# smhassanerfani/nasa-niswan

Measured on NVIDIA B200. Metric: train samples/sec, higher is better.
Workload: dtype bf16

## Files before the change

nasa_niswan_b200/csrc/nint_api.cu:

```cuda
#include <cuda.h>
#include <cuda_runtime.h>
#include <stdarg.h>
#include <stdio.h>
#include <stdlib.h>
#include <string.h>

#include <new>
#include <vector>

#include "../../include/nint.h"
#include "nint_kernels.h"

namespace {

using namespace nint;
enum : int { BF16 = 0, TF32 = 1 };

thread_local char g_err[512] = "";
int fail(const char* fmt, ...) {
  va_list ap;
  va_start(ap, fmt);
  vsnprintf(g_err, sizeof(g_err), fmt, ap);
  va_end(ap);
  return 1;
}
#define CK(expr)                                                                                   \
  do {                                                                                             \
    cudaError_t e__ = (expr);                                                                      \
    if (e__ != cudaSuccess) return fail("%s failed: %s (%s:%d)", #expr, cudaGetErrorString(e__), __FILE__, __LINE__); \
  } while (0)

typedef CUresult (*EncodeTiledFn)(CUtensorMap*, CUtensorMapDataType, cuuint32_t, void*, const cuuint64_t*,
                                  const cuuint64_t*, const cuuint32_t*, const cuuint32_t*, CUtensorMapInterleave,
                                  CUtensorMapSwizzle, CUtensorMapL2promotion, CUtensorMapFloatOOBfill);
EncodeTiledFn get_encode() {
  static EncodeTiledFn fn = nullptr;
  if (!fn) {
    void* p = nullptr;
    cudaDriverEntryPointQueryResult q;
    if (cudaGetDriverEntryPoint("cuTensorMapEncodeTiled", &p, cudaEnableDefault, &q) == cudaSuccess &&
        q == cudaDriverEntryPointSuccess)
      fn = reinterpret_cast<EncodeTiledFn>(p);
  }
  return fn;
}

inline size_t align_up(size_t v, size_t a) { return (v + a - 1) / a * a; }

enum : int { K_FWD = 0, K_BWD = 1, K_WGRAD = 2, K_OTHER = 3, K_NCLS = 4 };
constexpr int kResidCtas = 160;
constexpr long long kResidMaxPixelSteps = 1LL << 20;
long long g_launches[K_NCLS] = {0, 0, 0, 0};

struct Profile {
  bool on = false;
  std::vector<cudaEvent_t> pool;
  std::vector<int> cls;
  std::vector<int> weight;
  size_t used = 0;
};

struct Layer {
  int cin, hc_real, hc, k, taps;
  int cin_rows;
  int cx_pad, hc_pad, chx, chh;
  int hcb, n_blocks, n_tile;
  int nslots_h, nslots_c;
  uint8_t* Hs = nullptr;
  float* Cs = nullptr;
  uint8_t* G = nullptr;
  float* dC = nullptr;
  uint8_t *wx = nullptr, *wh = nullptr, *wdx = nullptr, *wdh = nullptr;
  float *bias_q = nullptr, *dw_acc = nullptr, *db_acc = nullptr;
  float* db_resid = nullptr;
  size_t dw_acc_bytes = 0;
  int det_splits = 0;
  int ncols = 0;
  CUtensorMap tm_H, tm_G;
  struct WMap { int ts = 0, rows = 0, n_tile = 0; CUtensorMap map; };
  std::vector<WMap> wmaps[4];
  CUtensorMap tm_H_up;
  CUtensorMap tmw_H, tmw_G;
  CUtensorMap tmw_H_up;
  CUtensorMap tmp_G, tmp_H, tmp_H_up;
  struct WgBlock {
    int col0 = 0, cols = 0;
    int n_mma = 0;
    int nch_x = 0, nch_h = 0;
    int chan0_x = 0, chan0_h = 0;
    bool pair = false;
    int pw = 16, a_bufs = 0, b_stages = 0;
  };
  std::vector<WgBlock> wg_blocks;
  CUtensorMap tme_C, tme_H, tme_G, tme_dC;
  bool weights_set = false;
  bool bias_folded = false;
  struct CachedConv { bool valid = false; ConvGemmParams g; };
  CachedConv fwd_cache[2][2], bwd_cache[2];
};

}

struct nint_plan {
  nint_config cfg;
  int L, B, T, H, W, dtype, esize, ce;
  int tile_w, tile_h, tiles_x, tiles_y;
  int num_sms = 148;
  Layer layer[NINT_MAX_LAYERS];
  size_t ws_bytes = 0;
  uint8_t* ws = nullptr;
  uint8_t* X = nullptr;
  CUtensorMap tm_X, tmw_X, tmp_X;
  bool x_bank = false;
  const void* bank_ptr = nullptr;
  long long bank_frames = 0;
  const int* win_start = nullptr;
  CUtensorMap tmb_X, tmbw_X, tmbp_X;
  float *head_w = nullptr, *head_b = nullptr;
  float* raw = nullptr;
  float* dh_ext = nullptr;
  float* head_part = nullptr;
  unsigned* step_done = nullptr;
  int fuse_steps = -1;
  bool head_set = false;
  bool zero_init = true;
  bool fwd_done = false;
  bool gates_valid = false;
  bool bptt_done = false;
  bool deterministic = false, input_grad = false;
  int pdl = 0;
  int sub_batch = 0;
  int final_slot_h = 0, final_slot_c = 0;
  int cluster = 2;
  int debug_flags = 0;
  int ones_lane = -1;
  int plan_g = 0, plan_ns = 0;
  Profile prof;
};

namespace {

template <typename F>
int launch(nint_plan* p, int cls, cudaStream_t st, const char* what, F&& f) {
  cudaEvent_t e1 = nullptr;
  if (p && p->prof.on) {
    Profile& pr = p->prof;
    if (pr.pool.size() < 2 * (pr.used + 1)) {
      cudaEvent_t a, b;
      if (cudaEventCreate(&a) != cudaSuccess || cudaEventCreate(&b) != cudaSuccess) return fail("cudaEventCreate failed");
      pr.pool.push_back(a);
      pr.pool.push_back(b);
    }
    e1 = pr.pool[2 * pr.used + 1];
    if (pr.cls.size() <= pr.used) pr.cls.resize(pr.used + 1), pr.weight.resize(pr.used + 1);
    pr.cls[pr.used] = cls;
    pr.weight[pr.used] = 1;
    cudaEventRecord(pr.pool[2 * pr.used], st);
    ++pr.used;
  }
  cudaError_t e = f();
  if (e1) cudaEventRecord(e1, st);
  if (e != cudaSuccess) return fail("%s failed: %s", what, cudaGetErrorString(e));
  ++g_launches[cls];
  return 0;
}
#define LAUNCH(plan, cls, st, call) \
  do { if (launch(plan, cls, st, #call, [&]() { return (call); })) return 1; } while (0)

int pick_tile(int H, int W, int* tw_out, int* th_out) {
  (void)H; (void)W;
  *tw_out = 8;
  *th_out = 16;
  return 0;
}

int encode_act_map(CUtensorMap* m, int dtype, void* base, int C, int W, int H, int B, int slots, int ce, int tw,
                   int th, bool wgrad = false, int halo = 0) {
  tw += 2 * halo;
  th += 2 * halo;
  EncodeTiledFn enc = get_encode();
  if (!enc) return fail("cuTensorMapEncodeTiled not available (no CUDA driver?)");
  const cuuint64_t es = dtype == BF16 ? 2 : 4;
  cuuint64_t dims[5] = {(cuuint64_t)C, (cuuint64_t)W, (cuuint64_t)H, (cuuint64_t)B, (cuuint64_t)slots};
  cuuint64_t strides[4] = {C * es, (cuuint64_t)W * C * es, (cuuint64_t)H * W * C * es,
                           (cuuint64_t)B * H * W * C * es};
  cuuint32_t box[5] = {(cuuint32_t)(wgrad ? 32 : ce), (cuuint32_t)tw, (cuuint32_t)th, 1, 1};
  cuuint32_t estr[5] = {1, 1, 1, 1, 1};
  const CUtensorMapSwizzle sw = (wgrad && dtype == TF32) ? CU_TENSOR_MAP_SWIZZLE_128B_ATOM_32B : CU_TENSOR_MAP_SWIZZLE_64B;
  CUresult r = enc(m, dtype == BF16 ? CU_TENSOR_MAP_DATA_TYPE_BFLOAT16 : CU_TENSOR_MAP_DATA_TYPE_FLOAT32, 5, base,
                   dims, strides, box, estr, CU_TENSOR_MAP_INTERLEAVE_NONE, sw,
                   CU_TENSOR_MAP_L2_PROMOTION_L2_128B, CU_TENSOR_MAP_FLOAT_OOB_FILL_NONE);
  if (r != CUDA_SUCCESS) return fail("cuTensorMapEncodeTiled(activation C=%d W=%d H=%d B=%d slots=%d) -> %d", C, W, H, B, slots, (int)r);
  return 0;
}

int encode_act_box(CUtensorMap* m, int dtype, void* base, int C, int W, int H, int B, int slots, int box_c, int tw,
                   int th, int halo, CUtensorMapSwizzle sw) {
  EncodeTiledFn enc = get_encode();
  if (!enc) return fail("cuTensorMapEncodeTiled not available (no CUDA driver?)");
  const cuuint64_t es = dtype == BF16 ? 2 : 4;
  cuuint64_t dims[5] = {(cuuint64_t)C, (cuuint64_t)W, (cuuint64_t)H, (cuuint64_t)B, (cuuint64_t)slots};
  cuuint64_t strides[4] = {C * es, (cuuint64_t)W * C * es, (cuuint64_t)H * W * C * es,
                           (cuuint64_t)B * H * W * C * es};
  cuuint32_t box[5] = {(cuuint32_t)box_c, (cuuint32_t)(tw + 2 * halo), (cuuint32_t)(th + 2 * halo), 1, 1};
  cuuint32_t estr[5] = {1, 1, 1, 1, 1};
  CUresult r = enc(m, dtype == BF16 ? CU_TENSOR_MAP_DATA_TYPE_BFLOAT16 : CU_TENSOR_MAP_DATA_TYPE_FLOAT32, 5, base,
                   dims, strides, box, estr, CU_TENSOR_MAP_INTERLEAVE_NONE, sw, CU_TENSOR_MAP_L2_PROMOTION_L2_128B,
                   CU_TENSOR_MAP_FLOAT_OOB_FILL_NONE);
  if (r != CUDA_SUCCESS) return fail("cuTensorMapEncodeTiled(box C=%d box_c=%d halo=%d) -> %d", C, box_c, halo, (int)r);
  return 0;
}

int encode_io_map(CUtensorMap* m, bool fp32, void* base, int C, int W, int H, int B, int slots, int box_c) {
  EncodeTiledFn enc = get_encode();
  if (!enc) return fail("cuTensorMapEncodeTiled not available (no CUDA driver?)");
  const cuuint64_t es = fp32 ? 4 : 2;
  cuuint64_t dims[5] = {(cuuint64_t)C, (cuuint64_t)W, (cuuint64_t)H, (cuuint64_t)B, (cuuint64_t)slots};
  cuuint64_t strides[4] = {C * es, (cuuint64_t)W * C * es, (cuuint64_t)H * W * C * es,
                           (cuuint64_t)B * H * W * C * es};
  cuuint32_t box[5] = {(cuuint32_t)box_c, 8, 16, 1, 1};
  cuuint32_t estr[5] = {1, 1, 1, 1, 1};
  const int row_bytes = box_c * (int)es;
  CUtensorMapSwizzle sw;
  if (row_bytes == 32) sw = CU_TENSOR_MAP_SWIZZLE_32B;
  else if (row_bytes == 64) sw = CU_TENSOR_MAP_SWIZZLE_64B;
  else if (row_bytes == 128) sw = CU_TENSOR_MAP_SWIZZLE_128B;
  else return fail("encode_io_map: unsupported box row of %d bytes", row_bytes);
  CUresult r = enc(m, fp32 ? CU_TENSOR_MAP_DATA_TYPE_FLOAT32 : CU_TENSOR_MAP_DATA_TYPE_BFLOAT16, 5, base, dims, strides,
                   box, estr, CU_TENSOR_MAP_INTERLEAVE_NONE, sw, CU_TENSOR_MAP_L2_PROMOTION_L2_128B,
                   CU_TENSOR_MAP_FLOAT_OOB_FILL_NONE);
  if (r != CUDA_SUCCESS) return fail("cuTensorMapEncodeTiled(io C=%d W=%d H=%d B=%d slots=%d box=%d) -> %d", C, W, H, B, slots, box_c, (int)r);
  return 0;
}

int encode_w_map(CUtensorMap* m, int dtype, void* base, long long chunk_taps, int ce, int n_tile, int w_rows, int ts) {
  EncodeTiledFn enc = get_encode();
  if (!enc) return fail("cuTensorMapEncodeTiled not available (no CUDA driver?)");
  const cuuint64_t es = dtype == BF16 ? 2 : 4;
  cuuint64_t dims[3] = {(cuuint64_t)ce, (cuuint64_t)n_tile, (cuuint64_t)chunk_taps};
  cuuint64_t strides[2] = {ce * es, (cuuint64_t)n_tile * ce * es};
  cuuint32_t box[3] = {(cuuint32_t)ce, (cuuint32_t)w_rows, (cuuint32_t)ts};
  cuuint32_t estr[3] = {1, 1, 1};
  CUresult r = enc(m, dtype == BF16 ? CU_TENSOR_MAP_DATA_TYPE_BFLOAT16 : CU_TENSOR_MAP_DATA_TYPE_FLOAT32, 3, base,
                   dims, strides, box, estr, CU_TENSOR_MAP_INTERLEAVE_NONE, CU_TENSOR_MAP_SWIZZLE_64B,
                   CU_TENSOR_MAP_L2_PROMOTION_L2_256B, CU_TENSOR_MAP_FLOAT_OOB_FILL_NONE);
  if (r != CUDA_SUCCESS) return fail("cuTensorMapEncodeTiled(weights chunk_taps=%lld n_tile=%d rows=%d ts=%d) -> %d", chunk_taps, n_tile, w_rows, ts, (int)r);
  return 0;
}

uint32_t idesc_of(int dtype, int m, int n, int a_mn, int b_mn) {
  const uint32_t fmt = dtype == BF16 ? 1u : 2u;
  return (1u << 4) | (fmt << 7) | (fmt << 10) | ((uint32_t)(a_mn & 1) << 15) | ((uint32_t)(b_mn & 1) << 16) |
         ((uint32_t)(n >> 3) << 17) | ((uint32_t)(m >> 4) << 24);
}

size_t act_bytes(const nint_plan* p, int slots, int c) {
  return static_cast<size_t>(slots) * p->B * p->H * p->W * c * p->esize;
}

size_t carve(nint_plan* p, uint8_t* base) {
  size_t off = 0;
  auto take = [&](size_t bytes) -> uint8_t* {
    uint8_t* r = base ? base + off : nullptr;
    off += align_up(bytes, 1024);
    return r;
  };
  const bool tr = p->cfg.training != 0;
  const size_t npix = static_cast<size_t>(p->B) * p->H * p->W;
  p->X = take(act_bytes(p, p->T, p->layer[0].cx_pad));
  for (int l = 0; l < p->L; ++l) {
    Layer& y = p->layer[l];
    y.Hs = take(act_bytes(p, y.nslots_h, y.hc_pad));
    y.Cs = reinterpret_cast<float*>(take(static_cast<size_t>(y.nslots_c) * npix * y.hc * 4));
    y.G = tr ? take(act_bytes(p, p->T, 4 * y.hc)) : nullptr;
    y.dC = tr ? reinterpret_cast<float*>(take(npix * y.hc * 4)) : nullptr;
    const size_t wrow = static_cast<size_t>(p->ce) * p->esize;
    y.wx = take(static_cast<size_t>(y.n_blocks) * y.taps * y.chx * y.n_tile * wrow);
    y.wh = take(static_cast<size_t>(y.n_blocks) * y.taps * y.chh * y.n_tile * wrow);
    y.bias_q = reinterpret_cast<float*>(take(4 * y.hc * 4));
    if (tr) {
      const int nch = 4 * y.hc / p->ce;
      y.wdx = (l > 0 || p->input_grad) ? take(static_cast<size_t>(y.taps) * nch * y.cin_rows * wrow) : nullptr;
      y.wdh = take(static_cast<size_t>(y.taps) * nch * y.hc * wrow);
      y.dw_acc_bytes = static_cast<size_t>(y.taps) * 4 * y.hc * y.ncols * 4;
      const size_t slices = p->deterministic ? static_cast<size_t>(y.det_splits) : 1;
      y.dw_acc = reinterpret_cast<float*>(take(y.dw_acc_bytes * slices));
      y.db_acc = reinterpret_cast<float*>(take(4 * y.hc * 4 * slices));
      y.db_resid = p->dtype == TF32 ? reinterpret_cast<float*>(take(static_cast<size_t>(kResidCtas) * 4 * 4 * y.hc * 4)) : nullptr;
    }
  }
  const Layer& top = p->layer[p->L - 1];
  p->head_w = reinterpret_cast<float*>(take(top.hc * 4));
  p->head_b = reinterpret_cast<float*>(take(16));
  if (tr && p->deterministic)
    p->head_part = reinterpret_cast<float*>(take(static_cast<size_t>(head_bwd_blocks(p->B)) * (top.hc_real + 1) * 4));
  p->step_done = reinterpret_cast<unsigned*>(take(static_cast<size_t>(p->T) * p->B * 4));
  if (tr && p->input_grad) {
    const Layer& y0 = p->layer[0];
    const size_t cols = y0.cin_rows > y0.hc ? y0.cin_rows : y0.hc;
    p->raw = reinterpret_cast<float*>(take(npix * cols * 4));
    p->dh_ext = reinterpret_cast<float*>(take(npix * y0.hc * 4));
  }
  return off;
}

inline uint8_t* slot_ptr(const nint_plan* p, uint8_t* base, int slot, int c) {
  return base + act_bytes(p, 1, c) * slot;
}
inline float* cslot_ptr(const nint_plan* p, const Layer& y, int slot) {
  return y.Cs + static_cast<size_t>(slot) * p->B * p->H * p->W * y.hc;
}

void fill_common(const nint_plan* p, const Layer& y, ConvGemmParams& g) {
  memset(&g, 0, sizeof(g));
  g.debug_flags = p->debug_flags;
  g.pdl = p->pdl;
  g.plan_g = p->plan_g; g.plan_ns = p->plan_ns;
  g.B = p->B; g.b0 = 0; g.H = p->H; g.W = p->W;
  g.tile_w = p->tile_w; g.tile_h = p->tile_h; g.tiles_x = p->tiles_x; g.tiles_y = p->tiles_y;
  g.hc = y.hc; g.hc_pad = y.hc_pad; g.hcb = y.hcb;
  g.n_steps = 1;
  g.c_prev_none_step = -1;
}

int arm_fused(nint_plan* p, ConvGemmParams& g, int n_steps, int storer_warps, cudaStream_t st) {
  g.n_steps = n_steps;
  g.step_done = p->step_done;
  g.step_target = static_cast<unsigned>(p->tiles_x * p->tiles_y * g.n_blocks * storer_warps);
  if (reinterpret_cast<uint8_t*>(p->step_done) < p->ws ||
      reinterpret_cast<uint8_t*>(p->step_done + static_cast<size_t>(n_steps) * p->B) > p->ws + p->ws_bytes)
    return fail("internal: step counters outside the workspace (%p, ws %p + %zu)", (void*)p->step_done, (void*)p->ws, p->ws_bytes);
  CK(cudaMemsetAsync(p->step_done, 0, static_cast<size_t>(n_steps) * p->B * 4, st));
  return 0;
}

int fwd_cluster(const nint_plan* p, int l) {
  (void)l;
  return p->cluster;
}
int bwd_cluster(const nint_plan* p, int l) {
  return p->layer[l].hc % 32 == 0 ? p->cluster : 1;
}

int get_w_map(nint_plan* p, Layer& y, int which, int n_tile, int rows, int ts, CUtensorMap* out) {
  for (const Layer::WMap& w : y.wmaps[which])
    if (w.ts == ts && w.rows == rows && w.n_tile == n_tile) { *out = w.map; return 0; }
  void* base = which == 0 ? y.wx : which == 1 ? y.wh : which == 2 ? y.wdx : y.wdh;
  if (!base) return fail("internal: packed weight tensor %d of this layer was not allocated", which);
  long long chunk_taps;
  if (which == 0) chunk_taps = (long long)y.n_blocks * y.chx * y.taps;
  else if (which == 1) chunk_taps = (long long)y.n_blocks * y.chh * y.taps;
  else chunk_taps = (long long)(4 * y.hc / p->ce) * y.taps;
  Layer::WMap w;
  w.ts = ts; w.rows = rows; w.n_tile = n_tile;
  if (encode_w_map(&w.map, p->dtype, base, chunk_taps, p->ce, n_tile, rows, ts)) return 1;
  y.wmaps[which].push_back(w);
  *out = w.map;
  return 0;
}

inline void set_batch_range(const nint_plan* p, ConvGemmParams& g, int b0, int nb) {
  g.b0 = nb > 0 ? b0 : 0;
  g.B = nb > 0 ? nb : p->B;
}

int fwd_conv_params(nint_plan* p, int l, bool have_state, int epi, ConvGemmParams& g) {
  Layer& y = p->layer[l];
  const bool tr = p->cfg.training != 0;
  const bool bank = l == 0 && p->x_bank;
  Layer::CachedConv* cache = epi == EPI_FWD ? &y.fwd_cache[have_state ? 1 : 0][bank ? 1 : 0] : nullptr;
  if (cache && cache->valid) {
    g = cache->g;
  } else {
    fill_common(p, y, g);
    g.n_tile = y.n_tile;
    g.n_blocks = y.n_blocks;
    g.cluster = fwd_cluster(p, l);
    g.idesc = idesc_of(p->dtype, 128 * g.cluster, y.n_tile, 0, 0);
    int s = 0;
    g.seg[s].tmap_act = l == 0 ? (bank ? p->tmb_X : p->tm_X) : p->layer[l - 1].tm_H_up;
    g.seg[s].wsel = 0;
    g.seg[s].ksize = y.k;
    g.seg[s].nchunks = y.chx;
    ++s;
    if (have_state) {
      g.seg[s].tmap_act = y.tm_H;
      g.seg[s].wsel = 1;
      g.seg[s].ksize = y.k;
      g.seg[s].nchunks = y.chh;
      ++s;
    }
    g.nseg = s;
    g.tm_c = y.tme_C; g.tm_h = y.tme_H; g.tm_g = y.tme_G; g.tm_dc = y.tme_dC;
    g.slot_g = (tr && epi == EPI_FWD) ? 0 : -1;
    if (conv_halo_plan(epi, p->dtype, g)) return fail("layer %d: the conv kernel's shared-memory plan does not fit (hidden %d, k %d)", l, y.hc, y.k);
    for (int i = 0; i < g.nseg; ++i)
      if (get_w_map(p, y, g.seg[i].wsel, g.n_tile, g.n_tile / g.cluster, g.seg[i].ts, &g.seg[i].tmap_w)) return 1;
    if (cache) { cache->g = g; cache->valid = true; }
  }
  return 0;
}

int cell_step(nint_plan* p, int l, int t, int epi, float* raw_out, cudaStream_t st, int b0 = 0, int nb = 0, int n_steps = 1) {
  Layer& y = p->layer[l];
  const bool tr = p->cfg.training != 0;
  const bool have_state = !(t == 0 && p->zero_init);
  const bool bank = l == 0 && p->x_bank;
  ConvGemmParams g;
  if (fwd_conv_params(p, l, have_state, epi, g)) return 1;
  const int in_slot_h = tr ? t : (t & 1);
  const int out_slot_h = tr ? t + 1 : ((t + 1) & 1);
  g.seg[0].slot = l == 0 ? t : (tr ? t + 1 : ((t + 1) & 1));
  g.seg[0].win_start = bank ? p->win_start : nullptr;
  g.seg[0].bank_frames = bank ? static_cast<int>(p->bank_frames) : 0;
  if (have_state) g.seg[1].slot = in_slot_h;
  g.slot_c_in = have_state ? (tr ? t : 0) : -1;
  g.slot_c_out = tr ? t + 1 : 0;
  g.slot_h_out = out_slot_h;
  g.slot_g = (tr && epi == EPI_FWD) ? t : -1;
  g.bias_q = (y.bias_folded && epi == EPI_FWD) ? nullptr : y.bias_q;
  g.raw_out = raw_out;
  set_batch_range(p, g, b0, nb);
  g.n_steps = 1;
  if (n_steps > 1) {
    if (!have_state || epi != EPI_FWD || nb > 0) return fail("internal: time-fused forward launch without a recurrent state");
    g.d_seg[0] = g.d_seg[1] = g.d_h_out = g.d_g = 1;
    g.d_c_in = g.d_c_out = tr ? 1 : 0;
    g.ring_bits = tr ? 0 : ((l > 0 ? 1 : 0) | 2 | 16);
    if (arm_fused(p, g, n_steps, 2, st)) return 1;
  }
  LAUNCH(p, (epi == EPI_FWD ? K_FWD : K_OTHER), st, launch_conv_halo(epi, p->dtype, g, p->num_sms, st));
  if (p->prof.on && p->prof.used > 0) p->prof.weight[p->prof.used - 1] = n_steps;
  return 0;
}

int dgrad_raw(nint_plan* p, int l, int t, int wsel, int n_rows, float* raw_out, cudaStream_t st) {
  Layer& y = p->layer[l];
  ConvGemmParams g;
  fill_common(p, y, g);
  g.n_tile = n_rows;
  g.n_blocks = 1;
  g.cluster = (n_rows % 32 == 0) ? p->cluster : 1;
  g.idesc = idesc_of(p->dtype, 128 * g.cluster, n_rows, 0, 0);
  g.seg[0].tmap_act = y.tm_G; g.seg[0].wsel = wsel; g.seg[0].slot = t;
  g.seg[0].ksize = y.k; g.seg[0].nchunks = 4 * y.hc / p->ce;
  g.nseg = 1;
  g.tm_c = y.tme_C; g.tm_h = y.tme_H; g.tm_g = y.tme_G; g.tm_dc = y.tme_dC;
  g.slot_g = g.slot_c_in = g.slot_c_out = g.slot_h_out = g.slot_c_prev = -1;
  g.raw_out = raw_out;
  if (conv_halo_plan(EPI_RAW, p->dtype, g)) return fail("layer %d: the dgrad kernel's shared-memory plan does not fit (N %d, k %d)", l, n_rows, y.k);
  if (get_w_map(p, y, wsel, g.n_tile, g.n_tile / g.cluster, g.seg[0].ts, &g.seg[0].tmap_w)) return 1;
  LAUNCH(p, K_OTHER, st, launch_conv_halo(EPI_RAW, p->dtype, g, p->num_sms, st));
  return 0;
}

}

static int plan_wgrad_blocks(nint_plan* p, Layer& y) {
  y.wg_blocks.clear();
  const int px = y.cx_pad / 32, ph = y.hc_pad / 32;
  auto pair_block = [&](int col0, int x_cols, int cols) {
    Layer::WgBlock b;
    b.col0 = col0; b.cols = cols;
    b.nch_x = x_cols / 32; b.nch_h = (cols - x_cols) / 32;
    b.pair = true;
    b.pw = wgrad_pair_panel_width(x_cols, cols);
    b.a_bufs = 3;
    b.b_stages = wgrad_pair_b_stages(x_cols, cols, y.k);
    b.n_mma = cols;
    return b;
  };
  if (p->cluster == 2 && p->dtype == TF32 && (4 * y.hc) % 256 == 0 && &y == &p->layer[0] && p->ones_lane >= 0) {
    const int n_mma = (y.ncols / 32 + 1) / 2 * 64;
    const int st = n_mma <= 256 ? wgrad_pair_b_stages_tf32(n_mma, y.k) : 0;
    if (st >= 2) {
      Layer::WgBlock b;
      b.col0 = 0; b.cols = y.ncols; b.n_mma = n_mma;
      b.nch_x = y.cx_pad / 32; b.nch_h = y.hc_pad / 32;
      b.pair = true; b.pw = 32; b.a_bufs = 2; b.b_stages = st;
      y.wg_blocks.push_back(b);
      return 0;
    }
  }
  if (p->cluster == 2 && p->dtype == BF16 && (4 * y.hc) % 256 == 0) {
    if (wgrad_pair_supported(p->dtype, 4 * y.hc, y.cx_pad, y.ncols, y.k)) {
      y.wg_blocks.push_back(pair_block(0, y.cx_pad, y.ncols));
      return 0;
    }
    if (wgrad_pair_supported(p->dtype, 4 * y.hc, y.cx_pad, y.cx_pad, y.k) &&
        wgrad_pair_supported(p->dtype, 4 * y.hc, 0, y.hc_pad, y.k)) {
      y.wg_blocks.push_back(pair_block(0, y.cx_pad, y.cx_pad));
      y.wg_blocks.push_back(pair_block(y.cx_pad, 0, y.hc_pad));
      return 0;
    }
  }
  const int panels = px + ph, bpb = wgrad_b_panel_bytes(p->dtype, 1, y.k);
  int per = panels, a_bufs = 0, b_stages = 0;
  for (; per >= 1; --per) {
    wgrad_pick_buffers(p->dtype, per, bpb, &a_bufs, &b_stages);
    if (per * 32 <= 256 && (b_stages >= 2 || (per == 1 && b_stages >= 1))) break;
  }
  if (per < 1) return 1;
  for (int j0 = 0; j0 < panels; j0 += per) {
    const int j1 = j0 + per < panels ? j0 + per : panels;
    Layer::WgBlock b;
    b.col0 = j0 * 32; b.cols = b.n_mma = (j1 - j0) * 32;
    b.nch_x = (j1 < px ? j1 : px) - (j0 < px ? j0 : px);
    b.nch_h = (j1 - j0) - b.nch_x;
    b.chan0_x = (j0 < px ? j0 : px) * 32;
    b.chan0_h = (j0 > px ? j0 - px : 0) * 32;
    wgrad_pick_buffers(p->dtype, j1 - j0, bpb, &b.a_bufs, &b.b_stages);
    y.wg_blocks.push_back(b);
  }
  return 0;
}

static int wgrad_params(nint_plan* p, int l, size_t bi, int num_sms, WgradParams& w) {
  Layer& y = p->layer[l];
  const int T = p->T;
  const Layer::WgBlock& blk = y.wg_blocks[bi];
  const int bias_col = (l == 0) ? p->ones_lane : -1;
  const long long total_tiles = static_cast<long long>(T) * p->B * p->tiles_x * p->tiles_y;
  memset(&w, 0, sizeof(w));
  w.halo = 1;
  w.debug_flags = p->debug_flags;
  w.b_panel_bytes = wgrad_b_panel_bytes(p->dtype, w.halo, y.k);
  w.slot_b0[0] = l == 0 ? 0 : 1;
  w.slot_b0[1] = 0;
  w.nchunks_b[0] = blk.nch_x;
  w.nchunks_b[1] = blk.nch_h;
  w.chan0[0] = blk.chan0_x;
  w.chan0[1] = blk.chan0_h;
  w.T = T; w.B = p->B; w.H = p->H; w.W = p->W;
  w.tile_w = p->tile_w; w.tile_h = p->tile_h; w.tiles_x = p->tiles_x; w.tiles_y = p->tiles_y;
  w.ksize = y.k;
  w.hc4 = 4 * y.hc;
  w.pair = blk.pair ? 1 : 0;
  const bool bank = l == 0 && p->x_bank;
  w.win_start = bank ? p->win_start : nullptr;
  if (w.pair && p->dtype == BF16) {
    w.tmap_dg = y.tmp_G;
    w.tmap_b[0] = l == 0 ? (bank ? p->tmbp_X : p->tmp_X) : p->layer[l - 1].tmp_H_up;
    w.tmap_b[1] = y.tmp_H;
  } else {
    w.tmap_dg = y.tmw_G;
    w.tmap_b[0] = l == 0 ? (bank ? p->tmbw_X : p->tmw_X) : p->layer[l - 1].tmw_H_up;
    w.tmap_b[1] = y.tmw_H;
  }
  if (blk.nch_x == 0) { w.tmap_b[0] = w.tmap_b[1]; w.win_start = nullptr; }
  if (blk.nch_h == 0) w.tmap_b[1] = w.tmap_b[0];
  w.m_blocks = w.pair ? w.hc4 / 256 : (w.hc4 + 127) / 128;
  w.ncols = y.ncols;
  w.acc_cols = blk.n_mma;
  w.real_cols = blk.cols;
  w.col0 = blk.col0;
  const int bias_cols = (bias_col >= 0 || bi > 0) ? 0 : 32;
  const int tpg = 512 / blk.n_mma;
  if (tpg < 1) return fail("wgrad: %d columns exceed the accumulator", blk.n_mma);
  int ng = 0, tap = 0;
  w.group_tap0[0] = 0;
  const int rest = y.taps % tpg;
  const bool bias_last = rest > 0 && rest * blk.n_mma + bias_cols <= 512;
  const int g0 = bias_last ? tpg : ((512 - bias_cols) / blk.n_mma < tpg ? (512 - bias_cols) / blk.n_mma : tpg);
  if (g0 < 1) return fail("wgrad: %d columns leave no room for the bias columns", blk.n_mma);
  while (tap < y.taps) {
    const int n = ng == 0 ? g0 : tpg;
    tap = tap + n > y.taps ? y.taps : tap + n;
    if (ng + 1 > kMaxWgradGroups) return fail("wgrad: too many tap groups");
    w.group_tap0[++ng] = tap;
  }
  w.bias_group = bias_cols == 0 ? -1 : (bias_last ? ng - 1 : 0);
  w.n_groups = ng;
  {
    int units = (w.pair ? num_sms / 2 : num_sms) / w.m_blocks;
    if (units < ng) units = ng;
    auto mma_cost = [&](int n) { return w.pair ? (n / 2 > 40 ? n / 2 : 40) : (n * 2 / 3 > 88 ? n * 2 / 3 : 88); };
    int cost[kMaxWgradGroups], tot = 0;
    for (int g = 0; g < ng; ++g) {
      cost[g] = (w.group_tap0[g + 1] - w.group_tap0[g]) * mma_cost(blk.n_mma) + (g == w.bias_group ? mma_cost(32) : 0);
      tot += cost[g];
    }
    const bool even = (p->debug_flags & 64) != 0;
    int used = 0;
    for (int g = 0; g < ng; ++g) {
      int sp = even ? units / ng : static_cast<int>(static_cast<long long>(units) * cost[g] / tot);
      if (sp < 1) sp = 1;
      w.group_splits[g] = sp;
      used += sp;
    }
    while (!even && used < units) {
      int best = 0;
      for (int g = 1; g < ng; ++g)
        if (static_cast<long long>(cost[g]) * w.group_splits[best] > static_cast<long long>(cost[best]) * w.group_splits[g]) best = g;
      ++w.group_splits[best];
      ++used;
    }
    w.group_unit0[0] = 0;
    for (int g = 0; g < ng; ++g) {
      if (w.group_splits[g] > total_tiles) w.group_splits[g] = static_cast<int>(total_tiles);
      w.group_unit0[g + 1] = w.group_unit0[g] + w.m_blocks * w.group_splits[g];
    }
  }
  w.b_pw = blk.pw;
  w.a_bufs = blk.a_bufs;
  w.b_stages = blk.b_stages;
  if (w.b_stages < 1) return fail("wgrad: operand panels do not fit in shared memory");
  w.idesc = idesc_of(p->dtype, w.pair ? 256 : 128, blk.n_mma, 1, 1);
  w.idesc_bias = idesc_of(p->dtype, w.pair ? 256 : 128, 32, 1, 1);
  w.dw_acc = y.dw_acc;
  w.db_acc = y.db_acc;
  w.dw_part = p->deterministic ? y.dw_acc : nullptr;
  w.db_part = p->deterministic ? y.db_acc : nullptr;
  return 0;
}
static int wgrad_max_splits(const WgradParams& w) {
  int m = 1;
  for (int g = 0; g < w.n_groups; ++g) if (w.group_splits[g] > m) m = w.group_splits[g];
  return m;
}

extern "C" {

int nint_version(void) { return 100; }
const char* nint_last_error(void) { return g_err; }
int nint_gate_column(int q, int hidden) { return q_to_n(q, hidden); }
int nint_pick_tile(int height, int width, int* tile_w, int* tile_h) {
  if (height < 1 || width < 1 || !tile_w || !tile_h) return fail("nint_pick_tile: bad arguments");
  return pick_tile(height, width, tile_w, tile_h);
}

long long nint_launch_count(int kernel_class) {
  if (kernel_class < 0) return g_launches[0] + g_launches[1] + g_launches[2] + g_launches[3];
  return kernel_class < K_NCLS ? g_launches[kernel_class] : 0;
}

int nint_plan_profile(nint_plan* p, int enable) {
  if (!p) return fail("null plan");
  p->prof.on = enable != 0;
  p->prof.used = 0;
  return 0;
}

int nint_plan_profile_read(nint_plan* p, double* ms, long long* count) {
  if (!p || !ms || !count) return fail("nint_plan_profile_read: null argument");
  Profile& pr = p->prof;
  for (int c = 0; c < K_NCLS; ++c) ms[c] = 0.0, count[c] = 0;
  for (size_t i = 0; i < pr.used; ++i) {
    CK(cudaEventSynchronize(pr.pool[2 * i + 1]));
    float t = 0.f;
    CK(cudaEventElapsedTime(&t, pr.pool[2 * i], pr.pool[2 * i + 1]));
    ms[pr.cls[i]] += t;
    count[pr.cls[i]] += pr.weight[i];
  }
  pr.used = 0;
  return 0;
}

int nint_plan_create(const nint_config* cfg, nint_plan** out) {
  if (!cfg || !out) return fail("nint_plan_create: null argument");
  if (cfg->num_layers < 1 || cfg->num_layers > NINT_MAX_LAYERS)
    return fail("num_layers must be in [1,%d], got %d", NINT_MAX_LAYERS, cfg->num_layers);
  if (cfg->batch < 1 || cfg->seq_len < 1 || cfg->height < 1 || cfg->width < 1 || cfg->in_channels < 1)
    return fail("batch/seq_len/height/width/in_channels must be positive");
  if (cfg->dtype != BF16 && cfg->dtype != TF32) return fail("unknown dtype %d", cfg->dtype);
  nint_plan* p = new (std::nothrow) nint_plan();
  if (!p) return fail("out of host memory");
  p->cfg = *cfg;
  p->L = cfg->num_layers; p->B = cfg->batch; p->T = cfg->seq_len; p->H = cfg->height; p->W = cfg->width;
  p->dtype = cfg->dtype;
  p->esize = cfg->dtype == BF16 ? 2 : 4;
  p->ce = 64 / p->esize;
  p->deterministic = (cfg->flags & NINT_FLAG_DETERMINISTIC) != 0;
  p->input_grad = (cfg->flags & NINT_FLAG_INPUT_GRAD) != 0;
  {
    const char* c = getenv("NINT_CLUSTER");
    p->cluster = c ? atoi(c) : 2;
    if (p->cluster != 1 && p->cluster != 2) p->cluster = 1;
    const char* d = getenv("NINT_DEBUG_FLAGS");
    p->debug_flags = d ? atoi(d) : 0;
    if (!NINT_KNOBS && (p->debug_flags & ~512)) {
      const int flags = p->debug_flags;
      delete p;
      return fail("NINT_DEBUG_FLAGS=%d needs the experiment build of the library (python -m nasa_niswan_b200.build --knobs, "
                  "then NINT_LIB=<...>/libnint_knobs.so): the product build compiles the kernel knobs out", flags);
    }
    const char* pg = getenv("NINT_PLAN_G");
    p->plan_g = pg ? atoi(pg) : 0;
    const char* pn = getenv("NINT_PLAN_NS");
    p->plan_ns = pn ? atoi(pn) : 0;
    if (const char* e = getenv("NINT_DETERMINISTIC")) p->deterministic = p->deterministic || atoi(e) != 0;
    const char* pd = getenv("NINT_PDL");
    p->pdl = pd ? (atoi(pd) != 0) : 0;
    if (const char* e = getenv("NINT_FUSE_STEPS")) p->fuse_steps = atoi(e);
    const char* sb = getenv("NINT_SUB_BATCH");
    p->sub_batch = sb ? atoi(sb) : 0;
    if (p->sub_batch < 0 || p->sub_batch >= p->B) p->sub_batch = 0;
  }
  pick_tile(p->H, p->W, &p->tile_w, &p->tile_h);
  p->tiles_x = (p->W + p->tile_w - 1) / p->tile_w;
  p->tiles_y = (p->H + p->tile_h - 1) / p->tile_h;
  int cin = cfg->in_channels, below_hc = 0;
  for (int l = 0; l < p->L; ++l) {
    Layer& y = p->layer[l];
    y.cin = cin; y.hc_real = cfg->hidden[l]; y.k = cfg->ksize[l]; y.taps = y.k * y.k;
    if (y.hc_real < 1 || y.hc_real > 256) {
      delete p;
      return fail("hidden_channels[%d] = %d unsupported (1 .. 256)", l, cfg->hidden[l]);
    }
    y.hc = y.hc_real <= 64 ? (y.hc_real + 15) / 16 * 16 : (y.hc_real + 63) / 64 * 64;
    if (y.k < 1 || y.k % 2 == 0 || y.k > 15) {
      delete p;
      return fail("kernel_size[%d] = %d unsupported (odd, <= 15)", l, y.k);
    }
    if (l > 0 && cin > 256) { delete p; return fail("layer %d input channels %d > 256", l, cin); }
    y.cx_pad = l == 0 ? (y.cin + 31) / 32 * 32 : (below_hc + 31) / 32 * 32;
    y.chx = y.cx_pad / p->ce;
    y.hc_pad = (y.hc + 31) / 32 * 32;  y.chh = y.hc_pad / p->ce;
    y.cin_rows = l == 0 ? y.cx_pad : below_hc;
    if (l == 0 && y.cx_pad > y.cin && !(p->debug_flags & 128)) p->ones_lane = y.cin;
    y.hcb = y.hc < 64 ? y.hc : 64;
    if (cfg->dtype == BF16) {
      bool fits = false;
      for (int cand = y.hcb; cand >= 32 && !fits; cand >>= 1) {
        const long long w_cta = static_cast<long long>(y.cx_pad / 32 + y.hc_pad / 32) * y.taps * (4 * cand / p->cluster) * 64;
        if (y.hc % cand == 0 && w_cta <= 112 * 1024) { y.hcb = cand; fits = true; }
      }
      if (!fits && y.hc >= 32 && y.hc % 32 == 0) y.hcb = 32;
    }
    if (const char* e = getenv("NINT_HCB")) {
      const int v = atoi(e);
      if (v >= 16 && v <= 64 && (v & (v - 1)) == 0 && y.hc % v == 0) y.hcb = v;
    }
    y.n_blocks = y.hc / y.hcb; y.n_tile = 4 * y.hcb;
    y.nslots_h = cfg->training ? p->T + 1 : 2;
    y.nslots_c = cfg->training ? p->T + 1 : 1;
    y.ncols = y.cx_pad + y.hc_pad;
    if (cfg->training && plan_wgrad_blocks(p, y)) {
      const int hc = y.hc, k = y.k;
      delete p;
      return fail("layer %d: training with hidden %d, kernel %d: not even one 32-channel wgrad operand panel fits in "
                  "shared memory", l, hc, k);
    }
    if (cfg->training && p->deterministic) {
      y.det_splits = 1;
      for (size_t bi = 0; bi < y.wg_blocks.size(); ++bi) {
        WgradParams w;
        if (wgrad_params(p, l, bi, 148, w)) { delete p; return 1; }
        if (wgrad_max_splits(w) > y.det_splits) y.det_splits = wgrad_max_splits(w);
      }
    }
    cin = y.hc_real;
    below_hc = y.hc;
  }
  if (p->input_grad && cfg->training && p->layer[0].cin_rows > 256) {
    delete p;
    return fail("input gradient: %d input channels exceed one MMA N (256)", cfg->in_channels);
  }
  p->ws_bytes = carve(p, nullptr);
  *out = p;
  return 0;
}

void nint_plan_destroy(nint_plan* plan) {
  if (!plan) return;
  for (cudaEvent_t e : plan->prof.pool) cudaEventDestroy(e);
  delete plan;
}

size_t nint_plan_workspace_bytes(const nint_plan* plan) { return plan ? plan->ws_bytes : 0; }

int nint_plan_input_layout(const nint_plan* plan, int* c_pad, int* ones_lane, int* elem_bytes) {
  if (!plan) return fail("null plan");
  if (c_pad) *c_pad = plan->layer[0].cx_pad;
  if (ones_lane) *ones_lane = plan->ones_lane;
  if (elem_bytes) *elem_bytes = plan->esize;
  return 0;
}

static int encode_input_maps(nint_plan* p, void* base, long long images, int slots, CUtensorMap* conv, CUtensorMap* wg,
                             CUtensorMap* wg_pair) {
  const int tw = p->tile_w, th = p->tile_h, ce = p->ce, pad0 = p->layer[0].k / 2;
  Layer& y = p->layer[0];
  if (images > 0x7fffffffLL) return fail("too many frames (%lld)", images);
  const int n = static_cast<int>(images);
  if (encode_act_map(conv, p->dtype, base, y.cx_pad, p->W, p->H, n, slots, ce, tw, th, false, pad0)) return 1;
  if (encode_act_map(wg, p->dtype, base, y.cx_pad, p->W, p->H, n, slots, ce, tw, th, true, pad0)) return 1;
  if (p->cfg.training && p->dtype == BF16)
    for (const Layer::WgBlock& b : y.wg_blocks) {
      if (!b.pair || b.nch_x == 0) continue;
      const CUtensorMapSwizzle sw = b.pw == 64 ? CU_TENSOR_MAP_SWIZZLE_128B : (b.pw == 32 ? CU_TENSOR_MAP_SWIZZLE_64B : CU_TENSOR_MAP_SWIZZLE_32B);
      if (encode_act_box(wg_pair, p->dtype, base, y.cx_pad, p->W, p->H, n, slots, b.pw, tw, th, pad0, sw)) return 1;
    }
  return 0;
}

int nint_plan_bind(nint_plan* p, void* workspace, size_t bytes, void* stream) {
  if (!p || !workspace) return fail("nint_plan_bind: null argument");
  if (bytes < p->ws_bytes) return fail("workspace too small: %zu < %zu", bytes, p->ws_bytes);
  if (reinterpret_cast<uintptr_t>(workspace) % 256) return fail("workspace must be 256-byte aligned");
  cudaStream_t st = static_cast<cudaStream_t>(stream);
  int dev = 0, sms = 0, cc_major = 0;
  CK(cudaGetDevice(&dev));
  CK(cudaDeviceGetAttribute(&sms, cudaDevAttrMultiProcessorCount, dev));
  CK(cudaDeviceGetAttribute(&cc_major, cudaDevAttrComputeCapabilityMajor, dev));
  if (cc_major != 10) return fail("libnint needs an sm_100 device (Blackwell B200); found compute capability %d.x", cc_major);
  p->num_sms = sms;
  p->ws = static_cast<uint8_t*>(workspace);
  carve(p, p->ws);
  CK(cudaMemsetAsync(p->ws, 0, p->ws_bytes, st));
  const int tw = p->tile_w, th = p->tile_h, ce = p->ce;
  auto pad_of = [&](int l) { return p->layer[l].k / 2; };
  if (encode_input_maps(p, p->X, p->B, p->T, &p->tm_X, &p->tmw_X, &p->tmp_X)) return 1;
  p->x_bank = false; p->bank_ptr = nullptr; p->bank_frames = 0; p->win_start = nullptr;
  for (int l = 0; l < p->L; ++l) {
    Layer& y = p->layer[l];
    for (auto& a : y.fwd_cache) for (auto& c : a) c.valid = false;
    for (auto& c : y.bwd_cache) c.valid = false;
    if (encode_act_map(&y.tm_H, p->dtype, y.Hs, y.hc_pad, p->W, p->H, p->B, y.nslots_h, ce, tw, th, false, pad_of(l))) return 1;
    if (l + 1 < p->L &&
        encode_act_map(&y.tm_H_up, p->dtype, y.Hs, y.hc_pad, p->W, p->H, p->B, y.nslots_h, ce, tw, th, false, pad_of(l + 1))) return 1;
    if (encode_io_map(&y.tme_C, true, y.Cs, y.hc, p->W, p->H, p->B, y.nslots_c, 16)) return 1;
    if (encode_io_map(&y.tme_H, p->dtype == TF32, y.Hs, y.hc_pad, p->W, p->H, p->B, y.nslots_h, 16)) return 1;
    if (p->cfg.training) {
      if (encode_io_map(&y.tme_G, p->dtype == TF32, y.G, 4 * y.hc, p->W, p->H, p->B, p->T, 128 / p->esize)) return 1;
      if (encode_io_map(&y.tme_dC, true, y.dC, y.hc, p->W, p->H, p->B, 1, 16)) return 1;
    } else {
      y.tme_G = y.tme_C;
      y.tme_dC = y.tme_C;
    }
    for (auto& v : y.wmaps) v.clear();
    if (p->cfg.training) {
      if (encode_act_map(&y.tm_G, p->dtype, y.G, 4 * y.hc, p->W, p->H, p->B, p->T, ce, tw, th, false, pad_of(l))) return 1;
      if (encode_act_map(&y.tmw_G, p->dtype, y.G, 4 * y.hc, p->W, p->H, p->B, p->T, ce, tw, th, true)) return 1;
      if (encode_act_map(&y.tmw_H, p->dtype, y.Hs, y.hc_pad, p->W, p->H, p->B, y.nslots_h, ce, tw, th, true, pad_of(l))) return 1;
      if (l + 1 < p->L &&
          encode_act_map(&y.tmw_H_up, p->dtype, y.Hs, y.hc_pad, p->W, p->H, p->B, y.nslots_h, ce, tw, th, true, pad_of(l + 1))) return 1;
    }
  }
  if (p->cfg.training) {
    for (int l = 0; l < p->L; ++l) {
      Layer& y = p->layer[l];
      auto sw_of = [](int pw) {
        return pw == 64 ? CU_TENSOR_MAP_SWIZZLE_128B : (pw == 32 ? CU_TENSOR_MAP_SWIZZLE_64B : CU_TENSOR_MAP_SWIZZLE_32B);
      };
      bool any_pair = false;
      for (const Layer::WgBlock& b : y.wg_blocks) {
        if (!b.pair || p->dtype != BF16) continue;
        any_pair = true;
        if (b.nch_h > 0 &&
            encode_act_box(&y.tmp_H, p->dtype, y.Hs, y.hc_pad, p->W, p->H, p->B, y.nslots_h, b.pw, tw, th, pad_of(l), sw_of(b.pw))) return 1;
        if (b.nch_x > 0 && l > 0) {
          Layer& dn = p->layer[l - 1];
          if (encode_act_box(&dn.tmp_H_up, p->dtype, dn.Hs, dn.hc_pad, p->W, p->H, p->B, dn.nslots_h, b.pw, tw, th, pad_of(l), sw_of(b.pw))) return 1;
        }
      }
      if (any_pair &&
          encode_act_box(&y.tmp_G, p->dtype, y.G, 4 * y.hc, p->W, p->H, p->B, p->T, 64, tw, th, 0, CU_TENSOR_MAP_SWIZZLE_128B)) return 1;
    }
  }
  p->zero_init = true;
  p->fwd_done = false;
  p->gates_valid = false;
  p->bptt_done = false;
  return 0;
}

int nint_plan_set_weights(nint_plan* p, int l, const float* weight, const float* bias, void* stream) {
  if (!p || !p->ws) return fail("plan not bound");
  if (l < 0 || l >= p->L) return fail("layer %d out of range", l);
  if (!weight) return fail("null weight");
  Layer& y = p->layer[l];
  cudaStream_t st = static_cast<cudaStream_t>(stream);
  y.bias_folded = l == 0 && p->ones_lane >= 0 && bias != nullptr && !(p->debug_flags & 512);
  LAUNCH(p, K_OTHER, st, launch_pack_weights_fwd(p->dtype, weight, bias, y.wx, y.wh, y.bias_q, y.cin, y.hc_real, y.hc, y.hcb, y.k, y.cx_pad, y.hc_pad,
                                                 y.bias_folded ? p->ones_lane : -1, st));
  if (p->cfg.training) LAUNCH(p, K_OTHER, st, launch_pack_weights_bwd(p->dtype, weight, y.wdx, y.wdh, y.cin, y.cin_rows, y.hc_real, y.hc, y.k, st));
  y.weights_set = true;
  return 0;
}

int nint_plan_set_head(nint_plan* p, const float* weight, const float* bias, void* stream) {
  if (!p || !p->ws) return fail("plan not bound");
  if (!weight || !bias) return fail("null head parameter");
  cudaStream_t st = static_cast<cudaStream_t>(stream);
  CK(cudaMemcpyAsync(p->head_w, weight, p->layer[p->L - 1].hc_real * 4, cudaMemcpyDeviceToDevice, st));
  CK(cudaMemcpyAsync(p->head_b, bias, 4, cudaMemcpyDeviceToDevice, st));
  p->head_set = true;
  return 0;
}

int nint_plan_reset_state(nint_plan* p, void* stream) {
  if (!p || !p->ws) return fail("plan not bound");
  cudaStream_t st = static_cast<cudaStream_t>(stream);
  if (!p->zero_init) {
    for (int l = 0; l < p->L; ++l) {
      Layer& y = p->layer[l];
      CK(cudaMemsetAsync(y.Hs, 0, act_bytes(p, 1, y.hc_pad), st));
      CK(cudaMemsetAsync(y.Cs, 0, static_cast<size_t>(p->B) * p->H * p->W * y.hc * 4, st));
    }
  }
  p->zero_init = true;
  return 0;
}

int nint_plan_set_state(nint_plan* p, int l, const float* h, const float* c, void* stream) {
  if (!p || !p->ws) return fail("plan not bound");
  if (l < 0 || l >= p->L || !h || !c) return fail("nint_plan_set_state: bad arguments");
  Layer& y = p->layer[l];
  cudaStream_t st = static_cast<cudaStream_t>(stream);
  if (p->zero_init) {
    for (int j = 0; j < p->L; ++j) {
      Layer& z = p->layer[j];
      CK(cudaMemsetAsync(z.Hs, 0, act_bytes(p, 1, z.hc_pad), st));
      CK(cudaMemsetAsync(z.Cs, 0, static_cast<size_t>(p->B) * p->H * p->W * z.hc * 4, st));
    }
  }
  LAUNCH(p, K_OTHER, st, launch_pack_state(p->dtype, h, y.Hs, p->B, y.hc_real, p->H, p->W, y.hc_pad, st));
  LAUNCH(p, K_OTHER, st, launch_nchw_to_nhwc_f32(c, y.Cs, p->B, y.hc_real, p->H, p->W, y.hc, st));
  p->zero_init = false;
  return 0;
}

int nint_plan_get_state(nint_plan* p, int l, float* h, float* c, void* stream) {
  if (!p || !p->ws) return fail("plan not bound");
  if (l < 0 || l >= p->L) return fail("layer %d out of range", l);
  if (!p->fwd_done) return fail("nint_plan_get_state before nint_forward");
  Layer& y = p->layer[l];
  cudaStream_t st = static_cast<cudaStream_t>(stream);
  if (h) LAUNCH(p, K_OTHER, st, launch_unpack_state(p->dtype, slot_ptr(p, y.Hs, p->final_slot_h, y.hc_pad), h, p->B, y.hc_real, p->H, p->W, y.hc_pad, st));
  if (c) LAUNCH(p, K_OTHER, st, launch_nhwc_to_nchw_f32(cslot_ptr(p, y, p->final_slot_c), c, p->B, y.hc_real, p->H, p->W, y.hc, st));
  return 0;
}

static int check_ready(nint_plan* p) {
  if (!p || !p->ws) return fail("plan not bound");
  for (int l = 0; l < p->L; ++l)
    if (!p->layer[l].weights_set) return fail("weights of layer %d not set", l);
  if (!p->head_set) return fail("head parameters not set");
  return 0;
}

static int fwd_should_fuse(nint_plan* p, int l, bool* fuse) {
  *fuse = false;
  if (p->fuse_steps == 0) return 0;
  if (p->fuse_steps > 0) {
    *fuse = (p->fuse_steps & 1) != 0;
    return 0;
  }
  ConvGemmParams g;
  if (fwd_conv_params(p, l, true, EPI_FWD, g)) return 1;
  const int per_group = g.cluster * g.group;
  const double groups = (static_cast<double>(p->B) * p->tiles_x * p->tiles_y + per_group - 1) / per_group;
  const int clusters = p->num_sms / (g.cluster * g.n_blocks);
  *fuse = clusters > 0 && groups / clusters <= 16.0;
  return 0;
}

static int forward_steps(nint_plan* p, float* pred, float* seq, cudaStream_t st) {
  const bool tr = p->cfg.training != 0;
  const long long HW = static_cast<long long>(p->H) * p->W;
  const Layer& top = p->layer[p->L - 1];
  const size_t top_img = static_cast<size_t>(HW) * top.hc_pad * p->esize;
  const int SB = p->sub_batch > 0 ? p->sub_batch : p->B;
  bool fuse_l[NINT_MAX_LAYERS];
  bool any_fused = false;
  for (int l = 0; l < p->L; ++l) {
    fuse_l[l] = false;
    if (SB >= p->B && p->T > 1 && (tr || (p->L == 1 && !seq)) && fwd_should_fuse(p, l, &fuse_l[l])) return 1;
    any_fused = any_fused || fuse_l[l];
  }
  if (any_fused) {
    for (int l = 0; l < p->L; ++l) {
      int t = 0;
      if (p->zero_init || !fuse_l[l]) {
        if (cell_step(p, l, 0, EPI_FWD, nullptr, st)) return 1;
        t = 1;
      }
      if (!fuse_l[l] || p->T - t == 1) {
        for (; t < p->T; ++t)
          if (cell_step(p, l, t, EPI_FWD, nullptr, st)) return 1;
      } else if (cell_step(p, l, t, EPI_FWD, nullptr, st, 0, 0, p->T - t)) return 1;
    }
    if (seq)
      for (int t = 0; t < p->T; ++t)
        LAUNCH(p, K_OTHER, st, launch_head_fwd(p->dtype, slot_ptr(p, top.Hs, t + 1, top.hc_pad), p->head_w, p->head_b,
                           seq + t * HW, HW, p->B, top.hc_real, top.hc_pad, p->T * HW, st));
  } else
  for (int b0 = 0; b0 < p->B; b0 += SB) {
    const int nb = b0 + SB <= p->B ? SB : p->B - b0;
    for (int t = 0; t < p->T; ++t) {
      for (int l = 0; l < p->L; ++l)
        if (cell_step(p, l, t, EPI_FWD, nullptr, st, b0, SB < p->B ? nb : 0)) return 1;
      if (seq) {
        const int slot = tr ? t + 1 : ((t + 1) & 1);
        LAUNCH(p, K_OTHER, st, launch_head_fwd(p->dtype, slot_ptr(p, top.Hs, slot, top.hc_pad) + b0 * top_img, p->head_w, p->head_b,
                           seq + b0 * p->T * HW + t * HW, HW, nb, top.hc_real, top.hc_pad, p->T * HW, st));
      }
    }
  }
  p->final_slot_h = tr ? p->T : (p->T & 1);
  p->final_slot_c = tr ? p->T : 0;
  LAUNCH(p, K_OTHER, st, launch_head_fwd(p->dtype, slot_ptr(p, top.Hs, p->final_slot_h, top.hc_pad), p->head_w, p->head_b, pred, HW, p->B,
                     top.hc_real, top.hc_pad, HW, st));
  p->fwd_done = true;
  p->gates_valid = tr;
  p->bptt_done = false;
  return 0;
}

int nint_forward_ex(nint_plan* p, const void* x, int x_dtype, float* pred, float* seq, void* stream) {
  if (check_ready(p)) return 1;
  if (!x || !pred) return fail("nint_forward: null x / pred");
  if (seq && !p->cfg.return_sequence) return fail("seq output requires return_sequence in the plan");
  if (x_dtype != NINT_X_FP32 && x_dtype != NINT_X_BF16) return fail("unknown x dtype %d", x_dtype);
  if (x_dtype == NINT_X_BF16 && p->dtype != BF16) return fail("bf16 inputs need a bf16 plan (a tf32 plan would lose input precision)");
  cudaStream_t st = static_cast<cudaStream_t>(stream);
  p->x_bank = false;
  LAUNCH(p, K_OTHER, st, launch_pack_input(p->dtype, x, x_dtype == NINT_X_BF16, p->X, p->B, p->T, p->cfg.in_channels, p->H, p->W, p->layer[0].cx_pad, p->ones_lane, st));
  return forward_steps(p, pred, seq, st);
}

int nint_forward(nint_plan* p, const float* x, float* pred, float* seq, void* stream) {
  return nint_forward_ex(p, x, NINT_X_FP32, pred, seq, stream);
}

int nint_forward_bank(nint_plan* p, const void* bank, long long n_frames, const int* win_start, float* pred, float* seq,
                      void* stream) {
  if (check_ready(p)) return 1;
  if (!bank || !win_start || !pred) return fail("nint_forward_bank: null bank / win_start / pred");
  if (n_frames < p->T) return fail("nint_forward_bank: %lld frames cannot hold a window of %d steps", n_frames, p->T);
  if (reinterpret_cast<uintptr_t>(bank) % 128) return fail("the frame bank must be 128-byte aligned");
  if (seq && !p->cfg.return_sequence) return fail("seq output requires return_sequence in the plan");
  cudaStream_t st = static_cast<cudaStream_t>(stream);
  if (bank != p->bank_ptr || n_frames != p->bank_frames) {
    if (encode_input_maps(p, const_cast<void*>(bank), n_frames, 1, &p->tmb_X, &p->tmbw_X, &p->tmbp_X)) return 1;
    p->bank_ptr = bank;
    p->bank_frames = n_frames;
    for (auto& a : p->layer[0].fwd_cache) a[1].valid = false;
  }
  p->x_bank = true;
  p->win_start = win_start;
  return forward_steps(p, pred, seq, st);
}

int nint_pack_frames(int dtype, const void* frames, int x_dtype, long long n_frames, int channels, int height, int width,
                     int c_pad, int ones_lane, void* bank, void* stream) {
  if (!frames || !bank) return fail("nint_pack_frames: null argument");
  if (dtype != BF16 && dtype != TF32) return fail("unknown dtype %d", dtype);
  if (x_dtype != NINT_X_FP32 && x_dtype != NINT_X_BF16) return fail("unknown x dtype %d", x_dtype);
  if (n_frames < 1 || channels < 1 || height < 1 || width < 1) return fail("nint_pack_frames: bad shape");
  if (c_pad < channels || c_pad % 16) return fail("nint_pack_frames: c_pad %d must be a multiple of 16 and >= %d", c_pad, channels);
  if (ones_lane >= 0 && (ones_lane < channels || ones_lane >= c_pad)) return fail("nint_pack_frames: ones lane %d outside the padding lanes", ones_lane);
  cudaStream_t st = static_cast<cudaStream_t>(stream);
  LAUNCH(nullptr, K_OTHER, st, launch_pack_frames(dtype, frames, x_dtype == NINT_X_BF16, bank, n_frames, channels, height, width, c_pad, ones_lane, st));
  return 0;
}

static int check_fuse_args(const float* levels3d, const float* emis2d, const float* mean, const float* std,
                           const float* statics, int n_static, long long frames, int levels, int height, int width,
                           int padded_height, int padded_width, int mode, const void* out) {
  if ((!levels3d && levels > 0) || !emis2d || !mean || !std || !out) return fail("nint_fuse_inputs: null argument");
  if (n_static < 0 || (n_static > 0 && !statics)) return fail("nint_fuse_inputs: %d static fields but no data", n_static);
  if (frames < 1 || levels < 0 || height < 1 || width < 1) return fail("nint_fuse_inputs: bad shape");
  if (mode != 0 && mode != 1) return fail("nint_fuse_inputs: mode must be 0 (reflect) or 1 (reference RNN dataset)");
  const int left = (padded_width - width) / 2, right = padded_width - width - left;
  const int top = (padded_height - height) / 2, bot = padded_height - height - top;
  if (padded_width < width || padded_height < height) return fail("nint_fuse_inputs: padded size smaller than the grid");
  if (left > width || right > width)
    return fail("The requested padding size is larger than width size of the input image.");
  if (top + 1 > height || bot + 1 > height)
    return fail("The requested padding size is larger than height size of the input image.");
  return 0;
}

int nint_fuse_inputs(const float* levels3d, const float* emis2d, const float* mean, const float* std,
                     const float* statics, int n_static, long long frames, int levels, int height, int width,
                     int padded_height, int padded_width, int mode, float* out, void* stream) {
  if (check_fuse_args(levels3d, emis2d, mean, std, statics, n_static, frames, levels, height, width, padded_height, padded_width, mode, out)) return 1;
  cudaStream_t st = static_cast<cudaStream_t>(stream);
  LAUNCH(nullptr, K_OTHER, st, launch_fuse_inputs(levels3d, emis2d, mean, std, statics, n_static, out, frames, levels, height, width, padded_height, padded_width, mode, st));
  return 0;
}

int nint_fuse_inputs_bank(const float* levels3d, const float* emis2d, const float* mean, const float* std,
                          const float* statics, int n_static, long long frames, int levels, int height, int width,
                          int padded_height, int padded_width, int mode, int dtype, int c_pad, int ones_lane,
                          void* bank, void* stream) {
  if (check_fuse_args(levels3d, emis2d, mean, std, statics, n_static, frames, levels, height, width, padded_height, padded_width, mode, bank)) return 1;
  if (dtype != BF16 && dtype != TF32) return fail("unknown dtype %d", dtype);
  const int C = levels + 1 + n_static;
  if (c_pad < C || c_pad % 16 || c_pad > 64) return fail("nint_fuse_inputs_bank: c_pad %d must be a multiple of 16 in [%d, 64]", c_pad, C);
  if (ones_lane >= 0 && (ones_lane < C || ones_lane >= c_pad)) return fail("nint_fuse_inputs_bank: ones lane %d outside the padding lanes", ones_lane);
  cudaStream_t st = static_cast<cudaStream_t>(stream);
  LAUNCH(nullptr, K_OTHER, st, launch_fuse_inputs_bank(dtype, levels3d, emis2d, mean, std, statics, n_static, bank, frames, levels, height, width, padded_height, padded_width, mode, c_pad, ones_lane, st));
  return 0;
}

static int check_loss_args(const float* pred, const float* y, const float* loss, const float* stats, int batch, int height,
                           int width, int crop_y0, int crop_y1, int crop_x0, int crop_x1) {
  if (!pred || !y || !loss || !stats) return fail("nint_loss_mse_l1: null argument");
  if (batch < 1 || height < 1 || width < 1) return fail("nint_loss_mse_l1: bad shape");
  if (crop_y0 < 0 || crop_y1 > height || crop_y0 >= crop_y1 || crop_x0 < 0 || crop_x1 > width || crop_x0 >= crop_x1)
    return fail("nint_loss_mse_l1: crop [%d:%d, %d:%d] outside %dx%d", crop_y0, crop_y1, crop_x0, crop_x1, height, width);
  return 0;
}

int nint_loss_mse_l1(const float* pred, const float* y, int batch, int height, int width, int crop_y0, int crop_y1,
                     int crop_x0, int crop_x1, float* dpred, float* loss, float* stats, void* stream) {
  if (check_loss_args(pred, y, loss, stats, batch, height, width, crop_y0, crop_y1, crop_x0, crop_x1)) return 1;
  cudaStream_t st = static_cast<cudaStream_t>(stream);
  LAUNCH(nullptr, K_OTHER, st, launch_loss_mse_l1(pred, y, dpred, stats, loss, batch, height, width, crop_y0, crop_y1, crop_x0, crop_x1, nullptr, 0, 0, st));
  return 0;
}

int nint_loss_mse_l1_bank(const float* pred, const float* ybank, long long n_frames, const int* win_start, int y_offset, int batch,
                          int height, int width, int crop_y0, int crop_y1, int crop_x0, int crop_x1, float* dpred,
                          float* loss, float* stats, void* stream) {
  if (check_loss_args(pred, ybank, loss, stats, batch, height, width, crop_y0, crop_y1, crop_x0, crop_x1)) return 1;
  if (!win_start || n_frames < 1) return fail("nint_loss_mse_l1_bank: null win_start / empty target bank");
  cudaStream_t st = static_cast<cudaStream_t>(stream);
  LAUNCH(nullptr, K_OTHER, st, launch_loss_mse_l1(pred, ybank, dpred, stats, loss, batch, height, width, crop_y0, crop_y1, crop_x0, crop_x1, win_start, y_offset, n_frames, st));
  return 0;
}

int nint_adam_step(float* params, const float* grads, float* exp_avg, float* exp_avg_sq, long long n, float lr,
                   float beta1, float beta2, float eps, int step, float grad_scale, void* stream) {
  if (!params || !grads || !exp_avg || !exp_avg_sq) return fail("nint_adam_step: null argument");
  if (n < 0 || step < 1) return fail("nint_adam_step: n >= 0 and step >= 1 required");
  cudaStream_t st = static_cast<cudaStream_t>(stream);
  LAUNCH(nullptr, K_OTHER, st, launch_adam(params, grads, exp_avg, exp_avg_sq, n, lr, beta1, beta2, eps, step, grad_scale, st));
  return 0;
}

int nint_adam_step_dev(float* params, const float* grads, float* exp_avg, float* exp_avg_sq, long long n, float* state,
                       float beta1, float beta2, float eps, float grad_scale, void* stream) {
  if (!params || !grads || !exp_avg || !exp_avg_sq || !state) return fail("nint_adam_step_dev: null argument");
  if (n < 0) return fail("nint_adam_step_dev: n >= 0 required");
  cudaStream_t st = static_cast<cudaStream_t>(stream);
  LAUNCH(nullptr, K_OTHER, st, launch_adam_dev(params, grads, exp_avg, exp_avg_sq, n, state, beta1, beta2, eps, grad_scale, st));
  ++g_launches[K_OTHER];
  return 0;
}

int nint_dp_allreduce_adam(const void* const* peer_buffers, long long slot_offset_bytes, long long flags_offset_bytes,
                           int rank, int world, unsigned seq, float* params, float* exp_avg, float* exp_avg_sq,
                           long long n, float* state, float beta1, float beta2, float eps, float grad_scale, void* stream) {
  if (!peer_buffers || !params || !exp_avg || !exp_avg_sq || !state) return fail("nint_dp_allreduce_adam: null argument");
  if (world < 1 || world > 16 || rank < 0 || rank >= world) return fail("nint_dp_allreduce_adam: rank %d of %d (at most 16 ranks)", rank, world);
  if (n < 0 || seq == 0) return fail("nint_dp_allreduce_adam: n >= 0 and seq >= 1 required");
  if (slot_offset_bytes % 16 || flags_offset_bytes % 16) return fail("nint_dp_allreduce_adam: offsets must be 16-byte aligned");
  for (int r = 0; r < world; ++r)
    if (!peer_buffers[r]) return fail("nint_dp_allreduce_adam: no mapping of rank %d's buffer", r);
  cudaStream_t st = static_cast<cudaStream_t>(stream);
  LAUNCH(nullptr, K_OTHER, st, launch_dp_allreduce_adam(peer_buffers, slot_offset_bytes, flags_offset_bytes, rank, world, seq, params,
                                                        exp_avg, exp_avg_sq, n, state, beta1, beta2, eps, grad_scale, st));
  return 0;
}

int nint_debug_read_trace(long long* host, int n, int clear) {
  if (!host || n < 0) return fail("nint_debug_read_trace: bad arguments");
  CK(cudaDeviceSynchronize());
  CK(read_trace(host, n));
  if (clear) CK(clear_trace());
  return 0;
}

int nint_debug_fail_record(unsigned long long* out5) {
  if (!out5) return fail("nint_debug_fail_record: null argument");
  cudaError_t e = fail_record(out5);
  if (e != cudaSuccess) return fail("nint_debug_fail_record: %s", cudaGetErrorString(e));
  return 0;
}

int nint_debug_raw_gates(nint_plan* p, const float* x, float* out, void* stream) {
  if (check_ready(p)) return 1;
  if (!x || !out) return fail("nint_debug_raw_gates: null argument");
  cudaStream_t st = static_cast<cudaStream_t>(stream);
  p->x_bank = false;
  LAUNCH(p, K_OTHER, st, launch_pack_input(p->dtype, x, 0, p->X, p->B, p->T, p->cfg.in_channels, p->H, p->W, p->layer[0].cx_pad, p->ones_lane, st));
  return cell_step(p, 0, 0, EPI_RAW, out, st);
}

static bool resid_on(const nint_plan* p) {
  return p->num_sms <= kResidCtas && static_cast<long long>(p->B) * p->T * p->H * p->W <= kResidMaxPixelSteps;
}

static int bwd_conv_params(nint_plan* p, int l, bool has_next, ConvGemmParams& g) {
  const int L = p->L;
  Layer& y = p->layer[l];
  Layer::CachedConv& cache = y.bwd_cache[has_next ? 1 : 0];
  if (cache.valid) {
    g = cache.g;
  } else {
    fill_common(p, y, g);
    g.n_tile = y.hc;
    g.n_blocks = 1;
    g.cluster = bwd_cluster(p, l);
    g.idesc = idesc_of(p->dtype, 128 * g.cluster, y.hc, 0, 0);
    int s = 0;
    if (has_next) {
      g.seg[s].tmap_act = y.tm_G; g.seg[s].wsel = 3;
      g.seg[s].ksize = y.k; g.seg[s].nchunks = 4 * y.hc / p->ce;
      ++s;
    }
    if (l < L - 1) {
      Layer& up = p->layer[l + 1];
      g.seg[s].tmap_act = up.tm_G; g.seg[s].wsel = 2;
      g.seg[s].ksize = up.k; g.seg[s].nchunks = 4 * up.hc / p->ce;
      ++s;
    }
    g.nseg = s;
    g.tm_c = y.tme_C; g.tm_h = y.tme_H; g.tm_g = y.tme_G; g.tm_dc = y.tme_dC;
    g.slot_c_in = g.slot_c_out = g.slot_h_out = -1;
    if (conv_halo_plan(EPI_BWD, p->dtype, g)) return fail("layer %d: the dgrad kernel's shared-memory plan does not fit (hidden %d, k %d)", l, y.hc, y.k);
    for (int i = 0; i < g.nseg; ++i) {
      Layer& owner = g.seg[i].wsel == 2 ? p->layer[l + 1] : y;
      if (get_w_map(p, owner, g.seg[i].wsel, g.n_tile, g.n_tile / g.cluster, g.seg[i].ts, &g.seg[i].tmap_w)) return 1;
    }
    cache.g = g;
    cache.valid = true;
  }
  return 0;
}

static int bwd_should_fuse(nint_plan* p, int l, bool* fuse) {
  *fuse = false;
  const int SB = p->sub_batch > 0 ? p->sub_batch : p->B;
  if (SB < p->B || p->T <= 2 || p->fuse_steps == 0) return 0;
  if (p->fuse_steps > 0) {
    *fuse = (p->fuse_steps & 2) != 0;
    return 0;
  }
  ConvGemmParams g;
  if (bwd_conv_params(p, l, true, g)) return 1;
  const int per_group = g.cluster * g.group;
  const double groups = (static_cast<double>(p->B) * p->tiles_x * p->tiles_y + per_group - 1) / per_group;
  const int clusters = p->num_sms / g.cluster;
  *fuse = clusters > 0 && groups / clusters <= 10.0;
  return 0;
}

static int bwd_step(nint_plan* p, int l, int t, const float* dpred, const float* dseq, const float* dh_ext, bool dc_given,
                    cudaStream_t st, int b0, int nb, int n_steps = 1) {
  const long long HW = static_cast<long long>(p->H) * p->W;
  const int L = p->L, T = p->T;
  Layer& y = p->layer[l];
  const bool has_next = t < T - 1;
  ConvGemmParams g;
  if (bwd_conv_params(p, l, has_next, g)) return 1;
  int s = 0;
  if (has_next) g.seg[s++].slot = t + 1;
  if (l < L - 1) g.seg[s++].slot = t;
  g.slot_g = t;
  g.slot_c_prev = (t == 0 && p->zero_init) ? -1 : t;
  g.has_dc_in = (t == T - 1) ? (dc_given ? 1 : 0) : 1;
  g.head_dpred = nullptr; g.head_w = nullptr; g.head_dpred_bstride = 0;
  if (l == L - 1) {
    if (dseq) {
      g.head_dpred = dseq + t * HW;
      g.head_dpred_bstride = T * HW;
      g.head_w = p->head_w;
    } else if (t == T - 1 && dpred) {
      g.head_dpred = dpred;
      g.head_dpred_bstride = HW;
      g.head_w = p->head_w;
    }
  }
  g.dh_ext = (l == L - 1 && t == T - 1) ? dh_ext : nullptr;
  g.db_resid = resid_on(p) ? y.db_resid : nullptr;
  set_batch_range(p, g, b0, nb);
  g.n_steps = 1;
  g.c_prev_none_step = -1;
  if (n_steps > 1) {
    if (!has_next || nb > 0 || t - n_steps + 1 < 0) return fail("internal: bad time-fused backward launch");
    g.d_seg[0] = g.d_seg[1] = g.d_g = g.d_c_prev = -1;
    g.ring_bits = 0;
    g.slot_c_prev = t;
    g.c_prev_none_step = (p->zero_init && t - n_steps + 1 == 0) ? n_steps - 1 : -1;
    g.head_dpred_sstride = -HW;
    if (arm_fused(p, g, n_steps, 2, st)) return 1;
  }
  LAUNCH(p, K_BWD, st, launch_conv_halo(EPI_BWD, p->dtype, g, p->num_sms, st));
  if (p->prof.on && p->prof.used > 0) p->prof.weight[p->prof.used - 1] = n_steps;
  return 0;
}

static int bptt_loop(nint_plan* p, const float* dpred, const float* dseq, const float* dh_ext, bool dc_given, cudaStream_t st) {
  const int SB = p->sub_batch > 0 ? p->sub_batch : p->B;
  for (int l = 0; l < p->L; ++l)
    if (p->layer[l].db_resid) CK(cudaMemsetAsync(p->layer[l].db_resid, 0, static_cast<size_t>(kResidCtas) * 4 * 4 * p->layer[l].hc * 4, st));
  bool any_fused = false;
  bool fuse_l[NINT_MAX_LAYERS];
  for (int l = 0; l < p->L; ++l) {
    if (bwd_should_fuse(p, l, &fuse_l[l])) return 1;
    any_fused = any_fused || fuse_l[l];
  }
  if (any_fused) {
    for (int l = p->L - 1; l >= 0; --l) {
      if (bwd_step(p, l, p->T - 1, dpred, dseq, dh_ext, dc_given, st, 0, 0)) return 1;
      if (fuse_l[l]) {
        if (bwd_step(p, l, p->T - 2, dpred, dseq, dh_ext, dc_given, st, 0, 0, p->T - 1)) return 1;
      } else {
        for (int t = p->T - 2; t >= 0; --t)
          if (bwd_step(p, l, t, dpred, dseq, dh_ext, dc_given, st, 0, 0)) return 1;
      }
    }
  } else
  for (int b0 = 0; b0 < p->B; b0 += SB) {
    const int nb = b0 + SB <= p->B ? SB : p->B - b0;
    for (int t = p->T - 1; t >= 0; --t)
      for (int l = p->L - 1; l >= 0; --l)
        if (bwd_step(p, l, t, dpred, dseq, dh_ext, dc_given, st, b0, SB < p->B ? nb : 0)) return 1;
  }
  p->gates_valid = false;
  p->bptt_done = true;
  return 0;
}

int nint_backward_bptt(nint_plan* p, const float* dpred, const float* dseq, float* grad_head_weight,
                       float* grad_head_bias, void* stream) {
  if (check_ready(p)) return 1;
  if (!p->cfg.training) return fail("nint_backward needs a training plan");
  if (!p->fwd_done) return fail("nint_backward before nint_forward");
  if (!p->gates_valid)
    return fail("nint_backward: the activations saved by the last forward were already consumed by a backward (BPTT "
                "turns the saved gates into their gradients in place); run the forward again");
  if (!dpred && !dseq) return fail("nint_backward: no upstream gradient");
  if (dseq && !p->cfg.return_sequence) return fail("dseq requires return_sequence in the plan");
  if (dseq && dpred) return fail("pass either dpred or dseq (fold dpred into dseq[:, T-1])");
  p->bptt_done = false;
  cudaStream_t st = static_cast<cudaStream_t>(stream);
  const long long HW = static_cast<long long>(p->H) * p->W;
  const int L = p->L, T = p->T;
  const Layer& top = p->layer[L - 1];
  if (grad_head_weight && grad_head_bias) {
    CK(cudaMemsetAsync(grad_head_weight, 0, top.hc_real * 4, st));
    CK(cudaMemsetAsync(grad_head_bias, 0, 4, st));
    if (dpred)
      LAUNCH(p, K_OTHER, st, launch_head_bwd(p->dtype, slot_ptr(p, top.Hs, T, top.hc_pad), dpred, HW, grad_head_weight, grad_head_bias, HW,
                         p->B, top.hc_real, top.hc_pad, p->head_part, st));
    if (dseq)
      for (int t = 0; t < T; ++t)
        LAUNCH(p, K_OTHER, st, launch_head_bwd(p->dtype, slot_ptr(p, top.Hs, t + 1, top.hc_pad), dseq + t * HW, T * HW, grad_head_weight,
                           grad_head_bias, HW, p->B, top.hc_real, top.hc_pad, p->head_part, st));
  }
  return bptt_loop(p, dpred, dseq, nullptr, false, st);
}

int nint_backward_wgrad(nint_plan* p, int l, float* grad_weight_l, float* grad_bias_l, void* stream) {
  if (check_ready(p)) return 1;
  if (!p->cfg.training) return fail("nint_backward_wgrad needs a training plan");
  if (!p->bptt_done) return fail("nint_backward_wgrad before nint_backward_bptt");
  if (l < 0 || l >= p->L) return fail("layer %d out of range", l);
  cudaStream_t st = static_cast<cudaStream_t>(stream);
  Layer& y = p->layer[l];
  const size_t slices = p->deterministic ? static_cast<size_t>(y.det_splits) : 1;
  CK(cudaMemsetAsync(y.dw_acc, 0, y.dw_acc_bytes * slices, st));
  CK(cudaMemsetAsync(y.db_acc, 0, 4 * y.hc * 4 * slices, st));
  const int bias_col = (l == 0) ? p->ones_lane : -1;
  for (size_t bi = 0; bi < y.wg_blocks.size(); ++bi) {
    WgradParams w;
    if (wgrad_params(p, l, bi, p->num_sms, w)) return 1;
    if (p->deterministic && wgrad_max_splits(w) > y.det_splits)
      return fail("deterministic wgrad: this device splits the reduction %d ways, the plan reserved %d slices", wgrad_max_splits(w), y.det_splits);
    LAUNCH(p, K_WGRAD, st, launch_wgrad(p->dtype, w, st));
  }
  if (grad_weight_l)
    LAUNCH(p, K_OTHER, st, launch_unpack_wgrad(y.dw_acc, y.db_acc, grad_weight_l, grad_bias_l, y.cin, y.hc_real, y.hc, y.k, y.ncols, y.cx_pad,
                                               bias_col, 0, p->deterministic ? y.det_splits : 0,
                                               resid_on(p) ? y.db_resid : nullptr, kResidCtas * 4, st));
  return 0;
}

int nint_backward(nint_plan* p, const float* dpred, const float* dseq, float* const* grad_weight,
                  float* const* grad_bias, float* grad_head_weight, float* grad_head_bias, void* stream) {
  if (!grad_weight || !grad_bias) return fail("nint_backward: null gradient tables");
  if (nint_backward_bptt(p, dpred, dseq, grad_head_weight, grad_head_bias, stream)) return 1;
  for (int l = 0; l < p->L; ++l)
    if (nint_backward_wgrad(p, l, grad_weight[l], grad_bias[l], stream)) return 1;
  return 0;
}

int nint_backward_input(nint_plan* p, float* dx, void* stream) {
  if (check_ready(p)) return 1;
  if (!p->cfg.training || !p->input_grad) return fail("nint_backward_input needs a training plan created with NINT_FLAG_INPUT_GRAD");
  if (!p->bptt_done) return fail("nint_backward_input before nint_backward_bptt");
  if (!dx) return fail("nint_backward_input: null dx");
  cudaStream_t st = static_cast<cudaStream_t>(stream);
  const Layer& y = p->layer[0];
  const long long HW = static_cast<long long>(p->H) * p->W;
  const int C = p->cfg.in_channels;
  for (int t = 0; t < p->T; ++t) {
    if (dgrad_raw(p, 0, t, 2, y.cin_rows, p->raw, st)) return 1;
    LAUNCH(p, K_OTHER, st, launch_unpack_raw(p->raw, dx + t * C * HW, p->B, C, p->H, p->W, y.cin_rows, static_cast<long long>(p->T) * C * HW, st));
  }
  return 0;
}

int nint_cell_forward(nint_plan* p, const float* x, const float* h, const float* c, float* h_out, float* c_out,
                      void* stream) {
  if (check_ready(p)) return 1;
  if (p->L != 1 || p->T != 1) return fail("nint_cell_forward needs a plan with one layer and seq_len 1");
  if (!x || !h || !c) return fail("nint_cell_forward: null argument");
  cudaStream_t st = static_cast<cudaStream_t>(stream);
  if (nint_plan_set_state(p, 0, h, c, stream)) return 1;
  p->x_bank = false;
  LAUNCH(p, K_OTHER, st, launch_pack_input(p->dtype, x, 0, p->X, p->B, 1, p->cfg.in_channels, p->H, p->W, p->layer[0].cx_pad, p->ones_lane, st));
  if (cell_step(p, 0, 0, EPI_FWD, nullptr, st)) return 1;
  const bool tr = p->cfg.training != 0;
  p->final_slot_h = tr ? 1 : 1;
  p->final_slot_c = tr ? 1 : 0;
  p->fwd_done = true;
  p->gates_valid = tr;
  p->bptt_done = false;
  return nint_plan_get_state(p, 0, h_out, c_out, stream);
}

int nint_cell_backward(nint_plan* p, const float* dh_out, const float* dc_out, float* dx, float* dh, float* dc,
                       float* grad_weight, float* grad_bias, void* stream) {
  if (check_ready(p)) return 1;
  if (p->L != 1 || p->T != 1 || !p->cfg.training || !p->input_grad)
    return fail("nint_cell_backward needs a one-layer, seq_len 1 training plan created with NINT_FLAG_INPUT_GRAD");
  if (!p->fwd_done || !p->gates_valid) return fail("nint_cell_backward: no forward to differentiate (or already consumed)");
  cudaStream_t st = static_cast<cudaStream_t>(stream);
  Layer& y = p->layer[0];
  const size_t npix = static_cast<size_t>(p->B) * p->H * p->W;
  if (dh_out) LAUNCH(p, K_OTHER, st, launch_nchw_to_nhwc_f32(dh_out, p->dh_ext, p->B, y.hc_real, p->H, p->W, y.hc, st));
  if (dc_out) {
    CK(cudaMemsetAsync(y.dC, 0, npix * y.hc * 4, st));
    LAUNCH(p, K_OTHER, st, launch_nchw_to_nhwc_f32(dc_out, y.dC, p->B, y.hc_real, p->H, p->W, y.hc, st));
  }
  if (bptt_loop(p, nullptr, nullptr, dh_out ? p->dh_ext : nullptr, dc_out != nullptr, st)) return 1;
  if (dc) LAUNCH(p, K_OTHER, st, launch_nhwc_to_nchw_f32(y.dC, dc, p->B, y.hc_real, p->H, p->W, y.hc, st));
  if (dh) {
    if (dgrad_raw(p, 0, 0, 3, y.hc, p->raw, st)) return 1;
    LAUNCH(p, K_OTHER, st, launch_unpack_raw(p->raw, dh, p->B, y.hc_real, p->H, p->W, y.hc, static_cast<long long>(y.hc_real) * p->H * p->W, st));
  }
  if (dx) {
    const int C = p->cfg.in_channels;
    if (dgrad_raw(p, 0, 0, 2, y.cin_rows, p->raw, st)) return 1;
    LAUNCH(p, K_OTHER, st, launch_unpack_raw(p->raw, dx, p->B, C, p->H, p->W, y.cin_rows, static_cast<long long>(C) * p->H * p->W, st));
  }
  if (grad_weight || grad_bias) {
    if (!grad_weight) return fail("nint_cell_backward: grad_bias without grad_weight");
    if (nint_backward_wgrad(p, 0, grad_weight, grad_bias, stream)) return 1;
  }
  return 0;
}

}
```

nasa_niswan_b200/csrc/nint_conv_halo.cu:

```cuda
#include "nint_epilogue.cuh"

namespace nint {

constexpr int kHaloCtrlBytes = 1024;
constexpr int kHaloMaxA = 12;
constexpr int kHaloMaxW = 28;
constexpr int kMaxAcc = 4;

__host__ __device__ inline int halo_rows(int ksize) { return (8 + (ksize & ~1)) * (16 + (ksize & ~1)); }
static inline int halo_a_buf_bytes(const ConvGemmParams& p) {
  int m = 0;
  for (int s = 0; s < p.nseg; ++s) {
    const int b = halo_rows(p.seg[s].ksize) * kChunkBytes;
    if (b > m) m = b;
  }
  return (m + 511) & ~511;
}

static int halo_operand_bytes(int a_buf_bytes, int na, int n_tile, int nw, int ts, int cluster) {
  return (na * a_buf_bytes + nw * ts * (n_tile / cluster) * kChunkBytes + 1023) & ~1023;
}
int conv_halo_smem_bytes(const ConvGemmParams& p) {
  return 1024 + halo_operand_bytes(p.a_buf_bytes, p.na_bufs, p.n_tile, p.num_stages, p.taps_per_stage, p.cluster) +
         p.e_stages * p.e_stage_bytes + p.c_ring * kEpiBoxBytes16 + kHaloCtrlBytes + (4 * p.hc + p.hc) * 4;
}

__device__ __forceinline__ int halo_operand_bytes_dev(int a_buf_bytes, int na, int stage_bytes, int nw) {
  return (na * a_buf_bytes + nw * stage_bytes + 1023) & ~1023;
}

template <typename E, int EPI, bool PAIR, bool FUSED>
__global__ void __launch_bounds__(kConvThreads, 1) conv_halo_kernel(const __grid_constant__ ConvGemmParams p) {
  constexpr int DT = ElemTraits<E>::kDtype;
  constexpr int CE = ElemTraits<E>::kPerChunk;
  extern __shared__ uint8_t smem_raw[];
  uint8_t* smem = reinterpret_cast<uint8_t*>((reinterpret_cast<uintptr_t>(smem_raw) + 1023) & ~uintptr_t(1023));
  const int warp = __shfl_sync(0xffffffffu, static_cast<int>(threadIdx.x >> 5), 0);
  const int lane = threadIdx.x & 31;
  constexpr int S = PAIR ? 2 : 1;
  constexpr bool pair = PAIR;
  const int NA = p.na_bufs, NW = p.num_stages, TS = p.taps_per_stage;
  const int w_rows = p.n_tile / S;
  const int w_bytes = w_rows * kChunkBytes;
  const int stage_bytes = TS * w_bytes;
  uint8_t* sA = smem;
  uint8_t* sW = sA + NA * p.a_buf_bytes;
  uint8_t* sE = smem + halo_operand_bytes_dev(p.a_buf_bytes, NA, stage_bytes, NW);
  uint8_t* ctrl = sE + p.e_stages * p.e_stage_bytes + p.c_ring * kEpiBoxBytes16;
  uint64_t* a_full = reinterpret_cast<uint64_t*>(ctrl);
  uint64_t* a_empty = a_full + kHaloMaxA;
  uint64_t* w_full = a_empty + kHaloMaxA;
  uint64_t* w_empty = w_full + kHaloMaxW;
  uint64_t* tfull_bar = w_empty + kHaloMaxW;
  uint64_t* tempty_bar = tfull_bar + kMaxAcc;
  uint64_t* e_full = tempty_bar + kMaxAcc;
  uint64_t* e_empty = e_full + kEpiMaxStages;
  uint64_t* st_ready = e_empty + kEpiMaxStages;
  uint64_t* hg_ready = st_ready + kEpiMaxStages;
  uint64_t* hg_empty = hg_ready + kEpiMaxStages;
  uint32_t* tmem_slot = reinterpret_cast<uint32_t*>(ctrl + kHaloCtrlBytes - 16);
  float* s_bias = reinterpret_cast<float*>(ctrl + kHaloCtrlBytes);
  float* s_headw = s_bias + 4 * p.hc;

  uint32_t crank = 0;
  if constexpr (pair) crank = __shfl_sync(0xffffffffu, cluster_ctarank(), 0);
  const bool lead_cta = crank == 0;
  const int G = p.group;
  const TileWalk walk = make_walk(p, S, static_cast<int>(crank));
  const bool resident = p.w_resident != 0;
  int chunks_per_tile = 0;
  bool all_k3 = true;
  for (int s = 0; s < p.nseg; ++s) {
    chunks_per_tile += p.seg[s].nchunks;
    all_k3 = all_k3 && p.seg[s].ksize == 3;
  }
  const bool dual = EPI == EPI_FWD && resident && G == 1 && all_k3 && TS == 9 && NA >= 4 && !(NINT_DBG(p) & 32);
  volatile uint32_t* mma_started = reinterpret_cast<volatile uint32_t*>(ctrl + kHaloCtrlBytes - 32);

  if (warp == 0 && lane == 0) {
    for (int s = 0; s < p.nseg; ++s) {
      prefetch_tensormap(&p.seg[s].tmap_act);
      prefetch_tensormap(&p.seg[s].tmap_w);
    }
  }
  if (warp == 3 && lane == 0 && EPI != EPI_RAW) {
    prefetch_tensormap(&p.tm_c);
    prefetch_tensormap(&p.tm_g);
    prefetch_tensormap(EPI == EPI_FWD ? &p.tm_h : &p.tm_dc);
  }
  if (warp == 1 && lane == 0) {
    for (int s = 0; s < NA; ++s) {
      mbar_init(&a_full[s], 1);
      mbar_init(&a_empty[s], 1);
    }
    for (int s = 0; s < NW; ++s) {
      mbar_init(&w_full[s], 1);
      mbar_init(&w_empty[s], 1);
    }
    *mma_started = 0;
    for (int s = 0; s < kMaxAcc; ++s) {
      mbar_init(&tfull_bar[s], (dual && chunks_per_tile >= 2) ? 2 : 1);
      mbar_init(&tempty_bar[s], 8 * S);
    }
    for (int s = 0; s < kEpiMaxStages; ++s) {
      mbar_init(&e_full[s], 1);
      mbar_init(&e_empty[s], 1);
      mbar_init(&st_ready[s], 8);
      mbar_init(&hg_ready[s], 8);
      mbar_init(&hg_empty[s], 1);
    }
    fence_barrier_init();
  }
  if (warp == 2) {
    if constexpr (pair) {
      tmem_alloc_pair(tmem_slot, kTmemCols);
    } else {
      tmem_alloc(tmem_slot, kTmemCols);
      tmem_relinquish();
    }
  }
  if (p.pdl) {
    asm volatile("griddepcontrol.launch_dependents;" ::: "memory");
    asm volatile("griddepcontrol.wait;" ::: "memory");
  }
  if (EPI == EPI_FWD) {
    for (int i = threadIdx.x; i < 4 * p.hc; i += kConvThreads) s_bias[i] = p.bias_q ? p.bias_q[i] : 0.f;
  }
  if (EPI == EPI_BWD) {
    for (int i = threadIdx.x; i < p.hc; i += kConvThreads) s_headw[i] = p.head_w ? p.head_w[i] : 0.f;
  }
  tc_fence_before();
  __syncthreads();
  if constexpr (pair) cluster_sync_all();
  tc_fence_after();
  const uint32_t tmem_base = __shfl_sync(0xffffffffu, *tmem_slot, 0);

  auto produce = [&](bool do_a, int a_par, int a_npar, bool do_w) {
    const bool by_tile = do_a && a_npar == 2 && G == 2;
    const bool leader = elect_one();
    Tracer tr(p, do_w ? 5 : 0, leader && (do_w || a_par == 0));
    int ia = 0, iw = 0, cc = 0, seen = -1;
    uint32_t pa = 0, pw = 0;
    bool first = true;
    StepCursor<FUSED> cur;
    for (int base = walk.first_tile; base < walk.tiles_padded; base += walk.tile_stride) {
      const GroupPos gp = cur.at(walk, base);
      const int g_begin = by_tile ? a_par : 0, g_end = by_tile ? a_par + 1 : G;
      ItemCoord c_first;
      c_first.b = c_first.x0 = c_first.y0 = 0;
      if (do_a) c_first = decode_tile(p, gp.tile0 + g_begin);
      if (FUSED && do_a && gp.step > 0) {
        ItemCoord cw = c_first;
        for (int g = g_begin; g < g_end; ++g, next_tile(p, cw))
          if (gp.tile0 + g < walk.num_tiles) wait_prev_step_warp<FUSED>(p, gp.step, cw.b, seen);
      }
      for (int s = 0; s < p.nseg; ++s) {
        const ConvSegment& sg = p.seg[s];
        const int seg_slot = step_slot<FUSED>(p, sg.slot, p.d_seg[s], s, gp.step);
        const int pad = sg.ksize >> 1;
        const int taps = sg.ksize * sg.ksize;
        const uint32_t a_bytes = static_cast<uint32_t>(halo_rows(sg.ksize) * kChunkBytes);
        int wtap = (walk.nb * sg.nchunks) * taps;
        for (int ch = 0; ch < sg.nchunks; ++ch, ++cc, wtap += taps) {
          if (do_a && (a_npar == 1 || by_tile || (cc & 1) == a_par)) {
            tr.stamp();
            mbar_wait(&a_empty[ia], pa ^ 1);
            tr.stamp();
            if (leader) {
              if (lead_cta && (!by_tile || a_par == 0)) mbar_arrive_expect_tx(&a_full[ia], a_bytes * G * S);
              uint32_t bar = 0;
              if constexpr (pair) bar = mapa_rank(smem_u32(&a_full[ia]), 0);
              ItemCoord cg = c_first;
              for (int g = g_begin; g < g_end; ++g, next_tile(p, cg)) {
                uint8_t* dst = sA + ia * p.a_buf_bytes + g * p.a_halo_bytes;
                int img = cg.b, slot = seg_slot;
                if (sg.win_start) {
                  img = (gp.tile0 + g < walk.num_tiles) ? __ldg(sg.win_start + cg.b) + seg_slot : sg.bank_frames;
                  slot = 0;
                }
                if constexpr (pair)
                  tma_load_5d_pair(dst, &sg.tmap_act, bar, ch * CE, cg.x0 - pad, cg.y0 - pad, img, slot);
                else
                  tma_load_5d(dst, &sg.tmap_act, &a_full[ia], ch * CE, cg.x0 - pad, cg.y0 - pad, img, slot);
              }
            }
            tr.stamp();
          }
          if (++ia == NA) {
            ia = 0;
            pa ^= 1;
          }
          if (!do_w || (resident && !first)) continue;
          for (int tap0 = 0; tap0 < taps; tap0 += sg.ts) {
            if (!resident) mbar_wait(&w_empty[iw], pw ^ 1);
            if (leader) {
              if (lead_cta) mbar_arrive_expect_tx(&w_full[iw], static_cast<uint32_t>(sg.ts * w_bytes * S));
              uint8_t* dst = sW + iw * stage_bytes;
              if constexpr (pair)
                tma_load_3d_pair(dst, &sg.tmap_w, mapa_rank(smem_u32(&w_full[iw]), 0), 0, static_cast<int>(crank) * w_rows, wtap + tap0);
              else
                tma_load_3d(dst, &sg.tmap_w, &w_full[iw], 0, 0, wtap + tap0);
            }
            if (++iw == NW) {
              iw = 0;
              pw ^= 1;
            }
          }
        }
      }
      first = false;
    }
  };
  auto issue_dual = [&](int which) {
    const bool leader = elect_one();
    Tracer tr(p, 1, leader && which == 0);
    const bool issue_any = !(NINT_DBG(p) & 2);
    const int n_acc = p.n_acc, acc_cols = p.acc_cols, a_buf_bytes = p.a_buf_bytes;
    const uint32_t idesc = p.idesc;
    const uint32_t w16l = static_cast<uint32_t>(w_bytes >> 4);
    const uint32_t sA_addr = smem_u32(sA), sW_addr = smem_u32(sW);
    const int ntiles = (walk.tiles_padded - walk.first_tile + walk.tile_stride - 1) / walk.tile_stride;
    const int cpt = chunks_per_tile;
    const int total = walk.first_tile < walk.tiles_padded ? ntiles * cpt : 0;
    const uint64_t adesc0 = make_smem_desc_sw64(0, 16, 10 * kChunkBytes);
    const uint64_t bdesc0 = make_smem_desc_sw64(0, 16, 512);
    const uint32_t ahi = static_cast<uint32_t>(adesc0 >> 32), bhi = static_cast<uint32_t>(bdesc0 >> 32);
    int k = which / cpt, j = which % cpt, ia = which % NA, abuf = k % n_acc;
    uint32_t pa = static_cast<uint32_t>(which / NA) & 1u, aphase = static_cast<uint32_t>(k / n_acc) & 1u;
    for (int c = which; c < total; c += 2) {
      tr.stamp();
      if (j == 0) mbar_wait(&tempty_bar[abuf], aphase ^ 1);
      mbar_wait(&a_full[ia], pa);
      if (k == 0) mbar_wait(&w_full[j], 0);
      spin_until_at_least(mma_started, static_cast<uint32_t>(c));
      tc_fence_after();
      tr.stamp();
      const uint32_t d_tmem = tmem_base + static_cast<uint32_t>(abuf * acc_cols);
      if (leader && issue_any) {
        const uint32_t alo = static_cast<uint32_t>(adesc0) + ((sA_addr + ia * a_buf_bytes) >> 4);
        const uint32_t blo = static_cast<uint32_t>(bdesc0) + ((sW_addr + j * stage_bytes) >> 4);
#pragma unroll 1
        for (int dy = 0; dy < 3; ++dy) {
          const uint32_t ar = alo + static_cast<uint32_t>(dy * 10 * (kChunkBytes >> 4));
          const uint32_t br = blo + static_cast<uint32_t>(dy * 3) * w16l;
#pragma unroll
          for (int dxc = 0; dxc < 3; ++dxc) {
            const uint32_t acc = (j | dy | dxc) == 0 ? 0u : 1u;
            umma_lohi<DT, pair>(d_tmem, ar + 4 * dxc, ahi, br + dxc * w16l, bhi, idesc, acc);
            umma_lohi<DT, pair>(d_tmem, ar + 4 * dxc + 2, ahi, br + dxc * w16l + 2, bhi, idesc, 1u);
          }
        }
      }
      if (leader) {
        __threadfence_block();
        *mma_started = static_cast<uint32_t>(c + 1);
      }
      __syncwarp();
      umma_commit_elect<pair>(&a_empty[ia]);
      if (j + 2 >= cpt) umma_commit_elect<pair>(&tfull_bar[abuf]);
      tr.stamp();
      j += 2;
      while (j >= cpt) {
        j -= cpt;
        ++k;
        if (++abuf == n_acc) {
          abuf = 0;
          aphase ^= 1;
        }
      }
      ia += 2;
      if (ia >= NA) {
        ia -= NA;
        pa ^= 1;
      }
    }
  };

  const bool a_split = (EPI != EPI_RAW);

  if (warp == 0) {
    if (p.nseg > 0) produce(true, 0, a_split ? 2 : 1, false);
  } else if (warp == 7) {
    if (p.nseg > 0 && a_split) produce(true, 1, 2, false);
  } else if (warp == 6) {
    if (p.nseg > 0) produce(false, 0, 1, true);
  } else if (warp == 1) {
    if (p.nseg > 0 && lead_cta && dual) {
      issue_dual(0);
    } else if (p.nseg > 0 && lead_cta) {
      const bool leader = elect_one();
      Tracer tr(p, 1, leader);
      const bool issue_any = !(NINT_DBG(p) & 2);
      const int n_acc = p.n_acc, acc_cols = p.acc_cols, nseg = p.nseg, a_buf_bytes = p.a_buf_bytes;
      const uint32_t idesc = p.idesc;
      const uint32_t n_tile = static_cast<uint32_t>(p.n_tile);
      const uint64_t a_halo16 = static_cast<uint64_t>(p.a_halo_bytes >> 4);
      const uint64_t w16 = static_cast<uint64_t>(w_bytes >> 4);
      const uint32_t sA_addr = smem_u32(sA), sW_addr = smem_u32(sW);
      int cbase = walk.first_tile, cs = 0, cch = 0;
      bool valid = cbase < walk.tiles_padded;
      int ia = 0, iw = 0;
      uint32_t pa = 0, pw = 0;
      int abuf = 0;
      uint32_t aphase = 0;
      bool first = true;
      const bool lookahead = NA >= 3;
      bool single_stage = true;
      for (int s = 0; s < nseg; ++s) single_stage = single_stage && (p.seg[s].ts == p.seg[s].ksize * p.seg[s].ksize);
      const bool w_ahead = lookahead && !resident && NW >= 3 && single_stage;
      bool cur_ready = false;
      int step_hi = walk.tiles_step;
      if (valid && lookahead) {
        mbar_wait(&tempty_bar[abuf], aphase ^ 1);
        mbar_wait(&a_full[ia], pa);
        if (w_ahead) mbar_wait(&w_full[0], 0);
        tc_fence_after();
        cur_ready = true;
      }
      while (valid) {
        int nbase = cbase, ns = cs, nch = cch + 1;
        if (nch == p.seg[cs].nchunks) {
          nch = 0;
          if (++ns == nseg) {
            ns = 0;
            nbase += walk.tile_stride;
          }
        }
        const bool nvalid = nbase < walk.tiles_padded;
        const bool last_of_tile = nbase != cbase;
        const int nia = (ia + 1 == NA) ? 0 : ia + 1;
        const uint32_t npa = (ia + 1 == NA) ? pa ^ 1 : pa;
        int nabuf = abuf;
        uint32_t naphase = aphase;
        if (last_of_tile && ++nabuf == n_acc) {
          nabuf = 0;
          naphase ^= 1;
        }
        const bool fast = lookahead && issue_any && p.seg[cs].ksize == 3 && p.seg[cs].ts == 9 && G == 2 && (resident || w_ahead);
        bool cross = false;
        if constexpr (FUSED) {
          if (last_of_tile) {
            while (cbase >= step_hi) step_hi += walk.tiles_step;
            cross = nvalid && (nbase >= step_hi || (NINT_DBG(p) & 4096));
          }
        }
        const bool look = lookahead && !cross;
        tr.stamp();
        if (!cur_ready) {
          if ((cs | cch) == 0) mbar_wait(&tempty_bar[abuf], aphase ^ 1);
          mbar_wait(&a_full[ia], pa);
          if (w_ahead) mbar_wait(&w_full[iw], pw);
          tc_fence_after();
        }
        if (look && !fast && nvalid) {
          if (last_of_tile) mbar_wait(&tempty_bar[nabuf], naphase ^ 1);
          mbar_wait(&a_full[nia], npa);
          if (w_ahead) {
            const int niw = (iw + 1 == NW) ? 0 : iw + 1;
            mbar_wait(&w_full[niw], (iw + 1 == NW) ? pw ^ 1 : pw);
          }
          tc_fence_after();
        }
        cur_ready = look && nvalid;
        tr.stamp();
        const int ks = p.seg[cs].ksize;
        const int hw = 8 + (ks & ~1);
        const uint32_t sbo = static_cast<uint32_t>(hw * kChunkBytes);
        const int taps = ks * ks;
        const uint64_t row_skip = static_cast<uint64_t>((hw - ks) * (kChunkBytes >> 4));
        const uint32_t d_tmem = tmem_base + static_cast<uint32_t>(abuf * acc_cols);
        uint32_t accumulate = (cs | cch) != 0 ? 1u : 0u;
        if (resident && (cs | cch) == 0) iw = 0;
        uint64_t adesc = make_smem_desc_sw64(sA_addr + ia * a_buf_bytes, 16, sbo);
        int dx = 0;
        if (fast) {
          if (resident && first) {
            mbar_wait(&w_full[iw], pw);
            tc_fence_after();
          }
          const uint64_t bdesc = make_smem_desc_sw64(sW_addr + iw * stage_bytes, 16, 512);
          const uint32_t alo = static_cast<uint32_t>(adesc), blo = static_cast<uint32_t>(bdesc);
          const uint32_t ahi = static_cast<uint32_t>(adesc >> 32), bhi = static_cast<uint32_t>(bdesc >> 32);
          const uint32_t w16l = static_cast<uint32_t>(w16);
          const uint32_t halo16l = static_cast<uint32_t>(a_halo16);
          const uint32_t d1 = d_tmem + n_tile;
          auto issue_row = [&](int dy) {
            if (leader) {
              const uint32_t ar = alo + static_cast<uint32_t>(dy * 10 * (kChunkBytes >> 4));
              const uint32_t br = blo + static_cast<uint32_t>(dy * 3) * w16l;
              if (G == 1) {
#pragma unroll
// ... 364 lines not shown
```

nasa_niswan_b200/csrc/nint_epilogue.cuh:

```cuda
#pragma once
#include "nint_common.cuh"
#include "nint_kernels.h"
#include "nint_pair.cuh"

namespace nint {

constexpr int kConvIoWarps = 8;
constexpr int kConvThreads = 512;
constexpr int kEpiMaxStages = 4;
constexpr int kEpiBoxBytes16 = kTilePixels * 16 * 4;

static __device__ unsigned long long* g_fail_host = nullptr;

constexpr int kTraceRoles = 8, kTraceLen = 1024;
__device__ long long g_trace[kTraceRoles * kTraceLen];
struct Tracer {
  long long* dst;
  int n;
  __device__ __forceinline__ Tracer(const ConvGemmParams& p, int role, bool on) {
    dst = (on && (NINT_DBG(p) & 8) && blockIdx.x == 0) ? g_trace + role * kTraceLen : nullptr;
    n = 0;
  }
  __device__ __forceinline__ void stamp() {
    if (dst && n < kTraceLen) dst[n++] = clock64();
  }
};

struct ItemCoord {
  int b, x0, y0;
};
__device__ __forceinline__ ItemCoord decode_tile(const ConvGemmParams& p, int tile) {
  ItemCoord c;
  const int tx = tile % p.tiles_x;
  int r = tile / p.tiles_x;
  const int ty = r % p.tiles_y;
  c.b = p.b0 + r / p.tiles_y;
  c.x0 = tx * p.tile_w;
  c.y0 = ty * p.tile_h;
  return c;
}

__device__ __forceinline__ void next_tile(const ConvGemmParams& p, ItemCoord& c) {
  c.x0 += p.tile_w;
  if (c.x0 >= p.tiles_x * p.tile_w) {
    c.x0 = 0;
    c.y0 += p.tile_h;
    if (c.y0 >= p.tiles_y * p.tile_h) {
      c.y0 = 0;
      ++c.b;
    }
  }
}

struct TileWalk {
  int nb, first_tile, tile_stride, tiles_padded, num_tiles;
  int tiles_step;
};
__device__ __forceinline__ TileWalk make_walk(const ConvGemmParams& p, int S, int crank) {
  TileWalk w;
  const int G = p.group;
  w.num_tiles = p.B * p.tiles_x * p.tiles_y;
  const int groups = (w.num_tiles + S * G - 1) / (S * G);
  const int cpn = static_cast<int>(gridDim.x) / (S * p.n_blocks);
  const int cid = static_cast<int>(blockIdx.x) / S;
  w.nb = cid % p.n_blocks;
  w.first_tile = ((cid / p.n_blocks) * S + crank) * G;
  w.tile_stride = cpn * S * G;
  w.tiles_step = groups * S * G;
  w.tiles_padded = w.tiles_step * p.n_steps;
  return w;
}

struct GroupPos {
  int step, tile0;
};
template <bool FUSED>
struct StepCursor {
  int step, lo;
  __device__ __forceinline__ StepCursor() : step(0), lo(0) {}
  __device__ __forceinline__ GroupPos at(const TileWalk& w, int base) {
    GroupPos g;
    if constexpr (FUSED) {
      while (base >= lo + w.tiles_step) {
        ++step;
        lo += w.tiles_step;
      }
      g.step = step;
      g.tile0 = base - lo;
    } else {
      g.step = 0;
      g.tile0 = base;
    }
    return g;
  }
  __device__ __forceinline__ bool last_in_step(const TileWalk& w, int base) const {
    if constexpr (!FUSED) return false;
    const int nb = base + w.tile_stride;
    return nb >= w.tiles_padded || nb >= lo + w.tiles_step;
  }
};
template <bool FUSED>
__device__ __forceinline__ int step_slot(const ConvGemmParams& p, int slot, int d, int ring_bit, int step) {
  if constexpr (!FUSED) return slot;
  if (slot < 0) return slot;
  const int v = slot + d * step;
  return (p.ring_bits >> ring_bit) & 1 ? (v & 1) : v;
}
__device__ __forceinline__ void wait_prev_step(const ConvGemmParams& p, int step, int b) {
  if (step == 0) return;
  const unsigned* ctr = p.step_done + static_cast<long long>(step - 1) * p.B + (b - p.b0);
  unsigned v;
  long long t0 = 0;
  unsigned spins = 0;
  const bool diag = (NINT_DBG(p) & 2048) != 0;
  for (;;) {
    asm volatile("ld.acquire.gpu.global.u32 %0, [%1];" : "=r"(v) : "l"(ctr) : "memory");
    if (v >= p.step_target) break;
    if (spins == 0) t0 = clock64();
    if ((++spins & 0x3ff) == 0 &&
        (clock64() - t0 > (diag ? 200000000LL : 4000000000LL) ||
         (diag && *reinterpret_cast<volatile long long*>(g_trace + (kTraceRoles - 1) * kTraceLen) != 0))) {
      if (!diag) {
        unsigned long long* h = g_fail_host;
        if (h && (threadIdx.x & 31) == 0) {
          h[1] = blockIdx.x;
          h[2] = threadIdx.x;
          h[3] = (static_cast<unsigned long long>(step) << 32) | static_cast<unsigned>(b);
          h[4] = v;
          h[0] = 3;
          __threadfence_system();
        }
        __syncwarp();
        __trap();
      }
      if ((threadIdx.x & 31) != 0) break;
      long long* row = g_trace + (kTraceRoles - 1) * kTraceLen;
      const unsigned long long i = atomicAdd(reinterpret_cast<unsigned long long*>(row), 1ULL);
      if (i < 200) {
        row[1 + 5 * i] = blockIdx.x;
        row[2 + 5 * i] = threadIdx.x >> 5;
        row[3 + 5 * i] = step;
        row[4 + 5 * i] = b;
        row[5 + 5 * i] = v;
      }
      break;
    }
  }
}
template <bool FUSED>
__device__ __forceinline__ void wait_prev_step_warp(const ConvGemmParams& p, int step, int b, int& seen) {
  if constexpr (!FUSED) return;
  if (step == 0) return;
  const int key = step * p.B + (b - p.b0);
  if (key == seen) return;
  seen = key;
  wait_prev_step(p, step, b);
}
template <bool FUSED>
struct TileSignal {
  int step, b;
  __device__ __forceinline__ TileSignal() : step(0), b(-1) {}
  __device__ __forceinline__ void count(const ConvGemmParams& p) {
    unsigned* ctr = p.step_done + static_cast<long long>(step) * p.B + (b - p.b0);
    asm volatile("red.relaxed.gpu.global.add.u32 [%0], 1;" ::"l"(ctr) : "memory");
    b = -1;
  }
  __device__ __forceinline__ void tile_done(const ConvGemmParams& p, int step_, int b_, int newest) {
    if constexpr (!FUSED) return;
    if (b >= 0) {
      if (newest <= 0) asm volatile("cp.async.bulk.wait_group 0;" ::: "memory");
      else if (newest == 1) asm volatile("cp.async.bulk.wait_group 1;" ::: "memory");
      else if (newest == 2) asm volatile("cp.async.bulk.wait_group 2;" ::: "memory");
      else if (newest == 3) asm volatile("cp.async.bulk.wait_group 3;" ::: "memory");
      else asm volatile("cp.async.bulk.wait_group 4;" ::: "memory");
      count(p);
    }
    step = step_;
    b = b_;
  }
  __device__ __forceinline__ void flush(const ConvGemmParams& p) {
    if constexpr (!FUSED) return;
    if (b < 0) return;
    asm volatile("cp.async.bulk.wait_group 0;" ::: "memory");
    count(p);
  }
};

template <int ROWB>
__device__ __forceinline__ uint32_t swz(uint32_t base, int row, int chunk) {
  const uint32_t off = static_cast<uint32_t>(row * ROWB + chunk * 16);
  constexpr uint32_t mask = ROWB / 16 - 1;
  return base + (off ^ (((off >> 7) & mask) << 4));
}
__device__ __forceinline__ void sts128(uint32_t saddr, const float* v) {
  asm volatile("st.shared.v4.f32 [%0], {%1,%2,%3,%4};" ::"r"(saddr), "f"(v[0]), "f"(v[1]), "f"(v[2]), "f"(v[3]) : "memory");
}
__device__ __forceinline__ void lds128u(uint32_t saddr, uint32_t* v) {
  asm volatile("ld.shared.v4.b32 {%0,%1,%2,%3}, [%4];" : "=r"(v[0]), "=r"(v[1]), "=r"(v[2]), "=r"(v[3]) : "r"(saddr));
}
__device__ __forceinline__ void sts128u(uint32_t saddr, const uint32_t* v) {
  asm volatile("st.shared.v4.b32 [%0], {%1,%2,%3,%4};" ::"r"(saddr), "r"(v[0]), "r"(v[1]), "r"(v[2]), "r"(v[3]) : "memory");
}
__device__ __forceinline__ void tmem_ld8(uint32_t taddr, float* v) {
  uint32_t* r = reinterpret_cast<uint32_t*>(v);
  asm volatile("tcgen05.ld.sync.aligned.32x32b.x8.b32 {%0,%1,%2,%3,%4,%5,%6,%7}, [%8];"
               : "=r"(r[0]), "=r"(r[1]), "=r"(r[2]), "=r"(r[3]), "=r"(r[4]), "=r"(r[5]), "=r"(r[6]), "=r"(r[7])
               : "r"(taddr)
               : "memory");
}
__device__ __forceinline__ void tma_store_5d(const CUtensorMap* map, const void* smem_src, int c0, int c1, int c2,
                                             int c3, int c4) {
  asm volatile("cp.async.bulk.tensor.5d.global.shared::cta.tile.bulk_group [%0, {%2, %3, %4, %5, %6}], [%1];" ::"l"(
                   reinterpret_cast<uint64_t>(map)),
               "r"(smem_u32(smem_src)), "r"(c0), "r"(c1), "r"(c2), "r"(c3), "r"(c4)
               : "memory");
}
__device__ __forceinline__ void tma_store_commit() { asm volatile("cp.async.bulk.commit_group;" ::: "memory"); }
__device__ __forceinline__ void tma_store_wait_read() { asm volatile("cp.async.bulk.wait_group.read 0;" ::: "memory"); }
__device__ __forceinline__ void tma_store_wait_all() { asm volatile("cp.async.bulk.wait_group 0;" ::: "memory"); }

template <typename E, int ROWB>
__device__ __forceinline__ void lds8(uint32_t base, int row, int ec, float* v) {
  if constexpr (sizeof(E) == 2) {
    uint32_t u[4];
    lds128u(swz<ROWB>(base, row, ec), u);
#pragma unroll
    for (int j = 0; j < 4; ++j) unpack_bf16x2(u[j], v[2 * j], v[2 * j + 1]);
  } else {
    lds128(swz<ROWB>(base, row, 2 * ec), v);
    lds128(swz<ROWB>(base, row, 2 * ec + 1), v + 4);
  }
}
template <typename E, int ROWB>
__device__ __forceinline__ void sts8(uint32_t base, int row, int ec, const float* v) {
  if constexpr (sizeof(E) == 2) {
    uint32_t u[4];
#pragma unroll
    for (int j = 0; j < 4; ++j) u[j] = pack_bf16x2(v[2 * j], v[2 * j + 1]);
    sts128u(swz<ROWB>(base, row, ec), u);
  } else {
    sts128(swz<ROWB>(base, row, 2 * ec), v);
    sts128(swz<ROWB>(base, row, 2 * ec + 1), v + 4);
  }
}

template <typename E>
struct EpiGeom {
  static constexpr int kGateBoxes = (64 * sizeof(E)) / 128;
  static constexpr int kGateBoxCols = 128 / sizeof(E);
  static constexpr int kGateBoxBytes = kTilePixels * 128;
  static constexpr int kGateBytes = kGateBoxes * kGateBoxBytes;
  static constexpr int kHRowB = 16 * sizeof(E);
  static constexpr int kHBytes = kTilePixels * kHRowB;
};

template <typename E>
__device__ __forceinline__ void lds_gate(uint32_t st, int row, int g, int half, float* v) {
  if constexpr (sizeof(E) == 2) lds8<E, 128>(st, row, g * 2 + half, v);
  else lds8<E, 128>(st + (g >> 1) * EpiGeom<E>::kGateBoxBytes, row, (g & 1) * 2 + half, v);
}
template <typename E>
__device__ __forceinline__ void sts_gate(uint32_t st, int row, int g, int half, const float* v) {
  if constexpr (sizeof(E) == 2) sts8<E, 128>(st, row, g * 2 + half, v);
  else sts8<E, 128>(st + (g >> 1) * EpiGeom<E>::kGateBoxBytes, row, (g & 1) * 2 + half, v);
}

__device__ __forceinline__ int group_q0(int ch) { return (ch >> 4) * 64; }

template <int EPI>
__device__ __forceinline__ int epi_groups(const ConvGemmParams& p) {
  return (EPI == EPI_FWD ? p.hcb : p.hc) >> 4;
}

struct FwdEpiBars {
  uint64_t *c_full, *c_empty, *c_ready, *hg_ready, *hg_empty;
};
__device__ __forceinline__ uint8_t* fwd_c_slot(const ConvGemmParams& p, uint8_t* sE, int s) { return sE + s * kEpiBoxBytes16; }
__device__ __forceinline__ uint8_t* fwd_hg_stage(const ConvGemmParams& p, uint8_t* sE, int s) {
  return sE + p.c_ring * kEpiBoxBytes16 + s * p.e_stage_bytes;
}

template <typename E, bool FUSED>
__device__ __forceinline__ void fwd_c_loader(const ConvGemmParams& p, uint8_t* sE, const FwdEpiBars& b, const TileWalk& w) {
  const bool leader = elect_one();
  Tracer tr(p, 2, leader);
  const int G = p.group, ngroups = p.hcb >> 4;
  int s = 0, seen = -1;
  uint32_t ph = 0;
  StepCursor<FUSED> cur;
  for (int base = w.first_tile; base < w.tiles_padded; base += w.tile_stride) {
    const GroupPos gp = cur.at(w, base);
    const int slot_c_in = step_slot<FUSED>(p, p.slot_c_in, p.d_c_in, 2, gp.step);
    for (int gi = 0; gi < G; ++gi) {
      const int tile = gp.tile0 + gi;
      if (tile >= w.num_tiles) break;
      const ItemCoord c = decode_tile(p, tile);
      wait_prev_step_warp<FUSED>(p, gp.step, c.b, seen);
      for (int grp = 0; grp < ngroups; ++grp) {
        tr.stamp();
        mbar_wait(&b.c_empty[s], ph ^ 1);
        tr.stamp();
        if (leader) {
          if (p.slot_c_in >= 0) {
            mbar_arrive_expect_tx(&b.c_full[s], kEpiBoxBytes16);
            tma_load_5d(fwd_c_slot(p, sE, s), &p.tm_c, &b.c_full[s], w.nb * p.hcb + grp * 16, c.x0, c.y0, c.b, slot_c_in);
          } else {
            mbar_arrive(&b.c_full[s]);
          }
        }
        tr.stamp();
        if (++s == p.c_ring) {
          s = 0;
          ph ^= 1;
        }
      }
    }
  }
}

template <typename E, bool FUSED>
__device__ __forceinline__ void fwd_storer(const ConvGemmParams& p, uint8_t* sE, const FwdEpiBars& b, const TileWalk& w, int kind) {
  using GE = EpiGeom<E>;
  const bool leader = elect_one();
  Tracer tr(p, 3, leader && kind == 1);
  const int G = p.group, ngroups = p.hcb >> 4;
  const int ring = kind == 0 ? p.c_ring : p.e_stages;
  uint64_t* ready = kind == 0 ? b.c_ready : b.hg_ready;
  uint64_t* empty = kind == 0 ? b.c_empty : b.hg_empty;
  int s = 0;
  uint32_t ph = 0;
  TileSignal<FUSED> sig;
  StepCursor<FUSED> cur;
  for (int base = w.first_tile; base < w.tiles_padded; base += w.tile_stride) {
    const GroupPos gp = cur.at(w, base);
    const int slot_c_out = step_slot<FUSED>(p, p.slot_c_out, p.d_c_out, 3, gp.step);
    const int slot_h_out = step_slot<FUSED>(p, p.slot_h_out, p.d_h_out, 4, gp.step);
    const int slot_g = step_slot<FUSED>(p, p.slot_g, p.d_g, 31, gp.step);
    for (int gi = 0; gi < G; ++gi) {
      const int tile = gp.tile0 + gi;
      if (tile >= w.num_tiles) break;
      const ItemCoord c = decode_tile(p, tile);
      for (int grp = 0; grp < ngroups; ++grp) {
        tr.stamp();
        mbar_wait(&ready[s], ph);
        tr.stamp();
        if (leader) {
          if (!(NINT_DBG(p) & 1)) {
            const int ch = w.nb * p.hcb + grp * 16;
            if (kind == 0) {
              tma_store_5d(&p.tm_c, fwd_c_slot(p, sE, s), ch, c.x0, c.y0, c.b, slot_c_out);
            } else {
              const uint8_t* st = fwd_hg_stage(p, sE, s);
              tma_store_5d(&p.tm_h, st + p.e_off_h, ch, c.x0, c.y0, c.b, slot_h_out);
              if (p.slot_g >= 0) {
                const int q0 = group_q0(ch);
#pragma unroll
                for (int bx = 0; bx < GE::kGateBoxes; ++bx)
                  tma_store_5d(&p.tm_g, st + bx * GE::kGateBoxBytes, q0 + bx * GE::kGateBoxCols, c.x0, c.y0, c.b, slot_g);
              }
            }
            tma_store_commit();
            tma_store_wait_read();
          }
          mbar_arrive(&empty[s]);
        }
        tr.stamp();
        if (++s == ring) {
          s = 0;
          ph ^= 1;
        }
      }
      if (leader) sig.tile_done(p, gp.step, c.b, (NINT_DBG(p) & 1) ? 0 : ngroups);
    }
    if (leader && cur.last_in_step(w, base)) sig.flush(p);
  }
  if (leader) tma_store_wait_all();
}

template <typename E, bool FUSED>
__device__ __forceinline__ void fwd_math(const ConvGemmParams& p, int warp, int lane, uint32_t tmem_base, uint8_t* sE,
                                         const FwdEpiBars& b, uint64_t* tfull_bar, uint64_t* tempty_bar,
                                         const float* s_bias, const TileWalk& w, uint32_t tempty_remote) {
  using GE = EpiGeom<E>;
  constexpr int DT = ElemTraits<E>::kDtype;
  constexpr bool FAST = (DT == NINT_BF16);
  const int G = p.group, ngroups = p.hcb >> 4;
  const int quad = warp & 3;
  const int half = (warp - kConvIoWarps) >> 2;
  const int row = quad * 32 + lane;
  const bool skip = (NINT_DBG(p) & 1) != 0;
  Tracer tr(p, 4, warp == kConvIoWarps && lane == 0);
  int cs = 0, hs = 0;
  uint32_t cph = 0, hph = 0;
  int abuf = 0;
  uint32_t aphase = 0;
  StepCursor<FUSED> cur;
  for (int base = w.first_tile; base < w.tiles_padded; base += w.tile_stride) {
    bool waited = false;
    const GroupPos gp = cur.at(w, base);
    for (int gi = 0; gi < G; ++gi) {
      const int tile = gp.tile0 + gi;
      if (tile >= w.num_tiles) break;
      const uint32_t taddr = tmem_base + (static_cast<uint32_t>(quad * 32) << 16) +
                             static_cast<uint32_t>(abuf * p.acc_cols + gi * p.n_tile);
      for (int grp = 0; grp < ngroups; ++grp) {
        const uint32_t cslot = smem_u32(fwd_c_slot(p, sE, cs));
        const uint32_t st = smem_u32(fwd_hg_stage(p, sE, hs));
        tr.stamp();
        mbar_wait(&b.c_full[cs], cph);
        mbar_wait(&b.hg_empty[hs], hph ^ 1);
        tr.stamp();
        if (!waited) {
          mbar_wait(&tfull_bar[abuf], aphase);
          tc_fence_after();
          waited = true;
        }
        tr.stamp();
        float a[4][8], cn[8], hn[8];
#pragma unroll
        for (int g = 0; g < 4; ++g) tmem_ld8(taddr + grp * 64 + g * 16 + half * 8, a[g]);
        if (p.slot_c_in >= 0 && !skip) {
          lds8<float, 64>(cslot, row, half, cn);
        } else {
#pragma unroll
          for (int j = 0; j < 8; ++j) cn[j] = 0.f;
        }
        const uint32_t bq = smem_u32(s_bias + w.nb * p.n_tile + grp * 64 + half * 8);
        tmem_ld_wait();
        if (!skip) {
          if (p.bias_q) {
#pragma unroll
            for (int g = 0; g < 4; ++g) {
              float bias[8];
              lds128(bq + g * 64, bias);
              lds128(bq + g * 64 + 16, bias + 4);
#pragma unroll
              for (int j = 0; j < 8; ++j) a[g][j] += bias[j];
            }
          }
#pragma unroll
          for (int j = 0; j < 8; ++j) {
            const float gi_ = act_sigmoid_halved<FAST>(a[0][j]);
            const float gf = act_sigmoid_halved<FAST>(a[1][j]);
            const float gg = act_tanh<FAST>(a[2][j]);
            const float go = act_sigmoid_halved<FAST>(a[3][j]);
            const float cv = fmaf(cn[j], gf, gi_ * gg);
            cn[j] = cv;
            float hv = go * act_tanh<FAST>(cv);
            if constexpr (DT == NINT_TF32) hv = round_tf32(hv);
            hn[j] = hv;
            a[0][j] = gi_; a[1][j] = gf; a[2][j] = gg; a[3][j] = go;
          }
          sts8<float, 64>(cslot, row, half, cn);
          sts8<E, GE::kHRowB>(st + p.e_off_h, row, half, hn);
          if (p.slot_g >= 0) {
#pragma unroll
            for (int g = 0; g < 4; ++g) sts_gate<E>(st, row, g, half, a[g]);
          }
        }
        fence_proxy_async_smem();
        __syncwarp();
        if (lane == 0) {
          mbar_arrive(&b.c_ready[cs]);
          mbar_arrive(&b.hg_ready[hs]);
        }
        tr.stamp();
        if (++cs == p.c_ring) {
          cs = 0;
          cph ^= 1;
        }
        if (++hs == p.e_stages) {
          hs = 0;
          hph ^= 1;
        }
      }
    }
    if (!waited) {
      mbar_wait(&tfull_bar[abuf], aphase);
      tc_fence_after();
    }
    tc_fence_before();
    __syncwarp();
    if (lane == 0) {
      if (tempty_remote) mbar_arrive_cluster(tempty_remote + abuf * 8); else mbar_arrive(&tempty_bar[abuf]);
    }
    if (++abuf == p.n_acc) {
      abuf = 0;
      aphase ^= 1;
    }
  }
}

template <typename E, int EPI, bool FUSED>
__device__ __forceinline__ void epi_loader(const ConvGemmParams& p, uint8_t* sE, uint64_t* e_full, uint64_t* e_empty,
                                           const TileWalk& w, int which, int nwhich) {
  using GE = EpiGeom<E>;
  const bool leader = elect_one();
  Tracer tr(p, 2, leader && which == 0);
  const int G = p.group;
  const int ngroups = epi_groups<EPI>(p);
  int s = 0, n = 0, seen = -1;
  uint32_t ph = 0;
  StepCursor<FUSED> cur;
  for (int base = w.first_tile; base < w.tiles_padded; base += w.tile_stride) {
    const GroupPos gp = cur.at(w, base);
    const int slot_g = step_slot<FUSED>(p, p.slot_g, p.d_g, 31, gp.step);
    const int slot_c_prev = (FUSED && gp.step == p.c_prev_none_step) ? -1 : step_slot<FUSED>(p, p.slot_c_prev, p.d_c_prev, 31, gp.step);
    for (int gi = 0; gi < G; ++gi) {
      const int tile = gp.tile0 + gi;
      if (tile >= w.num_tiles) break;
      const ItemCoord c = decode_tile(p, tile);
      wait_prev_step_warp<FUSED>(p, gp.step, c.b, seen);
      for (int grp = 0; grp < ngroups; ++grp, ++n) {
        const bool mine = (nwhich == 1) || ((n % nwhich) == which);
        if (mine) tr.stamp();
        if (mine) mbar_wait(&e_empty[s], ph ^ 1);
        if (mine) tr.stamp();
        if (mine && leader) {
          uint8_t* st = sE + s * p.e_stage_bytes;
          uint64_t* bar = &e_full[s];
          const uint32_t bytes = GE::kGateBytes + kEpiBoxBytes16 * ((slot_c_prev >= 0) + (p.has_dc_in != 0));
          mbar_arrive_expect_tx(bar, bytes);
          const int q0 = group_q0(grp * 16);
#pragma unroll
          for (int bx = 0; bx < GE::kGateBoxes; ++bx)
            tma_load_5d(st + bx * GE::kGateBoxBytes, &p.tm_g, bar, q0 + bx * GE::kGateBoxCols, c.x0, c.y0, c.b, slot_g);
          if (slot_c_prev >= 0)
            tma_load_5d(st + p.e_off_c2, &p.tm_c, bar, grp * 16, c.x0, c.y0, c.b, slot_c_prev);
          if (p.has_dc_in) tma_load_5d(st + p.e_off_dc, &p.tm_dc, bar, grp * 16, c.x0, c.y0, c.b, 0);
        }
        if (mine) tr.stamp();
        if (++s == p.e_stages) {
          s = 0;
          ph ^= 1;
        }
      }
    }
  }
}

template <typename E, int EPI, bool FUSED>
__device__ __forceinline__ void epi_storer(const ConvGemmParams& p, uint8_t* sE, uint64_t* st_ready, uint64_t* e_empty,
                                           const TileWalk& w, int which, int nwhich) {
  using GE = EpiGeom<E>;
  const bool leader = elect_one();
  Tracer tr(p, 3, leader && which == 0);
  const int G = p.group;
  const int ngroups = epi_groups<EPI>(p);
  int s = 0, n = 0;
  uint32_t ph = 0;
  TileSignal<FUSED> sig;
  StepCursor<FUSED> cur;
  for (int base = w.first_tile; base < w.tiles_padded; base += w.tile_stride) {
    const GroupPos gp = cur.at(w, base);
    const int slot_g = step_slot<FUSED>(p, p.slot_g, p.d_g, 31, gp.step);
    for (int gi = 0; gi < G; ++gi) {
      const int tile = gp.tile0 + gi;
      if (tile >= w.num_tiles) break;
      const ItemCoord c = decode_tile(p, tile);
      int committed = 0;
      for (int grp = 0; grp < ngroups; ++grp, ++n) {
        const bool mine = (nwhich == 1) || ((n % nwhich) == which);
        if (mine && !(NINT_DBG(p) & 1)) ++committed;
        if (mine) tr.stamp();
        if (mine) mbar_wait(&st_ready[s], ph);
        if (mine) tr.stamp();
        if (mine && leader) {
          const uint8_t* st = sE + s * p.e_stage_bytes;
          if (!(NINT_DBG(p) & 1)) {
            const int q0 = group_q0(grp * 16);
#pragma unroll
            for (int bx = 0; bx < GE::kGateBoxes; ++bx)
              tma_store_5d(&p.tm_g, st + bx * GE::kGateBoxBytes, q0 + bx * GE::kGateBoxCols, c.x0, c.y0, c.b, slot_g);
            tma_store_5d(&p.tm_dc, st + p.e_off_dc, grp * 16, c.x0, c.y0, c.b, 0);
            tma_store_commit();
            tma_store_wait_read();
          }
          mbar_arrive(&e_empty[s]);
        }
        if (mine) tr.stamp();
        if (++s == p.e_stages) {
          s = 0;
          ph ^= 1;
        }
      }
      if (leader) sig.tile_done(p, gp.step, c.b, committed);
    }
    if (leader && cur.last_in_step(w, base)) sig.flush(p);
  }
  if (leader) tma_store_wait_all();
}

template <typename E, int EPI, bool FUSED>
__device__ __forceinline__ void epi_math(const ConvGemmParams& p, int warp, int lane, uint32_t tmem_base, uint8_t* sE,
                                         uint64_t* e_full, uint64_t* st_ready, uint64_t* tfull_bar, uint64_t* tempty_bar,
                                         const float* s_bias, const float* s_headw, const TileWalk& w,
                                         uint32_t tempty_remote) {
  using GE = EpiGeom<E>;
  constexpr int DT = ElemTraits<E>::kDtype;
  constexpr bool FAST = (DT == NINT_BF16);
  const int G = p.group;
  const int ngroups = epi_groups<EPI>(p);
  const int quad = warp & 3;
  const int half = (warp - kConvIoWarps) >> 2;
  const int row = quad * 32 + lane;
  const bool skip = (NINT_DBG(p) & 1) != 0;
  Tracer tr(p, 4, warp == kConvIoWarps && lane == 0);
  int s = 0;
  uint32_t ph = 0;
  int abuf = 0;
  uint32_t aphase = 0;
  StepCursor<FUSED> cur;
  for (int base = w.first_tile; base < w.tiles_padded; base += w.tile_stride) {
    bool waited = (p.nseg == 0);
    const GroupPos gp = cur.at(w, base);
    const bool have_c_prev = p.slot_c_prev >= 0 && !(FUSED && gp.step == p.c_prev_none_step);
    for (int gi = 0; gi < G; ++gi) {
      const int tile = gp.tile0 + gi;
      if (tile >= w.num_tiles) break;
      const ItemCoord c = decode_tile(p, tile);
      const uint32_t taddr = tmem_base + (static_cast<uint32_t>(quad * 32) << 16) +
                             static_cast<uint32_t>(abuf * p.acc_cols + gi * p.n_tile);
      float dpred = 0.f;
      if constexpr (EPI == EPI_BWD) {
        if (p.head_dpred) {
          const int y = c.y0 + (row >> 3), x = c.x0 + (row & 7);
          if (y < p.H && x < p.W)
            dpred = p.head_dpred[(FUSED ? gp.step * p.head_dpred_sstride : 0) + c.b * p.head_dpred_bstride + static_cast<long long>(y) * p.W + x];
        }
      }
      for (int grp = 0; grp < ngroups; ++grp) {
        const uint32_t st = smem_u32(sE + s * p.e_stage_bytes);
        tr.stamp();
        mbar_wait(&e_full[s], ph);
        tr.stamp();
        if (!waited) {
          mbar_wait(&tfull_bar[abuf], aphase);
          tc_fence_after();
          waited = true;
        }
        tr.stamp();
        {
        float gi_[8], gf[8], gg[8], go[8], cp[8], dc[8], dh[8];
        const int c0 = grp * 16 + half * 8;
        if (p.nseg > 0) {
          tmem_ld8(taddr + c0, dh);
        } else {
#pragma unroll
          for (int j = 0; j < 8; ++j) dh[j] = 0.f;
        }
        if (!skip) {
          lds_gate<E>(st, row, 0, half, gi_);
          lds_gate<E>(st, row, 1, half, gf);
          lds_gate<E>(st, row, 2, half, gg);
          lds_gate<E>(st, row, 3, half, go);
          if (have_c_prev) {
            lds8<float, 64>(st + p.e_off_c2, row, half, cp);
          } else {
#pragma unroll
            for (int j = 0; j < 8; ++j) cp[j] = 0.f;
          }
          if (p.has_dc_in) {
            lds8<float, 64>(st + p.e_off_dc, row, half, dc);
          } else {
#pragma unroll
            for (int j = 0; j < 8; ++j) dc[j] = 0.f;
          }
        }
        float hw[8];
        if (p.head_dpred) {
          lds128(smem_u32(s_headw + c0), hw);
          lds128(smem_u32(s_headw + c0 + 4), hw + 4);
        } else {
#pragma unroll
          for (int j = 0; j < 8; ++j) hw[j] = 0.f;
        }
        if (p.nseg > 0) tmem_ld_wait();
        if (p.dh_ext) {
          const int y = c.y0 + (row >> 3), x = c.x0 + (row & 7);
          if (y < p.H && x < p.W) {
            float e[8];
            load_elems<float, 8>(p.dh_ext + ((static_cast<long long>(c.b) * p.H + y) * p.W + x) * p.hc + c0, e);
#pragma unroll
            for (int j = 0; j < 8; ++j) dh[j] += e[j];
          }
        }
        if (!skip) {
#pragma unroll
          for (int j = 0; j < 8; ++j) {
            const float dhv = fmaf(dpred, hw[j], dh[j]);
            const float tc = act_tanh<FAST>(fmaf(cp[j], gf[j], gi_[j] * gg[j]));
            const float d_o = dhv * tc;
            const float dcv = fmaf(dhv * go[j], 1.f - tc * tc, dc[j]);
            const float d_i = dcv * gg[j];
            const float d_g = dcv * gi_[j];
            const float d_f = dcv * cp[j];
            dc[j] = dcv * gf[j];
            const float i_ = gi_[j], f_ = gf[j], g_ = gg[j], o_ = go[j];
            gi_[j] = d_i * fmaf(-i_, i_, i_);
            gf[j] = d_f * fmaf(-f_, f_, f_);
            gg[j] = d_g * fmaf(-g_, g_, 1.f);
            go[j] = d_o * fmaf(-o_, o_, o_);
          }
          if constexpr (DT == NINT_TF32) {
            float res[32];
#pragma unroll
            for (int j = 0; j < 8; ++j) {
              float r;
              r = round_tf32(gi_[j]); res[j] = gi_[j] - r; gi_[j] = r;
              r = round_tf32(gf[j]); res[8 + j] = gf[j] - r; gf[j] = r;
              r = round_tf32(gg[j]); res[16 + j] = gg[j] - r; gg[j] = r;
              r = round_tf32(go[j]); res[24 + j] = go[j] - r; go[j] = r;
            }
            if (p.db_resid) {
#pragma unroll
              for (int st_ = 16; st_ >= 1; st_ >>= 1) {
                const bool upper = (lane & st_) != 0;
#pragma unroll
                for (int i = 0; i < st_; ++i) {
                  const float send = upper ? res[i] : res[i + st_];
                  const float keep = upper ? res[i + st_] : res[i];
                  res[i] = keep + __shfl_xor_sync(0xffffffffu, send, st_);
                }
              }
              float* slot = p.db_resid + (static_cast<long long>(blockIdx.x) * 4 + quad) * (4 * p.hc);
              slot[grp * 64 + (lane >> 3) * 16 + half * 8 + (lane & 7)] += res[0];
            }
          }
          sts8<float, 64>(st + p.e_off_dc, row, half, dc);
          sts_gate<E>(st, row, 0, half, gi_);
          sts_gate<E>(st, row, 1, half, gf);
          sts_gate<E>(st, row, 2, half, gg);
          sts_gate<E>(st, row, 3, half, go);
        }
      
        }
        fence_proxy_async_smem();
        __syncwarp();
        if (lane == 0) mbar_arrive(&st_ready[s]);
        tr.stamp();
        if (++s == p.e_stages) {
          s = 0;
          ph ^= 1;
        }
      }
    }
    if (p.nseg > 0) {
      if (!waited) {
        mbar_wait(&tfull_bar[abuf], aphase);
        tc_fence_after();
      }
      tc_fence_before();
      __syncwarp();
      if (lane == 0) {
        if (tempty_remote) mbar_arrive_cluster(tempty_remote + abuf * 8); else mbar_arrive(&tempty_bar[abuf]);
      }
      if (++abuf == p.n_acc) {
        abuf = 0;
        aphase ^= 1;
      }
    }
  }
}

__device__ __forceinline__ void epi_raw(const ConvGemmParams& p, int warp, int lane, uint32_t tmem_base,
                                        uint64_t* tfull_bar, uint64_t* tempty_bar, const TileWalk& w,
                                        uint32_t tempty_remote) {
  const int G = p.group;
  const int quad = warp & 3;
  const int half = (warp - kConvIoWarps) >> 2;
  const int row = quad * 32 + lane;
  int abuf = 0;
  uint32_t aphase = 0;
  for (int base = w.first_tile; base < w.tiles_padded; base += w.tile_stride) {
    mbar_wait(&tfull_bar[abuf], aphase);
    tc_fence_after();
    for (int gi = 0; gi < G; ++gi) {
      const int tile = base + gi;
      if (tile >= w.num_tiles) break;
      const ItemCoord c = decode_tile(p, tile);
      const int y = c.y0 + (row >> 3), x = c.x0 + (row & 7);
      const bool valid = y < p.H && x < p.W;
      const long long pix = (static_cast<long long>(c.b) * p.H + y) * p.W + x;
      const uint32_t taddr = tmem_base + (static_cast<uint32_t>(quad * 32) << 16) +
                             static_cast<uint32_t>(abuf * p.acc_cols + gi * p.n_tile);
      float* ro = p.raw_out + pix * (p.n_blocks * p.n_tile) + w.nb * p.n_tile;
      for (int c0 = half * 16; c0 < p.n_tile; c0 += 32) {
        float v[16];
        tmem_ld16(taddr + c0, v);
        tmem_ld_wait();
        if (valid) store_elems<float, 16>(ro + c0, v);
      }
    }
    tc_fence_before();
    __syncwarp();
    if (lane == 0) {
      if (tempty_remote) mbar_arrive_cluster(tempty_remote + abuf * 8); else mbar_arrive(&tempty_bar[abuf]);
    }
    if (++abuf == p.n_acc) {
      abuf = 0;
      aphase ^= 1;
    }
  }
}

}
```

nasa_niswan_b200/csrc/nint_kernels.h:

```cpp
#pragma once
#include <cuda.h>
#include <cuda_runtime.h>
#include <stdint.h>

#ifndef NINT_KNOBS
#define NINT_KNOBS 0
#endif
#define NINT_DBG(p) (NINT_KNOBS ? (p).debug_flags : 0)

namespace nint {

enum : int { EPI_FWD = 0, EPI_BWD = 1, EPI_RAW = 2 };

struct alignas(64) ConvSegment {
  CUtensorMap tmap_act;
  CUtensorMap tmap_w;
  int slot;
  int ksize;
  int nchunks;
  int wsel;
  int ts;
  const int* win_start;
  int bank_frames;
};

struct alignas(64) ConvGemmParams {
  ConvSegment seg[2];
  int nseg;
  int B, H, W;
  int b0;
  int tile_w, tile_h;
  int tiles_x, tiles_y;
  int n_tile;
  int n_blocks;
  int num_stages;
  int na_bufs, a_buf_bytes, cluster, taps_per_stage;
  int group, a_halo_bytes;
  int acc_cols, n_acc;
  int plan_g, plan_ns;
  int w_resident;
  int debug_flags;
  int pdl;
  CUtensorMap tm_c, tm_h, tm_g, tm_dc;
  int slot_c_in, slot_c_out, slot_h_out, slot_g;
  int slot_c_prev, has_dc_in;
  int e_stages, e_stage_bytes, e_off_c, e_off_c2, e_off_dc, e_off_h;
  int c_ring;
  uint32_t idesc;
  int hc, hc_pad;
  int hcb;
  const float* bias_q;
  const float* head_dpred;
  long long head_dpred_bstride;
  const float* head_w;
  float* db_resid;
  const float* dh_ext;
  float* raw_out;
  int n_steps;
  int d_seg[2], d_c_in, d_c_out, d_h_out, d_g, d_c_prev;
  int ring_bits;
  int c_prev_none_step;
  long long head_dpred_sstride;
  unsigned* step_done;
  unsigned step_target;
};

int conv_halo_plan(int epi, int dtype, ConvGemmParams& p);
int conv_halo_smem_bytes(const ConvGemmParams& p);
cudaError_t launch_conv_halo(int epi, int dtype, const ConvGemmParams& p, int num_sms, cudaStream_t stream);
cudaError_t read_trace(long long* host, int n);
cudaError_t fail_record(unsigned long long* out5);
cudaError_t clear_trace();

constexpr int kMaxWgradGroups = 32;
struct alignas(64) WgradParams {
  CUtensorMap tmap_dg;
  CUtensorMap tmap_b[2];
  int slot_b0[2];
  int nchunks_b[2];
  int T, B, H, W;
  int tile_w, tile_h, tiles_x, tiles_y;
  int ksize;
  int m_blocks;
  int n_groups;
  int group_tap0[kMaxWgradGroups + 1];
  int bias_group;
  int group_splits[kMaxWgradGroups];
  int group_unit0[kMaxWgradGroups + 1];
  int ncols;
  int acc_cols;
  int col0;
  int real_cols;
  int chan0[2];
  int a_bufs, b_stages;
  int halo;
  int b_panel_bytes;
  int debug_flags;
  int pair;
  int b_pw;
  uint32_t idesc, idesc_bias;
  int hc4;
  const int* win_start;
  float* dw_part;
  float* db_part;
  float* dw_acc;
  float* db_acc;
};
int wgrad_b_panel_bytes(int dtype, int halo, int ksize);
int wgrad_smem_bytes(int dtype, int bpanels, int a_bufs, int b_stages, int b_panel_bytes);
void wgrad_pick_buffers(int dtype, int bpanels, int b_panel_bytes, int* a_bufs, int* b_stages);
int wgrad_pair_supported(int dtype, int hc4, int cx_pad, int ncols, int ksize);
int wgrad_pair_panel_width(int cx_pad, int ncols);
int wgrad_pair_b_stages(int cx_pad, int ncols, int ksize);
int wgrad_pair_b_stages_tf32(int n_mma, int ksize);
cudaError_t launch_wgrad(int dtype, const WgradParams& p, cudaStream_t stream);

cudaError_t launch_pack_input(int dtype, const void* x, int x_bf16, void* X, int B, int T, int C, int H, int W, int c_pad,
                              int ones_lane, cudaStream_t s);
cudaError_t launch_pack_frames(int dtype, const void* src, int src_bf16, void* bank, long long N, int C, int H, int W,
                               int c_pad, int ones_lane, cudaStream_t s);
cudaError_t launch_pack_state(int dtype, const float* src_nchw, void* dst_nhwc, int B, int C, int H, int W,
                              int c_pad, cudaStream_t s);
cudaError_t launch_unpack_state(int dtype, const void* src_nhwc, float* dst_nchw, int B, int C, int H, int W,
                                int c_pad, cudaStream_t s);
cudaError_t launch_nchw_to_nhwc_f32(const float* src, float* dst, int B, int C, int H, int W, int c_pad, cudaStream_t s);
cudaError_t launch_nhwc_to_nchw_f32(const float* src, float* dst, int B, int C, int H, int W, int c_pad, cudaStream_t s);
cudaError_t launch_pack_weights_fwd(int dtype, const float* w, const float* bias, void* wpack_x, void* wpack_h,
                                    float* bias_q, int cin, int hc_real, int hc, int hcb, int k, int cx_pad, int hc_pad,
                                    int bias_lane, cudaStream_t s);
cudaError_t launch_pack_weights_bwd(int dtype, const float* w, void* wpack_dx, void* wpack_dh, int cin, int cin_rows,
                                    int hc_real, int hc, int k, cudaStream_t s);
cudaError_t launch_head_fwd(int dtype, const void* h, const float* w, const float* b, float* out, long long npix_per_img,
                            int B, int hc, int hc_pad, long long out_bstride, cudaStream_t s);
int head_bwd_blocks(int B);
cudaError_t launch_head_bwd(int dtype, const void* h, const float* dpred, long long dpred_bstride, float* dw, float* db,
                            long long npix_per_img, int B, int hc, int hc_pad, float* part, cudaStream_t s);
cudaError_t launch_unpack_wgrad(const float* dw_acc, const float* db_acc, float* gw, float* gb, int cin, int hc_real,
                                int hc, int k, int ncols, int cx_pad, int bias_col, int accumulate, int nparts,
                                const float* db_resid, int resid_slots, cudaStream_t s);
cudaError_t launch_unpack_raw(const float* raw, float* dst, int B, int C, int H, int W, int ncols, long long dst_bstride,
                              cudaStream_t s);

cudaError_t launch_fuse_inputs(const float* lev, const float* emis, const float* mean, const float* stdv,
                               const float* statics, int S, float* out, long long N, int L, int H, int W, int Hp, int Wp,
                               int mode, cudaStream_t s);
cudaError_t launch_fuse_inputs_bank(int dtype, const float* lev, const float* emis, const float* mean, const float* stdv,
                                    const float* statics, int S, void* out, long long N, int L, int H, int W, int Hp, int Wp,
                                    int mode, int c_pad, int ones_lane, cudaStream_t s);
cudaError_t launch_loss_mse_l1(const float* pred, const float* y, float* dpred, float* stats, float* loss, int B, int H,
                               int W, int y0, int y1, int x0, int x1, const int* y_index, int y_offset, long long y_frames,
                               cudaStream_t s);
cudaError_t launch_adam(float* p, const float* g, float* m, float* v, long long n, float lr, float beta1, float beta2,
                        float eps, int step, float grad_scale, cudaStream_t s);
cudaError_t launch_adam_dev(float* p, const float* g, float* m, float* v, long long n, float* state, float beta1,
                            float beta2, float eps, float grad_scale, cudaStream_t s);

cudaError_t launch_dp_allreduce_adam(const void* const* peer_bases, long long slot_offset_bytes, long long flags_offset_bytes,
                                     int rank, int world, unsigned seq, float* params, float* m, float* v, long long n,
                                     float* state, float beta1, float beta2, float eps, float grad_scale, cudaStream_t s);

__host__ __device__ inline int q_to_n(int q, int hc) { return ((q >> 4) & 3) * hc + (q >> 6) * 16 + (q & 15); }

}
```

nasa_niswan_b200/csrc/nint_pointwise.cu:

```cuda
#include <type_traits>

#include "nint_common.cuh"
#include "nint_kernels.h"

namespace nint {

__device__ __forceinline__ float round_for(float v, __nv_bfloat16*) { return v; }
__device__ __forceinline__ float round_for(float v, float*) {
  uint32_t r;
  asm("cvt.rna.tf32.f32 %0, %1;" : "=r"(r) : "f"(v));
  return __uint_as_float(r);
}
template <typename E>
__device__ __forceinline__ E to_elem(float v);
template <>
__device__ __forceinline__ __nv_bfloat16 to_elem<__nv_bfloat16>(float v) { return __float2bfloat16_rn(v); }
template <>
__device__ __forceinline__ float to_elem<float>(float v) { return round_for(v, (float*)nullptr); }
__device__ __forceinline__ float from_elem(__nv_bfloat16 v) { return __bfloat162float(v); }
__device__ __forceinline__ float from_elem(float v) { return v; }

__device__ __forceinline__ float ldg_f(const float* p) { return __ldg(p); }
__device__ __forceinline__ float ldg_f(const __nv_bfloat16* p) {
  return __uint_as_float(static_cast<uint32_t>(__ldg(reinterpret_cast<const unsigned short*>(p))) << 16);
}
template <typename S> struct RawOf;
template <> struct RawOf<float> { using type = float; };
template <> struct RawOf<__nv_bfloat16> { using type = unsigned short; };
__device__ __forceinline__ float ldg_raw(const float* p) { return __ldg(p); }
__device__ __forceinline__ unsigned short ldg_raw(const __nv_bfloat16* p) { return __ldg(reinterpret_cast<const unsigned short*>(p)); }
__device__ __forceinline__ float raw_to_f(float v) { return v; }
__device__ __forceinline__ float raw_to_f(unsigned short v) { return __uint_as_float(static_cast<uint32_t>(v) << 16); }

template <typename S, typename E, int CP>
__global__ void pack_cl_kernel(const S* __restrict__ src, E* __restrict__ dst, int C, long long HW,
                               int n_outer, int n_inner, long long src_outer_stride, long long src_inner_stride,
                               long long dst_outer_stride, long long dst_inner_stride, int ones_lane) {
  const long long total = static_cast<long long>(n_outer) * n_inner * HW;
  for (long long idx = blockIdx.x * static_cast<long long>(blockDim.x) + threadIdx.x; idx < total;
       idx += static_cast<long long>(gridDim.x) * blockDim.x) {
    const long long pix = idx % HW;
    const long long img = idx / HW;
    const int i = static_cast<int>(img % n_inner);
    const int o = static_cast<int>(img / n_inner);
    const S* s = src + o * src_outer_stride + i * src_inner_stride + pix;
    E* d = dst + o * dst_outer_stride + i * dst_inner_stride + pix * CP;
    typename RawOf<S>::type raw[CP];
#pragma unroll
    for (int c = 0; c < CP; ++c) {
      if constexpr (sizeof(S) == 2) raw[c] = ldg_raw(s + (c < C ? c : C - 1) * HW);
      else raw[c] = (c < C) ? ldg_raw(s + c * HW) : typename RawOf<S>::type(0);
    }
    float v[CP];
#pragma unroll
    for (int c = 0; c < CP; ++c) v[c] = (c < C) ? round_for(raw_to_f(raw[c]), (E*)nullptr) : (c == ones_lane ? 1.f : 0.f);
    store_elems<E, CP>(d, v);
  }
}

template <typename S, typename E>
static cudaError_t pack_cl(const S* src, E* dst, int C, int c_pad, long long HW, int n_outer, int n_inner,
                           long long so, long long si, long long dso, long long dsi, int ones_lane, cudaStream_t s) {
  const long long total = static_cast<long long>(n_outer) * n_inner * HW;
  const int threads = 256;
  long long blocks = (total + threads - 1) / threads;
  if (blocks > 148 * 16) blocks = 148 * 16;
  if (blocks <= 0) return cudaSuccess;
  switch (c_pad) {
    case 16: pack_cl_kernel<S, E, 16><<<blocks, threads, 0, s>>>(src, dst, C, HW, n_outer, n_inner, so, si, dso, dsi, ones_lane); break;
    case 32: pack_cl_kernel<S, E, 32><<<blocks, threads, 0, s>>>(src, dst, C, HW, n_outer, n_inner, so, si, dso, dsi, ones_lane); break;
    case 48: pack_cl_kernel<S, E, 48><<<blocks, threads, 0, s>>>(src, dst, C, HW, n_outer, n_inner, so, si, dso, dsi, ones_lane); break;
    case 64: pack_cl_kernel<S, E, 64><<<blocks, threads, 0, s>>>(src, dst, C, HW, n_outer, n_inner, so, si, dso, dsi, ones_lane); break;
    default: return cudaErrorInvalidValue;
  }
  return cudaGetLastError();
}

template <typename S, typename E>
__global__ void pack_cl_wide_kernel(const S* __restrict__ src, E* __restrict__ dst, int C, int c_pad,
                                    long long HW, int n_outer, int n_inner, long long so, long long si,
                                    long long dso, long long dsi, int ones_lane) {
  const int groups = c_pad / 16;
  const long long total = static_cast<long long>(n_outer) * n_inner * groups * HW;
  for (long long idx = blockIdx.x * static_cast<long long>(blockDim.x) + threadIdx.x; idx < total;
       idx += static_cast<long long>(gridDim.x) * blockDim.x) {
    const long long pix = idx % HW;
    long long r = idx / HW;
    const int g = static_cast<int>(r % groups);
    r /= groups;
    const int i = static_cast<int>(r % n_inner);
    const int o = static_cast<int>(r / n_inner);
    const S* s = src + o * so + i * si + pix;
    E* d = dst + o * dso + i * dsi + pix * c_pad + g * 16;
    float v[16];
#pragma unroll
    for (int c = 0; c < 16; ++c) {
      const int ch = g * 16 + c;
      v[c] = (ch < C) ? round_for(ldg_f(s + ch * HW), (E*)nullptr) : (ch == ones_lane ? 1.f : 0.f);
    }
    store_elems<E, 16>(d, v);
  }
}

template <typename S, typename E>
static cudaError_t pack_any(const S* src, E* dst, int C, int c_pad, long long HW, int n_outer, int n_inner,
                            long long so, long long si, long long dso, long long dsi, cudaStream_t s, int ones_lane = -1) {
  if (c_pad % 16) return cudaErrorInvalidValue;
  if (c_pad <= 64) return pack_cl<S, E>(src, dst, C, c_pad, HW, n_outer, n_inner, so, si, dso, dsi, ones_lane, s);
  const long long total = static_cast<long long>(n_outer) * n_inner * (c_pad / 16) * HW;
  long long blocks = (total + 255) / 256;
  if (blocks > 148 * 16) blocks = 148 * 16;
  if (blocks <= 0) return cudaSuccess;
  pack_cl_wide_kernel<S, E><<<blocks, 256, 0, s>>>(src, dst, C, c_pad, HW, n_outer, n_inner, so, si, dso, dsi, ones_lane);
  return cudaGetLastError();
}

template <typename S>
static cudaError_t pack_dispatch(int dtype, const S* src, void* dst, int C, int c_pad, long long HW, int n_outer, int n_inner,
                                 long long so, long long si, long long dso, long long dsi, int ones_lane, cudaStream_t s) {
  if (dtype == NINT_BF16)
    return pack_any<S, __nv_bfloat16>(src, reinterpret_cast<__nv_bfloat16*>(dst), C, c_pad, HW, n_outer, n_inner, so, si, dso, dsi, s, ones_lane);
  return pack_any<S, float>(src, reinterpret_cast<float*>(dst), C, c_pad, HW, n_outer, n_inner, so, si, dso, dsi, s, ones_lane);
}

cudaError_t launch_pack_input(int dtype, const void* x, int x_bf16, void* X, int B, int T, int C, int H, int W, int c_pad,
                              int ones_lane, cudaStream_t s) {
  const long long HW = static_cast<long long>(H) * W;
  const long long so = static_cast<long long>(T) * C * HW, si = C * HW;
  const long long dso = HW * c_pad, dsi = static_cast<long long>(B) * HW * c_pad;
  if (x_bf16) return pack_dispatch(dtype, reinterpret_cast<const __nv_bfloat16*>(x), X, C, c_pad, HW, B, T, so, si, dso, dsi, ones_lane, s);
  return pack_dispatch(dtype, reinterpret_cast<const float*>(x), X, C, c_pad, HW, B, T, so, si, dso, dsi, ones_lane, s);
}

cudaError_t launch_pack_frames(int dtype, const void* src, int src_bf16, void* bank, long long N, int C, int H, int W,
                               int c_pad, int ones_lane, cudaStream_t s) {
  const long long HW = static_cast<long long>(H) * W;
  if (N > 0x7fffffffLL) return cudaErrorInvalidValue;
  if (src_bf16) return pack_dispatch(dtype, reinterpret_cast<const __nv_bfloat16*>(src), bank, C, c_pad, HW, static_cast<int>(N), 1, C * HW, 0, HW * c_pad, 0, ones_lane, s);
  return pack_dispatch(dtype, reinterpret_cast<const float*>(src), bank, C, c_pad, HW, static_cast<int>(N), 1, C * HW, 0, HW * c_pad, 0, ones_lane, s);
}

cudaError_t launch_pack_state(int dtype, const float* src, void* dst, int B, int C, int H, int W, int c_pad,
                              cudaStream_t s) {
  const long long HW = static_cast<long long>(H) * W;
  return pack_dispatch(dtype, src, dst, C, c_pad, HW, B, 1, C * HW, 0, HW * c_pad, 0, -1, s);
}

template <typename E>
__global__ void unpack_cl_kernel(const E* __restrict__ src, float* __restrict__ dst, int C, int c_pad, long long HW,
                                 long long dst_bstride) {
  __shared__ float tile[32][33];
  const int b = blockIdx.z;
  const long long p0 = static_cast<long long>(blockIdx.x) * 32;
  const int c0 = blockIdx.y * 32;
  const E* s = src + static_cast<long long>(b) * HW * c_pad;
  float* d = dst + static_cast<long long>(b) * dst_bstride;
  for (int r = threadIdx.y; r < 32; r += blockDim.y) {
    const long long p = p0 + r;
    const int c = c0 + threadIdx.x;
    tile[r][threadIdx.x] = (p < HW && c < C) ? from_elem(s[p * c_pad + c]) : 0.f;
  }
  __syncthreads();
  for (int r = threadIdx.y; r < 32; r += blockDim.y) {
    const int c = c0 + r;
    const long long p = p0 + threadIdx.x;
    if (c < C && p < HW) d[c * HW + p] = tile[threadIdx.x][r];
  }
}

cudaError_t launch_unpack_state(int dtype, const void* src, float* dst, int B, int C, int H, int W, int c_pad,
                                cudaStream_t s) {
  const long long HW = static_cast<long long>(H) * W;
  dim3 grid(static_cast<unsigned>((HW + 31) / 32), (C + 31) / 32, B), block(32, 8);
  if (dtype == NINT_BF16)
    unpack_cl_kernel<__nv_bfloat16><<<grid, block, 0, s>>>(reinterpret_cast<const __nv_bfloat16*>(src), dst, C, c_pad, HW, C * HW);
  else
    unpack_cl_kernel<float><<<grid, block, 0, s>>>(reinterpret_cast<const float*>(src), dst, C, c_pad, HW, C * HW);
  return cudaGetLastError();
}
cudaError_t launch_unpack_raw(const float* raw, float* dst, int B, int C, int H, int W, int ncols, long long dst_bstride,
                              cudaStream_t s) {
  const long long HW = static_cast<long long>(H) * W;
  dim3 grid(static_cast<unsigned>((HW + 31) / 32), (C + 31) / 32, B), block(32, 8);
  unpack_cl_kernel<float><<<grid, block, 0, s>>>(raw, dst, C, ncols, HW, dst_bstride);
  return cudaGetLastError();
}

__global__ void nchw_to_nhwc_f32_kernel(const float* __restrict__ src, float* __restrict__ dst, int C, int c_pad, long long HW) {
  __shared__ float tile[32][33];
  const int b = blockIdx.z;
  const long long p0 = static_cast<long long>(blockIdx.x) * 32;
  const int c0 = blockIdx.y * 32;
  const float* s = src + static_cast<long long>(b) * C * HW;
  float* d = dst + static_cast<long long>(b) * c_pad * HW;
  for (int r = threadIdx.y; r < 32; r += blockDim.y) {
    const int c = c0 + r;
    const long long p = p0 + threadIdx.x;
    tile[r][threadIdx.x] = (c < C && p < HW) ? s[c * HW + p] : 0.f;
  }
  __syncthreads();
  for (int r = threadIdx.y; r < 32; r += blockDim.y) {
    const long long p = p0 + r;
    const int c = c0 + threadIdx.x;
    if (p < HW && c < C) d[p * c_pad + c] = tile[threadIdx.x][r];
  }
}
cudaError_t launch_nchw_to_nhwc_f32(const float* src, float* dst, int B, int C, int H, int W, int c_pad, cudaStream_t s) {
  const long long HW = static_cast<long long>(H) * W;
  dim3 grid(static_cast<unsigned>((HW + 31) / 32), (C + 31) / 32, B), block(32, 8);
  nchw_to_nhwc_f32_kernel<<<grid, block, 0, s>>>(src, dst, C, c_pad, HW);
  return cudaGetLastError();
}
cudaError_t launch_nhwc_to_nchw_f32(const float* src, float* dst, int B, int C, int H, int W, int c_pad, cudaStream_t s) {
  return launch_unpack_state(NINT_TF32, src, dst, B, C, H, W, c_pad, s);
}

__device__ __forceinline__ int q_gate(int q) { return (q >> 4) & 3; }
__device__ __forceinline__ int q_chan(int q) { return (q >> 6) * 16 + (q & 15); }

template <typename E>
__global__ void pack_w_fwd_kernel(const float* __restrict__ w, const float* __restrict__ bias, E* __restrict__ wx,
                                  E* __restrict__ wh, float* __restrict__ bias_q, int cin, int hc_real, int hc, int hcb,
                                  int k, int cx_pad, int hc_pad, int bias_lane) {
  constexpr int CE = ElemTraits<E>::kPerChunk;
  const int n_blocks = hc / hcb, n_tile = 4 * hcb, taps = k * k;
  const int ctot = cin + hc_real;
  const int chx = cx_pad / CE, chh = hc_pad / CE;
  const long long nx = static_cast<long long>(n_blocks) * taps * chx * n_tile * CE;
  const long long nh = static_cast<long long>(n_blocks) * taps * chh * n_tile * CE;
  for (long long idx = blockIdx.x * static_cast<long long>(blockDim.x) + threadIdx.x; idx < nx + nh;
       idx += static_cast<long long>(gridDim.x) * blockDim.x) {
    const bool is_h = idx >= nx;
    long long r = is_h ? idx - nx : idx;
    const int nch = is_h ? chh : chx;
    const int e = static_cast<int>(r % CE); r /= CE;
    const int col = static_cast<int>(r % n_tile); r /= n_tile;
    const int tap = static_cast<int>(r % taps); r /= taps;
    const int ch = static_cast<int>(r % nch);
    const int nb = static_cast<int>(r / nch);
    const int q = nb * n_tile + col;
    const int oc = q_chan(q);
    const int cl = ch * CE + e;
    const int climit = is_h ? hc_real : cin;
    float v = 0.f;
    if (cl < climit && oc < hc_real)
      v = w[(static_cast<long long>(q_gate(q) * hc_real + oc) * ctot + (is_h ? cin + cl : cl)) * taps + tap];
    if (!is_h && cl == bias_lane && tap == taps / 2 && oc < hc_real && bias) v = bias[q_gate(q) * hc_real + oc];
    if (q_gate(q) != 2) v *= 0.5f;
    (is_h ? wh : wx)[is_h ? idx - nx : idx] = to_elem<E>(v);
  }
  for (int q = blockIdx.x * blockDim.x + threadIdx.x; q < 4 * hc; q += gridDim.x * blockDim.x)
    bias_q[q] = (bias && q_chan(q) < hc_real) ? bias[q_gate(q) * hc_real + q_chan(q)] * (q_gate(q) != 2 ? 0.5f : 1.f) : 0.f;
}

template <typename E>
__global__ void pack_w_bwd_kernel(const float* __restrict__ w, E* __restrict__ wdx, E* __restrict__ wdh, int cin,
                                  int cin_rows, int hc_real, int hc, int k) {
  constexpr int CE = ElemTraits<E>::kPerChunk;
  const int taps = k * k, ctot = cin + hc_real, nch = 4 * hc / CE;
  const long long nx = wdx ? static_cast<long long>(taps) * nch * cin_rows * CE : 0;
  const long long nh = static_cast<long long>(taps) * nch * hc * CE;
  for (long long idx = blockIdx.x * static_cast<long long>(blockDim.x) + threadIdx.x; idx < nx + nh;
       idx += static_cast<long long>(gridDim.x) * blockDim.x) {
    const bool is_h = idx >= nx;
    long long r = is_h ? idx - nx : idx;
    const int ncol = is_h ? hc : cin_rows;
    const int e = static_cast<int>(r % CE); r /= CE;
    const int col = static_cast<int>(r % ncol); r /= ncol;
    const int tap = static_cast<int>(r % taps);
    const int ch = static_cast<int>(r / taps);
    const int q = ch * CE + e;
    const int oc = q_chan(q);
    float v = 0.f;
    if (oc < hc_real && col < (is_h ? hc_real : cin)) {
      const int c = is_h ? cin + col : col;
      v = w[(static_cast<long long>(q_gate(q) * hc_real + oc) * ctot + c) * taps + (taps - 1 - tap)];
    }
    (is_h ? wdh : wdx)[is_h ? idx - nx : idx] = to_elem<E>(v);
  }
}

cudaError_t launch_pack_weights_fwd(int dtype, const float* w, const float* bias, void* wx, void* wh, float* bias_q,
                                    int cin, int hc_real, int hc, int hcb, int k, int cx_pad, int hc_pad, int bias_lane,
                                    cudaStream_t s) {
  if (dtype == NINT_BF16)
    pack_w_fwd_kernel<__nv_bfloat16><<<296, 256, 0, s>>>(w, bias, reinterpret_cast<__nv_bfloat16*>(wx),
                                                         reinterpret_cast<__nv_bfloat16*>(wh), bias_q, cin, hc_real, hc, hcb,
                                                         k, cx_pad, hc_pad, bias_lane);
  else
    pack_w_fwd_kernel<float><<<296, 256, 0, s>>>(w, bias, reinterpret_cast<float*>(wx), reinterpret_cast<float*>(wh),
                                                 bias_q, cin, hc_real, hc, hcb, k, cx_pad, hc_pad, bias_lane);
  return cudaGetLastError();
}
cudaError_t launch_pack_weights_bwd(int dtype, const float* w, void* wdx, void* wdh, int cin, int cin_rows, int hc_real,
                                    int hc, int k, cudaStream_t s) {
  if (dtype == NINT_BF16)
    pack_w_bwd_kernel<__nv_bfloat16><<<296, 256, 0, s>>>(w, reinterpret_cast<__nv_bfloat16*>(wdx),
                                                         reinterpret_cast<__nv_bfloat16*>(wdh), cin, cin_rows, hc_real, hc, k);
  else
    pack_w_bwd_kernel<float><<<296, 256, 0, s>>>(w, reinterpret_cast<float*>(wdx), reinterpret_cast<float*>(wdh), cin,
                                                 cin_rows, hc_real, hc, k);
  return cudaGetLastError();
}

template <typename E>
__global__ void head_fwd_kernel(const E* __restrict__ h, const float* __restrict__ w, const float* __restrict__ bias,
                                float* __restrict__ out, long long npix, int B, int hc, int hc_pad,
                                long long out_bstride) {
  extern __shared__ float s_w[];
  for (int i = threadIdx.x; i < hc_pad; i += blockDim.x) s_w[i] = i < hc ? w[i] : 0.f;
  __syncthreads();
  constexpr int V = 16 / sizeof(E);
  const long long total = static_cast<long long>(B) * npix;
  const float b0 = bias[0];
  for (long long gp = blockIdx.x * static_cast<long long>(blockDim.x) + threadIdx.x; gp < total;
       gp += static_cast<long long>(gridDim.x) * blockDim.x) {
    const E* hp = h + gp * hc_pad;
    float acc = b0;
    for (int c0 = 0; c0 < hc_pad; c0 += V) {
      float f[V];
      load_elems<E, V>(hp + c0, f);
#pragma unroll
      for (int j = 0; j < V; ++j) acc = fmaf(f[j], s_w[c0 + j], acc);
    }
    const long long b = gp / npix;
    out[b * out_bstride + (gp - b * npix)] = acc;
  }
}

cudaError_t launch_head_fwd(int dtype, const void* h, const float* w, const float* b, float* out, long long npix,
                            int B, int hc, int hc_pad, long long out_bstride, cudaStream_t s) {
  const long long total = static_cast<long long>(B) * npix;
  long long blocks = (total + 255) / 256;
  if (blocks > 148 * 8) blocks = 148 * 8;
  if (blocks <= 0) return cudaSuccess;
  if (dtype == NINT_BF16)
    head_fwd_kernel<__nv_bfloat16><<<blocks, 256, hc_pad * 4, s>>>(reinterpret_cast<const __nv_bfloat16*>(h), w, b, out,
                                                                  npix, B, hc, hc_pad, out_bstride);
  else
    head_fwd_kernel<float><<<blocks, 256, hc_pad * 4, s>>>(reinterpret_cast<const float*>(h), w, b, out, npix, B, hc,
                                                          hc_pad, out_bstride);
  return cudaGetLastError();
}

static int head_lanes_per_pixel(int dtype, int hc_pad) {
  const int cpp = hc_pad / (dtype == NINT_BF16 ? 8 : 4);
  int lp = 1;
  while (lp * 2 <= cpp && lp < 32) lp *= 2;
  return lp;
}

template <typename E>
__global__ void __launch_bounds__(256) head_bwd_kernel(const E* __restrict__ h, const float* __restrict__ dpred,
                                                       long long dpred_bstride, float* __restrict__ dw,
                                                       float* __restrict__ db, long long npix, int hc, int hc_pad, int lp,
                                                       float* __restrict__ part) {
  constexpr int V = 16 / sizeof(E);
  constexpr int KMAX = 2;
  const int cpp = hc_pad / V;
  const int lane = threadIdx.x & 31, warp = threadIdx.x >> 5;
  const int sub = lane & (lp - 1), ppw = 32 / lp;
  const int b = blockIdx.y;
  const float* dp = dpred + b * dpred_bstride;
  const E* hb = h + static_cast<long long>(b) * npix * hc_pad;
  float acc[KMAX][V];
#pragma unroll
  for (int k = 0; k < KMAX; ++k)
#pragma unroll
    for (int j = 0; j < V; ++j) acc[k][j] = 0.f;
  float accb = 0.f;
  const long long wstride = static_cast<long long>(gridDim.x) * (blockDim.x >> 5) * ppw;
  for (long long p0 = (static_cast<long long>(blockIdx.x) * (blockDim.x >> 5) + warp) * ppw; p0 < npix; p0 += wstride) {
    const long long px = p0 + lane / lp;
    if (px < npix) {
      const float d = __ldg(dp + px);
      const E* row = hb + px * hc_pad;
#pragma unroll
      for (int k = 0; k < KMAX; ++k) {
        const int ck = sub + k * lp;
        if (ck < cpp) {
          float f[V];
          load_elems<E, V>(row + ck * V, f);
#pragma unroll
          for (int j = 0; j < V; ++j) acc[k][j] = fmaf(d, f[j], acc[k][j]);
        }
      }
      if (sub == 0) accb += d;
    }
  }
  for (int o = lp; o < 32; o <<= 1) {
#pragma unroll
    for (int k = 0; k < KMAX; ++k)
#pragma unroll
      for (int j = 0; j < V; ++j) acc[k][j] += __shfl_xor_sync(0xffffffffu, acc[k][j], o);
    accb += __shfl_xor_sync(0xffffffffu, accb, o);
  }
  __shared__ float red[8][256 + 1];
  if (lane < lp) {
#pragma unroll
    for (int k = 0; k < KMAX; ++k) {
      const int ck = sub + k * lp;
      if (ck < cpp) {
#pragma unroll
        for (int j = 0; j < V; ++j) red[warp][ck * V + j] = acc[k][j];
      }
    }
    if (lane == 0) red[warp][256] = accb;
  }
  __syncthreads();
  const int blk = blockIdx.y * gridDim.x + blockIdx.x;
  for (int c = threadIdx.x; c <= hc; c += blockDim.x) {
    const int col = c < hc ? c : 256;
    float sum = 0.f;
    for (int wv = 0; wv < 8; ++wv) sum += red[wv][col];
    if (part) part[static_cast<long long>(blk) * (hc + 1) + c] = sum;
    else atomicAdd(c < hc ? dw + c : db, sum);
  }
}
__global__ void head_bwd_reduce_kernel(const float* __restrict__ part, int nblocks, int hc, float* __restrict__ dw,
                                       float* __restrict__ db) {
  for (int c = blockIdx.x * blockDim.x + threadIdx.x; c <= hc; c += gridDim.x * blockDim.x) {
    float sum = 0.f;
    for (int i = 0; i < nblocks; ++i) sum += part[static_cast<long long>(i) * (hc + 1) + c];
    if (c < hc) dw[c] += sum; else db[0] += sum;
  }
}

int head_bwd_blocks(int B) {
  int gx = (148 * 4 + B - 1) / B;
  return (gx < 1 ? 1 : gx) * B;
}
cudaError_t launch_head_bwd(int dtype, const void* h, const float* dpred, long long dpred_bstride, float* dw, float* db,
                            long long npix, int B, int hc, int hc_pad, float* part, cudaStream_t s) {
  if (hc_pad > 256) return cudaErrorInvalidValue;
  const int lp = head_lanes_per_pixel(dtype, hc_pad);
  const dim3 grid(head_bwd_blocks(B) / B, B);
  if (dtype == NINT_BF16)
    head_bwd_kernel<__nv_bfloat16><<<grid, 256, 0, s>>>(reinterpret_cast<const __nv_bfloat16*>(h), dpred, dpred_bstride,
                                                       dw, db, npix, hc, hc_pad, lp, part);
  else
    head_bwd_kernel<float><<<grid, 256, 0, s>>>(reinterpret_cast<const float*>(h), dpred, dpred_bstride, dw, db, npix,
                                               hc, hc_pad, lp, part);
  cudaError_t e = cudaGetLastError();
  if (e != cudaSuccess || !part) return e;
  head_bwd_reduce_kernel<<<1, 256, 0, s>>>(part, grid.x * grid.y, hc, dw, db);
  return cudaGetLastError();
}

__global__ void unpack_wgrad_kernel(const float* __restrict__ dw_acc, const float* __restrict__ db_acc,
                                    float* __restrict__ gw, float* __restrict__ gb, int cin, int hc_real, int hc, int k,
                                    int ncols, int cx_pad, int bias_col, int accumulate, int nparts,
                                    const float* __restrict__ db_resid, int resid_slots) {
  const int taps = k * k, ctot = cin + hc_real, hc4 = 4 * hc;
  const long long total = static_cast<long long>(hc4) * ctot * taps;
  const long long slice = static_cast<long long>(taps) * hc4 * ncols;
  const int np = nparts > 0 ? nparts : 1;
  for (long long idx = blockIdx.x * static_cast<long long>(blockDim.x) + threadIdx.x; idx < total;
       idx += static_cast<long long>(gridDim.x) * blockDim.x) {
    const int c = static_cast<int>(idx % ctot);
    long long r = idx / ctot;
    const int q = static_cast<int>(r % hc4);
    const int tap = static_cast<int>(r / hc4);
    if (q_chan(q) >= hc_real) continue;
    const int col = c < cin ? c : cx_pad + (c - cin);
    const float* src = dw_acc + (static_cast<long long>(tap) * hc4 + q) * ncols + col;
    float v = 0.f;
    for (int s = 0; s < np; ++s) v += src[s * slice];
    float* dst = gw + (static_cast<long long>(q_gate(q) * hc_real + q_chan(q)) * ctot + c) * taps + tap;
    *dst = accumulate ? *dst + v : v;
  }
  if (gb) {
    for (int q = blockIdx.x * blockDim.x + threadIdx.x; q < hc4; q += gridDim.x * blockDim.x) {
      if (q_chan(q) >= hc_real) continue;
      float* dst = gb + q_gate(q) * hc_real + q_chan(q);
      float v = 0.f;
      for (int s = 0; s < np; ++s)
        v += bias_col >= 0 ? dw_acc[s * slice + (static_cast<long long>(taps / 2) * hc4 + q) * ncols + bias_col]
                           : db_acc[static_cast<long long>(s) * hc4 + q];
      float r = 0.f;
      for (int i = 0; i < resid_slots; ++i) r += db_resid[static_cast<long long>(i) * hc4 + q];
      v += r;
      *dst = accumulate ? *dst + v : v;
    }
  }
}
cudaError_t launch_unpack_wgrad(const float* dw_acc, const float* db_acc, float* gw, float* gb, int cin, int hc_real,
                                int hc, int k, int ncols, int cx_pad, int bias_col, int accumulate, int nparts,
                                const float* db_resid, int resid_slots, cudaStream_t s) {
  unpack_wgrad_kernel<<<296, 256, 0, s>>>(dw_acc, db_acc, gw, gb, cin, hc_real, hc, k, ncols, cx_pad, bias_col, accumulate,
                                          nparts, db_resid, db_resid ? resid_slots : 0);
  return cudaGetLastError();
}

__device__ __forceinline__ float zscore_exact(float a, float sd, float rcp) {
  const float q0 = a * rcp;
  const float q1 = fmaf(fmaf(-sd, q0, a), rcp, q0);
  return fmaf(fmaf(-sd, q1, a), rcp, q1);
}

struct FuseChan {
  const float* src;
  long long frame_stride;
};

template <typename E, int CP, bool PLANAR>
__global__ void __launch_bounds__(256) fuse_kernel(const float* __restrict__ lev, const float* __restrict__ emis,
                                                   const float* __restrict__ mean, const float* __restrict__ stdv,
                                                   const float* __restrict__ statics, int S, E* __restrict__ out,
                                                   long long N, int L, int H, int W, int Hp, int Wp, int mode,
                                                   int ones_lane) {
  const int C = L + 1 + S;
  const int HWp = Hp * Wp;
  const long long HW = static_cast<long long>(H) * W;
  __shared__ FuseChan s_ch[CP];
  __shared__ float4 s_k[CP];
  __shared__ const float* s_base[CP];
  for (int c = threadIdx.x; c < CP; c += blockDim.x) {
// ... 253 lines not shown
```

Measured before the change: 5343.

## Store LSTM cell state in tile-blocked layout with 1D bulk copies

```diff
diff --git a/nasa_niswan_b200/csrc/nint_api.cu b/nasa_niswan_b200/csrc/nint_api.cu
--- a/nasa_niswan_b200/csrc/nint_api.cu
+++ b/nasa_niswan_b200/csrc/nint_api.cu
@@ -92,7 +92,7 @@
     int pw = 16, a_bufs = 0, b_stages = 0;
   };
   std::vector<WgBlock> wg_blocks;
-  CUtensorMap tme_C, tme_H, tme_G, tme_dC;
+  CUtensorMap tme_H, tme_G;
   bool weights_set = false;
   bool bias_folded = false;
   struct CachedConv { bool valid = false; ConvGemmParams g; };
@@ -257,6 +257,9 @@
 size_t act_bytes(const nint_plan* p, int slots, int c) {
   return static_cast<size_t>(slots) * p->B * p->H * p->W * c * p->esize;
 }
+size_t state_floats(const nint_plan* p, const Layer& y) {
+  return static_cast<size_t>(p->B) * p->tiles_y * p->tiles_x * p->tile_w * p->tile_h * y.hc;
+}
 
 size_t carve(nint_plan* p, uint8_t* base) {
   size_t off = 0;
@@ -271,9 +274,9 @@
   for (int l = 0; l < p->L; ++l) {
     Layer& y = p->layer[l];
     y.Hs = take(act_bytes(p, y.nslots_h, y.hc_pad));
-    y.Cs = reinterpret_cast<float*>(take(static_cast<size_t>(y.nslots_c) * npix * y.hc * 4));
+    y.Cs = reinterpret_cast<float*>(take(y.nslots_c * state_floats(p, y) * 4));
     y.G = tr ? take(act_bytes(p, p->T, 4 * y.hc)) : nullptr;
-    y.dC = tr ? reinterpret_cast<float*>(take(npix * y.hc * 4)) : nullptr;
+    y.dC = tr ? reinterpret_cast<float*>(take(state_floats(p, y) * 4)) : nullptr;
     const size_t wrow = static_cast<size_t>(p->ce) * p->esize;
     y.wx = take(static_cast<size_t>(y.n_blocks) * y.taps * y.chx * y.n_tile * wrow);
     y.wh = take(static_cast<size_t>(y.n_blocks) * y.taps * y.chh * y.n_tile * wrow);
@@ -308,7 +311,7 @@
   return base + act_bytes(p, 1, c) * slot;
 }
 inline float* cslot_ptr(const nint_plan* p, const Layer& y, int slot) {
-  return y.Cs + static_cast<size_t>(slot) * p->B * p->H * p->W * y.hc;
+  return y.Cs + static_cast<size_t>(slot) * state_floats(p, y);
 }
 
 void fill_common(const nint_plan* p, const Layer& y, ConvGemmParams& g) {
@@ -319,6 +322,9 @@
   g.B = p->B; g.b0 = 0; g.H = p->H; g.W = p->W;
   g.tile_w = p->tile_w; g.tile_h = p->tile_h; g.tiles_x = p->tiles_x; g.tiles_y = p->tiles_y;
   g.hc = y.hc; g.hc_pad = y.hc_pad; g.hcb = y.hcb;
+  g.c_state = y.Cs; g.dc_state = y.dC;
+  g.state_slot_stride = static_cast<long long>(state_floats(p, y));
+  g.state_img_stride = g.state_slot_stride / p->B;
   g.n_steps = 1;
   g.c_prev_none_step = -1;
 }
@@ -391,7 +397,7 @@
       ++s;
     }
     g.nseg = s;
-    g.tm_c = y.tme_C; g.tm_h = y.tme_H; g.tm_g = y.tme_G; g.tm_dc = y.tme_dC;
+    g.tm_h = y.tme_H; g.tm_g = y.tme_G;
     g.slot_g = (tr && epi == EPI_FWD) ? 0 : -1;
     if (conv_halo_plan(epi, p->dtype, g)) return fail("layer %d: the conv kernel's shared-memory plan does not fit (hidden %d, k %d)", l, y.hc, y.k);
     for (int i = 0; i < g.nseg; ++i)
@@ -445,7 +451,7 @@
   g.seg[0].tmap_act = y.tm_G; g.seg[0].wsel = wsel; g.seg[0].slot = t;
   g.seg[0].ksize = y.k; g.seg[0].nchunks = 4 * y.hc / p->ce;
   g.nseg = 1;
-  g.tm_c = y.tme_C; g.tm_h = y.tme_H; g.tm_g = y.tme_G; g.tm_dc = y.tme_dC;
+  g.tm_h = y.tme_H; g.tm_g = y.tme_G;
   g.slot_g = g.slot_c_in = g.slot_c_out = g.slot_h_out = g.slot_c_prev = -1;
   g.raw_out = raw_out;
   if (conv_halo_plan(EPI_RAW, p->dtype, g)) return fail("layer %d: the dgrad kernel's shared-memory plan does not fit (N %d, k %d)", l, n_rows, y.k);
@@ -819,14 +825,11 @@
     if (encode_act_map(&y.tm_H, p->dtype, y.Hs, y.hc_pad, p->W, p->H, p->B, y.nslots_h, ce, tw, th, false, pad_of(l))) return 1;
     if (l + 1 < p->L &&
         encode_act_map(&y.tm_H_up, p->dtype, y.Hs, y.hc_pad, p->W, p->H, p->B, y.nslots_h, ce, tw, th, false, pad_of(l + 1))) return 1;
-    if (encode_io_map(&y.tme_C, true, y.Cs, y.hc, p->W, p->H, p->B, y.nslots_c, 16)) return 1;
     if (encode_io_map(&y.tme_H, p->dtype == TF32, y.Hs, y.hc_pad, p->W, p->H, p->B, y.nslots_h, 16)) return 1;
     if (p->cfg.training) {
       if (encode_io_map(&y.tme_G, p->dtype == TF32, y.G, 4 * y.hc, p->W, p->H, p->B, p->T, 128 / p->esize)) return 1;
-      if (encode_io_map(&y.tme_dC, true, y.dC, y.hc, p->W, p->H, p->B, 1, 16)) return 1;
     } else {
-      y.tme_G = y.tme_C;
-      y.tme_dC = y.tme_C;
+      y.tme_G = y.tme_H;
     }
     for (auto& v : y.wmaps) v.clear();
     if (p->cfg.training) {
@@ -896,7 +899,7 @@
     for (int l = 0; l < p->L; ++l) {
       Layer& y = p->layer[l];
       CK(cudaMemsetAsync(y.Hs, 0, act_bytes(p, 1, y.hc_pad), st));
-      CK(cudaMemsetAsync(y.Cs, 0, static_cast<size_t>(p->B) * p->H * p->W * y.hc * 4, st));
+      CK(cudaMemsetAsync(y.Cs, 0, state_floats(p, y) * 4, st));
     }
   }
   p->zero_init = true;
@@ -912,11 +915,11 @@
     for (int j = 0; j < p->L; ++j) {
       Layer& z = p->layer[j];
       CK(cudaMemsetAsync(z.Hs, 0, act_bytes(p, 1, z.hc_pad), st));
-      CK(cudaMemsetAsync(z.Cs, 0, static_cast<size_t>(p->B) * p->H * p->W * z.hc * 4, st));
+      CK(cudaMemsetAsync(z.Cs, 0, state_floats(p, z) * 4, st));
     }
   }
   LAUNCH(p, K_OTHER, st, launch_pack_state(p->dtype, h, y.Hs, p->B, y.hc_real, p->H, p->W, y.hc_pad, st));
-  LAUNCH(p, K_OTHER, st, launch_nchw_to_nhwc_f32(c, y.Cs, p->B, y.hc_real, p->H, p->W, y.hc, st));
+  LAUNCH(p, K_OTHER, st, launch_nchw_to_blocked_f32(c, y.Cs, p->B, y.hc_real, p->H, p->W, y.hc, st));
   p->zero_init = false;
   return 0;
 }
@@ -928,7 +931,7 @@
   Layer& y = p->layer[l];
   cudaStream_t st = static_cast<cudaStream_t>(stream);
   if (h) LAUNCH(p, K_OTHER, st, launch_unpack_state(p->dtype, slot_ptr(p, y.Hs, p->final_slot_h, y.hc_pad), h, p->B, y.hc_real, p->H, p->W, y.hc_pad, st));
-  if (c) LAUNCH(p, K_OTHER, st, launch_nhwc_to_nchw_f32(cslot_ptr(p, y, p->final_slot_c), c, p->B, y.hc_real, p->H, p->W, y.hc, st));
+  if (c) LAUNCH(p, K_OTHER, st, launch_blocked_to_nchw_f32(cslot_ptr(p, y, p->final_slot_c), c, p->B, y.hc_real, p->H, p->W, y.hc, st));
   return 0;
 }
 
@@ -1210,7 +1213,7 @@
       ++s;
     }
     g.nseg = s;
-    g.tm_c = y.tme_C; g.tm_h = y.tme_H; g.tm_g = y.tme_G; g.tm_dc = y.tme_dC;
+    g.tm_h = y.tme_H; g.tm_g = y.tme_G;
     g.slot_c_in = g.slot_c_out = g.slot_h_out = -1;
     if (conv_halo_plan(EPI_BWD, p->dtype, g)) return fail("layer %d: the dgrad kernel's shared-memory plan does not fit (hidden %d, k %d)", l, y.hc, y.k);
     for (int i = 0; i < g.nseg; ++i) {
@@ -1424,14 +1427,10 @@
   if (!p->fwd_done || !p->gates_valid) return fail("nint_cell_backward: no forward to differentiate (or already consumed)");
   cudaStream_t st = static_cast<cudaStream_t>(stream);
   Layer& y = p->layer[0];
-  const size_t npix = static_cast<size_t>(p->B) * p->H * p->W;
   if (dh_out) LAUNCH(p, K_OTHER, st, launch_nchw_to_nhwc_f32(dh_out, p->dh_ext, p->B, y.hc_real, p->H, p->W, y.hc, st));
-  if (dc_out) {
-    CK(cudaMemsetAsync(y.dC, 0, npix * y.hc * 4, st));
-    LAUNCH(p, K_OTHER, st, launch_nchw_to_nhwc_f32(dc_out, y.dC, p->B, y.hc_real, p->H, p->W, y.hc, st));
-  }
+  if (dc_out) LAUNCH(p, K_OTHER, st, launch_nchw_to_blocked_f32(dc_out, y.dC, p->B, y.hc_real, p->H, p->W, y.hc, st));
   if (bptt_loop(p, nullptr, nullptr, dh_out ? p->dh_ext : nullptr, dc_out != nullptr, st)) return 1;
-  if (dc) LAUNCH(p, K_OTHER, st, launch_nhwc_to_nchw_f32(y.dC, dc, p->B, y.hc_real, p->H, p->W, y.hc, st));
+  if (dc) LAUNCH(p, K_OTHER, st, launch_blocked_to_nchw_f32(y.dC, dc, p->B, y.hc_real, p->H, p->W, y.hc, st));
   if (dh) {
     if (dgrad_raw(p, 0, 0, 3, y.hc, p->raw, st)) return 1;
     LAUNCH(p, K_OTHER, st, launch_unpack_raw(p->raw, dh, p->B, y.hc_real, p->H, p->W, y.hc, static_cast<long long>(y.hc_real) * p->H * p->W, st));
diff --git a/nasa_niswan_b200/csrc/nint_conv_halo.cu b/nasa_niswan_b200/csrc/nint_conv_halo.cu
--- a/nasa_niswan_b200/csrc/nint_conv_halo.cu
+++ b/nasa_niswan_b200/csrc/nint_conv_halo.cu
@@ -84,9 +84,8 @@
     }
   }
   if (warp == 3 && lane == 0 && EPI != EPI_RAW) {
-    prefetch_tensormap(&p.tm_c);
     prefetch_tensormap(&p.tm_g);
-    prefetch_tensormap(EPI == EPI_FWD ? &p.tm_h : &p.tm_dc);
+    if (EPI == EPI_FWD) prefetch_tensormap(&p.tm_h);
   }
   if (warp == 1 && lane == 0) {
     for (int s = 0; s < NA; ++s) {
diff --git a/nasa_niswan_b200/csrc/nint_epilogue.cuh b/nasa_niswan_b200/csrc/nint_epilogue.cuh
--- a/nasa_niswan_b200/csrc/nint_epilogue.cuh
+++ b/nasa_niswan_b200/csrc/nint_epilogue.cuh
@@ -219,6 +219,35 @@
 __device__ __forceinline__ void tma_store_wait_read() { asm volatile("cp.async.bulk.wait_group.read 0;" ::: "memory"); }
 __device__ __forceinline__ void tma_store_wait_all() { asm volatile("cp.async.bulk.wait_group 0;" ::: "memory"); }
 
+__device__ __forceinline__ long long state_block(const ConvGemmParams& p, int slot, const ItemCoord& c, int ch) {
+  const int tile = (c.y0 >> 4) * p.tiles_x + (c.x0 >> 3);
+  return slot * p.state_slot_stride + c.b * p.state_img_stride + (static_cast<long long>(tile) * p.hc + ch) * kTilePixels;
+}
+__device__ __forceinline__ void blk_lds8(uint32_t blk, int row, int half, float* v) {
+  lds128(blk + (2 * half) * 2048 + row * 16, v);
+  lds128(blk + (2 * half + 1) * 2048 + row * 16, v + 4);
+}
+__device__ __forceinline__ void blk_sts8(uint32_t blk, int row, int half, const float* v) {
+  sts128(blk + (2 * half) * 2048 + row * 16, v);
+  sts128(blk + (2 * half + 1) * 2048 + row * 16, v + 4);
+}
+__device__ __forceinline__ void blk_stg8(float* blk, int row, int half, const float* v) {
+  float* a = blk + (2 * half) * 512 + row * 4;
+  asm volatile("st.global.v4.f32 [%0], {%1,%2,%3,%4};" ::"l"(a), "f"(v[0]), "f"(v[1]), "f"(v[2]), "f"(v[3]) : "memory");
+  asm volatile("st.global.v4.f32 [%0], {%1,%2,%3,%4};" ::"l"(a + 512), "f"(v[4]), "f"(v[5]), "f"(v[6]), "f"(v[7]) : "memory");
+}
+__device__ __forceinline__ void bulk_load_block(void* smem_dst, const float* src, uint64_t* bar) {
+  asm volatile("cp.async.bulk.shared::cluster.global.mbarrier::complete_tx::bytes [%0], [%1], %2, [%3];" ::"r"(
+                   smem_u32(smem_dst)),
+               "l"(src), "n"(kEpiBoxBytes16), "r"(smem_u32(bar))
+               : "memory");
+}
+__device__ __forceinline__ void bulk_store_block(float* dst, const void* smem_src) {
+  asm volatile("cp.async.bulk.global.shared::cta.bulk_group [%0], [%1], %2;" ::"l"(dst), "r"(smem_u32(smem_src)),
+               "n"(kEpiBoxBytes16)
+               : "memory");
+}
+
 template <typename E, int ROWB>
 __device__ __forceinline__ void lds8(uint32_t base, int row, int ec, float* v) {
   if constexpr (sizeof(E) == 2) {
@@ -303,7 +332,7 @@
         if (leader) {
           if (p.slot_c_in >= 0) {
             mbar_arrive_expect_tx(&b.c_full[s], kEpiBoxBytes16);
-            tma_load_5d(fwd_c_slot(p, sE, s), &p.tm_c, &b.c_full[s], w.nb * p.hcb + grp * 16, c.x0, c.y0, c.b, slot_c_in);
+            bulk_load_block(fwd_c_slot(p, sE, s), p.c_state + state_block(p, slot_c_in, c, w.nb * p.hcb + grp * 16), &b.c_full[s]);
           } else {
             mbar_arrive(&b.c_full[s]);
           }
@@ -348,7 +377,7 @@
           if (!(NINT_DBG(p) & 1)) {
             const int ch = w.nb * p.hcb + grp * 16;
             if (kind == 0) {
-              tma_store_5d(&p.tm_c, fwd_c_slot(p, sE, s), ch, c.x0, c.y0, c.b, slot_c_out);
+              bulk_store_block(p.c_state + state_block(p, slot_c_out, c, ch), fwd_c_slot(p, sE, s));
             } else {
               const uint8_t* st = fwd_hg_stage(p, sE, s);
               tma_store_5d(&p.tm_h, st + p.e_off_h, ch, c.x0, c.y0, c.b, slot_h_out);
@@ -390,6 +419,7 @@
   const int row = quad * 32 + lane;
   const bool skip = (NINT_DBG(p) & 1) != 0;
   Tracer tr(p, 4, warp == kConvIoWarps && lane == 0);
+  const int ry = row >> 3, rx = row & 7;
   int cs = 0, hs = 0;
   uint32_t cph = 0, hph = 0;
   int abuf = 0;
@@ -403,6 +433,8 @@
       if (tile >= w.num_tiles) break;
       const uint32_t taddr = tmem_base + (static_cast<uint32_t>(quad * 32) << 16) +
                              static_cast<uint32_t>(abuf * p.acc_cols + gi * p.n_tile);
+      const ItemCoord c = decode_tile(p, tile);
+      const bool inside = c.y0 + ry < p.H && c.x0 + rx < p.W;
       for (int grp = 0; grp < ngroups; ++grp) {
         const uint32_t cslot = smem_u32(fwd_c_slot(p, sE, cs));
         const uint32_t st = smem_u32(fwd_hg_stage(p, sE, hs));
@@ -420,7 +452,7 @@
 #pragma unroll
         for (int g = 0; g < 4; ++g) tmem_ld8(taddr + grp * 64 + g * 16 + half * 8, a[g]);
         if (p.slot_c_in >= 0 && !skip) {
-          lds8<float, 64>(cslot, row, half, cn);
+          blk_lds8(cslot, row, half, cn);
         } else {
 #pragma unroll
           for (int j = 0; j < 8; ++j) cn[j] = 0.f;
@@ -445,13 +477,13 @@
             const float gg = act_tanh<FAST>(a[2][j]);
             const float go = act_sigmoid_halved<FAST>(a[3][j]);
             const float cv = fmaf(cn[j], gf, gi_ * gg);
-            cn[j] = cv;
+            cn[j] = inside ? cv : 0.f;
             float hv = go * act_tanh<FAST>(cv);
             if constexpr (DT == NINT_TF32) hv = round_tf32(hv);
             hn[j] = hv;
             a[0][j] = gi_; a[1][j] = gf; a[2][j] = gg; a[3][j] = go;
           }
-          sts8<float, 64>(cslot, row, half, cn);
+          blk_sts8(cslot, row, half, cn);
           sts8<E, GE::kHRowB>(st + p.e_off_h, row, half, hn);
           if (p.slot_g >= 0) {
 #pragma unroll
@@ -525,9 +557,8 @@
 #pragma unroll
           for (int bx = 0; bx < GE::kGateBoxes; ++bx)
             tma_load_5d(st + bx * GE::kGateBoxBytes, &p.tm_g, bar, q0 + bx * GE::kGateBoxCols, c.x0, c.y0, c.b, slot_g);
-          if (slot_c_prev >= 0)
-            tma_load_5d(st + p.e_off_c2, &p.tm_c, bar, grp * 16, c.x0, c.y0, c.b, slot_c_prev);
-          if (p.has_dc_in) tma_load_5d(st + p.e_off_dc, &p.tm_dc, bar, grp * 16, c.x0, c.y0, c.b, 0);
+          if (slot_c_prev >= 0) bulk_load_block(st + p.e_off_c2, p.c_state + state_block(p, slot_c_prev, c, grp * 16), bar);
+          if (p.has_dc_in) bulk_load_block(st + p.e_off_dc, p.dc_state + state_block(p, 0, c, grp * 16), bar);
         }
         if (mine) tr.stamp();
         if (++s == p.e_stages) {
@@ -572,7 +603,7 @@
 #pragma unroll
             for (int bx = 0; bx < GE::kGateBoxes; ++bx)
               tma_store_5d(&p.tm_g, st + bx * GE::kGateBoxBytes, q0 + bx * GE::kGateBoxCols, c.x0, c.y0, c.b, slot_g);
-            tma_store_5d(&p.tm_dc, st + p.e_off_dc, grp * 16, c.x0, c.y0, c.b, 0);
+            if constexpr (FUSED) bulk_store_block(p.dc_state + state_block(p, 0, c, grp * 16), st + p.e_off_dc);
             tma_store_commit();
             tma_store_wait_read();
           }
@@ -606,6 +637,7 @@
   const int row = quad * 32 + lane;
   const bool skip = (NINT_DBG(p) & 1) != 0;
   Tracer tr(p, 4, warp == kConvIoWarps && lane == 0);
+  const int ry = row >> 3, rx = row & 7;
   int s = 0;
   uint32_t ph = 0;
   int abuf = 0;
@@ -621,11 +653,12 @@
       const ItemCoord c = decode_tile(p, tile);
       const uint32_t taddr = tmem_base + (static_cast<uint32_t>(quad * 32) << 16) +
                              static_cast<uint32_t>(abuf * p.acc_cols + gi * p.n_tile);
+      const bool inside = c.y0 + ry < p.H && c.x0 + rx < p.W;
       float dpred = 0.f;
       if constexpr (EPI == EPI_BWD) {
         if (p.head_dpred) {
-          const int y = c.y0 + (row >> 3), x = c.x0 + (row & 7);
-          if (y < p.H && x < p.W)
+          const int y = c.y0 + ry, x = c.x0 + rx;
+          if (inside)
             dpred = p.head_dpred[(FUSED ? gp.step * p.head_dpred_sstride : 0) + c.b * p.head_dpred_bstride + static_cast<long long>(y) * p.W + x];
         }
       }
@@ -655,13 +688,13 @@
           lds_gate<E>(st, row, 2, half, gg);
           lds_gate<E>(st, row, 3, half, go);
           if (have_c_prev) {
-            lds8<float, 64>(st + p.e_off_c2, row, half, cp);
+            blk_lds8(st + p.e_off_c2, row, half, cp);
           } else {
 #pragma unroll
             for (int j = 0; j < 8; ++j) cp[j] = 0.f;
           }
           if (p.has_dc_in) {
-            lds8<float, 64>(st + p.e_off_dc, row, half, dc);
+            blk_lds8(st + p.e_off_dc, row, half, dc);
           } else {
 #pragma unroll
             for (int j = 0; j < 8; ++j) dc[j] = 0.f;
@@ -677,8 +710,8 @@
         }
         if (p.nseg > 0) tmem_ld_wait();
         if (p.dh_ext) {
-          const int y = c.y0 + (row >> 3), x = c.x0 + (row & 7);
-          if (y < p.H && x < p.W) {
+          const int y = c.y0 + ry, x = c.x0 + rx;
+          if (inside) {
             float e[8];
             load_elems<float, 8>(p.dh_ext + ((static_cast<long long>(c.b) * p.H + y) * p.W + x) * p.hc + c0, e);
 #pragma unroll
@@ -695,7 +728,7 @@
             const float d_i = dcv * gg[j];
             const float d_g = dcv * gi_[j];
             const float d_f = dcv * cp[j];
-            dc[j] = dcv * gf[j];
+            dc[j] = inside ? dcv * gf[j] : 0.f;
             const float i_ = gi_[j], f_ = gf[j], g_ = gg[j], o_ = go[j];
             gi_[j] = d_i * fmaf(-i_, i_, i_);
             gf[j] = d_f * fmaf(-f_, f_, f_);
@@ -727,7 +760,8 @@
               slot[grp * 64 + (lane >> 3) * 16 + half * 8 + (lane & 7)] += res[0];
             }
           }
-          sts8<float, 64>(st + p.e_off_dc, row, half, dc);
+          if constexpr (FUSED) blk_sts8(st + p.e_off_dc, row, half, dc);
+          else blk_stg8(p.dc_state + state_block(p, 0, c, grp * 16), row, half, dc);
           sts_gate<E>(st, row, 0, half, gi_);
           sts_gate<E>(st, row, 1, half, gf);
           sts_gate<E>(st, row, 2, half, gg);
diff --git a/nasa_niswan_b200/csrc/nint_kernels.h b/nasa_niswan_b200/csrc/nint_kernels.h
--- a/nasa_niswan_b200/csrc/nint_kernels.h
+++ b/nasa_niswan_b200/csrc/nint_kernels.h
@@ -41,7 +41,10 @@
   int w_resident;
   int debug_flags;
   int pdl;
-  CUtensorMap tm_c, tm_h, tm_g, tm_dc;
+  CUtensorMap tm_h, tm_g;
+  float* c_state;
+  float* dc_state;
+  long long state_slot_stride, state_img_stride;
   int slot_c_in, slot_c_out, slot_h_out, slot_g;
   int slot_c_prev, has_dc_in;
   int e_stages, e_stage_bytes, e_off_c, e_off_c2, e_off_dc, e_off_h;
@@ -124,7 +127,8 @@
 cudaError_t launch_unpack_state(int dtype, const void* src_nhwc, float* dst_nchw, int B, int C, int H, int W,
                                 int c_pad, cudaStream_t s);
 cudaError_t launch_nchw_to_nhwc_f32(const float* src, float* dst, int B, int C, int H, int W, int c_pad, cudaStream_t s);
-cudaError_t launch_nhwc_to_nchw_f32(const float* src, float* dst, int B, int C, int H, int W, int c_pad, cudaStream_t s);
+cudaError_t launch_nchw_to_blocked_f32(const float* src, float* dst, int B, int C, int H, int W, int c_pad, cudaStream_t s);
+cudaError_t launch_blocked_to_nchw_f32(const float* src, float* dst, int B, int C, int H, int W, int c_pad, cudaStream_t s);
 cudaError_t launch_pack_weights_fwd(int dtype, const float* w, const float* bias, void* wpack_x, void* wpack_h,
                                     float* bias_q, int cin, int hc_real, int hc, int hcb, int k, int cx_pad, int hc_pad,
                                     int bias_lane, cudaStream_t s);
diff --git a/nasa_niswan_b200/csrc/nint_pointwise.cu b/nasa_niswan_b200/csrc/nint_pointwise.cu
--- a/nasa_niswan_b200/csrc/nint_pointwise.cu
+++ b/nasa_niswan_b200/csrc/nint_pointwise.cu
@@ -211,8 +211,65 @@
   nchw_to_nhwc_f32_kernel<<<grid, block, 0, s>>>(src, dst, C, c_pad, HW);
   return cudaGetLastError();
 }
-cudaError_t launch_nhwc_to_nchw_f32(const float* src, float* dst, int B, int C, int H, int W, int c_pad, cudaStream_t s) {
-  return launch_unpack_state(NINT_TF32, src, dst, B, C, H, W, c_pad, s);
+
+__device__ __forceinline__ void blocked_coords(long long i, int tiles_x, int tiles_y, int nq, int& b, int& y, int& x,
+                                               int& c0) {
+  const int px = static_cast<int>(i & 127);
+  long long r = i >> 7;
+  const int q = static_cast<int>(r % nq);
+  r /= nq;
+  const int tx = static_cast<int>(r % tiles_x);
+  r /= tiles_x;
+  const int ty = static_cast<int>(r % tiles_y);
+  b = static_cast<int>(r / tiles_y);
+  y = ty * 16 + (px >> 3);
+  x = tx * 8 + (px & 7);
+  c0 = q * 4;
+}
+__global__ void nchw_to_blocked_f32_kernel(const float* __restrict__ src, float4* __restrict__ dst, int C, int H, int W,
+                                           int tiles_x, int tiles_y, int nq, long long n) {
+  const long long i = static_cast<long long>(blockIdx.x) * blockDim.x + threadIdx.x;
+  if (i >= n) return;
+  int b, y, x, c0;
+  blocked_coords(i, tiles_x, tiles_y, nq, b, y, x, c0);
+  float v[4] = {0.f, 0.f, 0.f, 0.f};
+  if (y < H && x < W) {
+    const long long HW = static_cast<long long>(H) * W;
+    const float* s = src + static_cast<long long>(b) * C * HW + static_cast<long long>(y) * W + x;
+#pragma unroll
+    for (int j = 0; j < 4; ++j)
+      if (c0 + j < C) v[j] = s[(c0 + j) * HW];
+  }
+  dst[i] = make_float4(v[0], v[1], v[2], v[3]);
+}
+__global__ void blocked_to_nchw_f32_kernel(const float4* __restrict__ src, float* __restrict__ dst, int C, int H, int W,
+                                           int tiles_x, int tiles_y, int nq, long long n) {
+  const long long i = static_cast<long long>(blockIdx.x) * blockDim.x + threadIdx.x;
+  if (i >= n) return;
+  int b, y, x, c0;
+  blocked_coords(i, tiles_x, tiles_y, nq, b, y, x, c0);
+  if (y >= H || x >= W || c0 >= C) return;
+  const float4 v4 = src[i];
+  const float v[4] = {v4.x, v4.y, v4.z, v4.w};
+  const long long HW = static_cast<long long>(H) * W;
+  float* d = dst + static_cast<long long>(b) * C * HW + static_cast<long long>(y) * W + x;
+#pragma unroll
+  for (int j = 0; j < 4; ++j)
+    if (c0 + j < C) d[(c0 + j) * HW] = v[j];
+}
+cudaError_t launch_nchw_to_blocked_f32(const float* src, float* dst, int B, int C, int H, int W, int c_pad, cudaStream_t s) {
+  const int tiles_x = (W + 7) / 8, tiles_y = (H + 15) / 16, nq = c_pad / 4;
+  const long long n = static_cast<long long>(B) * tiles_y * tiles_x * nq * 128;
+  nchw_to_blocked_f32_kernel<<<static_cast<unsigned>((n + 255) / 256), 256, 0, s>>>(src, reinterpret_cast<float4*>(dst), C, H, W,
+                                                                                      tiles_x, tiles_y, nq, n);
+  return cudaGetLastError();
+}
+cudaError_t launch_blocked_to_nchw_f32(const float* src, float* dst, int B, int C, int H, int W, int c_pad, cudaStream_t s) {
+  const int tiles_x = (W + 7) / 8, tiles_y = (H + 15) / 16, nq = c_pad / 4;
+  const long long n = static_cast<long long>(B) * tiles_y * tiles_x * nq * 128;
+  blocked_to_nchw_f32_kernel<<<static_cast<unsigned>((n + 255) / 256), 256, 0, s>>>(reinterpret_cast<const float4*>(src), dst, C, H, W,
+                                                                                      tiles_x, tiles_y, nq, n);
+  return cudaGetLastError();
 }
 
 __device__ __forceinline__ int q_gate(int q) { return (q >> 4) & 3; }
```

After: 5271, median of 6. No clear change (-1.3%).
